# BurryChen/lv_slam

Hardware: AMD Instinct MI355X
Metric: NDT registrations/sec (64k-pt Velodyne pairs) (higher is better)
Workload: dtype f32 terms, f64 accumulation

## Files before the change

include/mi355_ndt.h:

```cpp
#ifndef MI355_NDT_H_
#define MI355_NDT_H_

#include <stddef.h>
#include <stdint.h>

#ifdef __cplusplus
extern "C" {
#endif

#define MI355NDT_OK               0
#define MI355NDT_ERR_BAD_HANDLE  (-1)
#define MI355NDT_ERR_BAD_ARG     (-2)
#define MI355NDT_ERR_HIP         (-3)
#define MI355NDT_ERR_GRID        (-4)
#define MI355NDT_ERR_NO_DEVICE   (-5)
#define MI355NDT_ERR_UNSUPPORTED (-6)
#define MI355NDT_WARN_TOLERANCE_ARITH 1
#define MI355NDT_TOLERANCE_MIN_HITS   4096
#define MI355NDT_ERR_STATE       (-7)

enum mi355ndt_neighbor { MI355NDT_KDTREE = 0, MI355NDT_DIRECT26 = 1, MI355NDT_DIRECT7 = 2, MI355NDT_DIRECT1 = 3 };
enum mi355ndt_variant { MI355NDT_VARIANT_OMP = 0 , MI355NDT_VARIANT_PCA = 1  };

typedef struct mi355ndt_params {
  float  resolution;
  double step_size;
  double outlier_ratio;
  double trans_epsilon;
  int    max_iterations;
  int    neighbor_mode;
  int    variant;
  int    min_points_per_voxel;
  double min_covar_eigvalue_mult;
} mi355ndt_params;

typedef struct mi355ndt_result {
  float     final_colmajor[16];
  double    trans_probability;
  double    score;
  int       iterations;
  int       converged;
  int       sweeps;
  int       status;
  long long hits_last;
} mi355ndt_result;

typedef struct mi355ndt_voxel {
  int32_t idx;
  int32_t n;
  double  mean[3];
  float   icov[9];
  int32_t weight;
} mi355ndt_voxel;

typedef struct mi355ndt_profile {
  double    sweep_ms;
  long long sweep_launches;
  double    sweep_alg_bytes;
  long long sweep_hits;
  long long sweep_points;
  double    build_ms;
  long long build_launches;
  double    build_alg_bytes;
  double    update_ms;
  long long update_launches;
  long long async_fallbacks;
  long long stream_launches;
  long long stream_carried;
  long long stream_redone;
  long long cloud_uploads;
  long long cloud_upload_bytes;
  long long cloud_transfers;
  long long cloud_promotions;
  long long stream_reserved_slots;
  long long stream_launch_slots;
  long long score_only_sweeps;
} mi355ndt_profile;

typedef struct mi355ndt_handle mi355ndt_handle;

const char* mi355ndt_version(void);
int mi355ndt_device_count(void);
int mi355ndt_host_numa_node(int device);

int mi355ndt_default_params(mi355ndt_params* p);

int mi355ndt_create(const mi355ndt_params* params, int device, mi355ndt_handle** out);
int mi355ndt_destroy(mi355ndt_handle* h);

int mi355ndt_set_params(mi355ndt_handle* h, const mi355ndt_params* params);
int mi355ndt_get_params(const mi355ndt_handle* h, mi355ndt_params* out);

int mi355ndt_set_stream(mi355ndt_handle* h, void* hip_stream);
const char* mi355ndt_last_error(const mi355ndt_handle* h);


int mi355ndt_set_target(mi355ndt_handle* h, const void* pts, size_t n, size_t stride_bytes);
int mi355ndt_set_source(mi355ndt_handle* h, const void* pts, size_t n, size_t stride_bytes);
int mi355ndt_promote_source_to_target(mi355ndt_handle* h);
int mi355ndt_align(mi355ndt_handle* h, const float guess_colmajor[16], mi355ndt_result* out);
int mi355ndt_get_aligned(mi355ndt_handle* h, void* out_pts, size_t stride_bytes);

int mi355ndt_get_incremental(mi355ndt_handle* h, int pair, float transformation_colmajor[16], float previous_colmajor[16]);

int mi355ndt_get_fitness_score(mi355ndt_handle* h, double max_range, double* score, long long* n_inliers);
int mi355ndt_fitness_score_T(mi355ndt_handle* h, const float T_colmajor[16], double max_range, double* score, long long* n_inliers);

int mi355ndt_calculate_score(mi355ndt_handle* h, const void* pts, size_t n, size_t stride_bytes, double* score);

int mi355ndt_convert_transform(const double x[6], float out_colmajor[16]);

enum mi355ndt_option {
  MI355NDT_OPT_F32_SUM_ORDER = 1,
  MI355NDT_OPT_ASYNC_ALIGN = 2,
  MI355NDT_OPT_DEBUG_ASYNC_ABORT = 3,
  MI355NDT_OPT_STREAM_THRESHOLD = 4,
  MI355NDT_OPT_STREAM_RESERVE = 5,
  MI355NDT_OPT_DEBUG_ASYNC_RINGS = 6,
  MI355NDT_OPT_ARITH = 7,
  MI355NDT_OPT_SCORE_ONLY_LAST_SWEEP = 8,
  MI355NDT_OPT_KF_FITNESS_CELL_MM = 9,
  MI355NDT_OPT_OUTLIER_CELL_MM = 10,
  MI355NDT_OPT_PREFILTER_GROUP = 11,
  MI355NDT_OPT_POSE_MODEL = 12,
  MI355NDT_OPT_NDT_CLASS = 13
};
int mi355ndt_set_option(mi355ndt_handle* h, int option, int value);
int mi355ndt_get_option(const mi355ndt_handle* h, int option, int* value);

int mi355ndt_derivatives(mi355ndt_handle* h, const double p[6], double* score, double g[6], double H[36], long long* hits);
int mi355ndt_compute_hessian(mi355ndt_handle* h, const double p[6], double H[36]);
int mi355ndt_derivatives_T(mi355ndt_handle* h, const float T_colmajor[16], const float Rj_rowmajor[9],
                           double* score, double g[6], double H[36], long long* hits);
int mi355ndt_get_grid(mi355ndt_handle* h, int pair, int min_b[3], int max_b[3], int div_b[3], int* n_voxels);
int mi355ndt_get_voxels(mi355ndt_handle* h, int pair, mi355ndt_voxel* out, size_t capacity);


int mi355ndt_batch_reserve(mi355ndt_handle* h, int n_pairs, size_t max_target_pts, size_t max_source_pts);
int mi355ndt_batch_set_target(mi355ndt_handle* h, int pair, const void* pts, size_t n, size_t stride_bytes);
int mi355ndt_batch_set_source(mi355ndt_handle* h, int pair, const void* pts, size_t n, size_t stride_bytes);
int mi355ndt_batch_set_clouds(mi355ndt_handle* h, int first_pair, int n, const void* const* targets, const size_t* target_counts,
                              const void* const* sources, const size_t* source_counts, size_t stride_bytes, int n_threads);
int mi355ndt_batch_bind_device(mi355ndt_handle* h, int n_pairs,
                               const float* d_targets, const int* target_counts, size_t target_pitch,
                               const float* d_sources, const int* source_counts, size_t source_pitch);
int mi355ndt_batch_build_targets(mi355ndt_handle* h);
int mi355ndt_batch_align(mi355ndt_handle* h, const float* guesses_colmajor, mi355ndt_result* out);
int mi355ndt_batch_size(const mi355ndt_handle* h);
int mi355ndt_batch_fitness_scores(mi355ndt_handle* h, const float* T_colmajor, double max_range, double* scores, long long* n_inliers);
int mi355ndt_batch_pose_records(mi355ndt_handle* h, int id_base, int id_stride, void* d_records, size_t capacity);

int mi355ndt_stream_begin(mi355ndt_handle* h, int n_contexts , int max_pairs, size_t max_target_pts, size_t max_source_pts);
int mi355ndt_stream_submit(mi355ndt_handle* h, int n_pairs, const float* d_targets, const int* target_counts, size_t target_pitch,
                           const float* d_sources, const int* source_counts, size_t source_pitch, const float* guesses_colmajor,
                           long long* batch_id);
int mi355ndt_stream_submit_host(mi355ndt_handle* h, int n_pairs, const void* const* targets, const size_t* target_counts, const void* const* sources,
                                const size_t* source_counts, size_t stride_bytes, const float* guesses_colmajor, int n_threads, long long* batch_id);
int mi355ndt_stream_collect(mi355ndt_handle* h, long long batch_id, mi355ndt_result* out);
int mi355ndt_stream_pose_records(mi355ndt_handle* h, void* d_records, size_t capacity, int id_base, int id_stride);
int mi355ndt_pack_pose_records(const mi355ndt_result* results, int n, int id_base, int id_stride, void* records, size_t capacity);
int mi355ndt_stream_end(mi355ndt_handle* h);

int mi355ndt_set_latency_mode(mi355ndt_handle* h, int on);

typedef struct mi355ndt_seq_params {
  double keyframe_delta_trans;
  double keyframe_delta_angle;
  double keyframe_delta_time;
} mi355ndt_seq_params;

typedef struct mi355ndt_seq_frame {
  double odom_colmajor[16];
  float  tf_s2k_colmajor[16];
  double trans_probability;
  double dx, da, dt;
  int    key_id;
  int    new_keyframe;
  int    iterations, converged;
  int    aligns;
  int    pad;
} mi355ndt_seq_frame;

typedef struct mi355ndt_seq_stats {
  double    upload_ms;
  double    build_ms;
  double    track_ms;
// ... 187 lines not shown
```

lv_slam_amd/csrc/mi355_ndt.hip:

```cpp
#include <hip/hip_runtime.h>

#include <cstdio>
#include <cstdlib>
#include <cstddef>
#include <cstring>
#include <string>
#include <vector>
#include <algorithm>
#include <cmath>
#include <mutex>
#include <atomic>
#include <thread>
#include <sched.h>
#include <fstream>
#include <chrono>
#include <memory>
#include <map>
#include <array>
#include <type_traits>

#include "mi355_ndt.h"
#include "ndt_math.hpp"
#include "ndt_types.hpp"
#include "ndt_build.hpp"
#include "ndt_segsort.hpp"
#include "ndt_sweep.hpp"
#include "ndt_newton.hpp"
#include "ndt_update.hpp"
#include "ndt_upload.hpp"
#include "ndt_pose_record.hpp"
#include "ndt_hessian.hpp"
#include "ndt_sweep_kd.hpp"
#include "ndt_fitness.hpp"
#include "ndt_prefilter.hpp"
#include "ndt_prefilter_batch.hpp"
#include "ndt_prefilter_approx.hpp"
#include "ndt_mapcloud.hpp"
#include "ndt_keyframe.hpp"
#include "ndt_kffitness.hpp"
#include "ndt_outlier.hpp"
#include "ndt_outlier_batch.hpp"
#include "ndt_gicp.hpp"
#include "gicp_bfgs.hpp"
#include "gicp_lockstep.hpp"
#include "ndt_icp.hpp"
#include "icp_outer.hpp"
#include "ndt_sequence.hpp"
#include "ndt_async.hpp"
#include "ndt_hostmem.hpp"
#include "ndt_grid_state.hpp"
#ifndef NDT_SINGLE_TU
#include "ndt_ord1_list.hpp"
#include "ndt_fast_list.hpp"
#define NDT_DECLARE extern template
NDT_ORD1_KERNELS(NDT_DECLARE)
NDT_FAST_KERNELS(NDT_DECLARE)
#endif

#include "ndt_engine.hpp"
#include "ndt_host_life.hpp"
#include "ndt_host_upload.hpp"
#include "ndt_host_profile.hpp"
#include "ndt_host_build.hpp"
#include "ndt_host_sweep.hpp"
#include "ndt_host_align.hpp"
#include "ndt_host_hooks.hpp"
#include "ndt_host_fitness.hpp"
#include "ndt_host_voxel.hpp"
#include "ndt_host_prefilter.hpp"
#include "ndt_host_mapcloud.hpp"
#include "ndt_host_keyframe.hpp"
#include "ndt_host_kffitness.hpp"
#include "ndt_host_outlier.hpp"
#include "ndt_host_gicp.hpp"
#include "ndt_host_gicp_batch.hpp"
#include "ndt_host_icp.hpp"
#include "ndt_host_icp_batch.hpp"
#include "ndt_host_sequence.hpp"
#include "ndt_host_stream.hpp"
```

lv_slam_amd/csrc/ndt_async.hpp:

```cpp
#pragma once
#include "ndt_types.hpp"
#include "ndt_math.hpp"
#include "ndt_sweep.hpp"
#include "ndt_update.hpp"
#include "ndt_pose_record.hpp"

#define ASYNC_POS_STRIDE 32
#define ASYNC_ARR_STRIDE 16
#define ASYNC_MAX_CTX    4
#define ASYNC_MAX_CARRY  128
#define ASYNC_CTX_SHIFT  24

struct AsyncCtx {
  const float* src; size_t pitch;
  PairState* st; const GridDesc* gd; const BitWord* words; const VoxelRec* recs; const float* cent;
  double* partials; const int* src_cnt; unsigned* arrived; mi355ndt_result* results;
  unsigned* n_done;
  int must_finish;
  int pose_base; PoseRecord* pose; int pose_stride;
  int score_only;
};
struct AsyncTab { AsyncCtx c[ASYNC_MAX_CTX]; };
#define NDT_GP(T) __attribute__((address_space(1))) T*
struct AsyncCtxG {
// ... 129 lines not shown
    if (rc == NEWTON_SWEEP && stop_thresh > 0 && !C.must_finish)
      suspend = n_live - __hip_atomic_load((const gu32*)&ctl->fin, RLX_AGENT) <= (unsigned)stop_thresh;
    if (rc == NEWTON_SWEEP && !suspend) {
      const unsigned g = __hip_atomic_fetch_add((gu32*)&ctl->pub, 1u, RLX_AGENT);
      __hip_atomic_store((gu32*)reinterpret_cast<unsigned*>(ring + (size_t)(g & 7u) * ring_cap + (g >> 3)), (unsigned)tw, RLX_AGENT);
    } else if (rc == NEWTON_SWEEP) {
      const unsigned k = __hip_atomic_fetch_add((gu32*)&ctl->susp, 1u, RLX_AGENT);
      if (k < (unsigned)ASYNC_MAX_CARRY) __hip_atomic_store((gu32*)&ctl->carry[k], (unsigned)tw, RLX_AGENT);
      asm volatile("s_waitcnt vmcnt(0)" ::: "memory");
      __hip_atomic_fetch_add((gu32*)&ctl->fin, 1u, RLX_AGENT);
    } else {
      if (C.pose) C.pose[b] = pose_record(Ssh.final_cm, Ssh.score, Ssh.it, Ssh.converged, C.pose_base + b * C.pose_stride);
      asm volatile("s_waitcnt vmcnt(0)" ::: "memory");
      if (C.n_done) __hip_atomic_fetch_add((gu32*)C.n_done, 1u, RLX_AGENT);
      __hip_atomic_fetch_add((gu32*)&ctl->fin, 1u, RLX_AGENT);
    }
  }
  TL_STAMP(9);
  if (rc == NEWTON_SWEEP) {
    constexpr int RBI = (int)(offsetof(PairState, reb_inc) / 8);
    double pn[6]; float inc[16];
    newton_rebase(Ssh.p, Ssh.dir, Ssh.a_t, pn, inc);
    if (lane == 0) {
      for (int a = 0; a < 6; a++) __hip_atomic_store(sg + RB0 + a, (unsigned long long)__double_as_longlong(pn[a]), RLX_AGENT);
      for (int a = 0; a < 8; a++)
        __hip_atomic_store(sg + RBI + a, (unsigned long long)__float_as_uint(inc[2 * a]) | ((unsigned long long)__float_as_uint(inc[2 * a + 1]) << 32), RLX_AGENT);
      asm volatile("s_waitcnt vmcnt(0)" ::: "memory");
      __hip_atomic_store(sg + RBT, (unsigned long long)(long long)Ssh.sweeps, RLX_AGENT);
    }
  }
  __builtin_amdgcn_s_setprio(0);
}

NDT_KERNEL void k_stream_inputs(const unsigned* __restrict__ host_in, unsigned* __restrict__ dev_in, const unsigned n_in, unsigned* __restrict__ clear, const unsigned n_clear,
                                unsigned long long* stamp) {
  if (threadIdx.x == 0 && stamp) *stamp = (unsigned long long)wall_clock64();
  for (unsigned i = threadIdx.x; i < n_in; i += blockDim.x) dev_in[i] = host_in[i];
  for (unsigned i = threadIdx.x; i < n_clear; i += blockDim.x) clear[i] = 0u;
}

NDT_KERNEL void k_stream_status(const AsyncCtl* __restrict__ ctl, const CtxStat* __restrict__ stat, volatile unsigned* host_slot, const unsigned seq) {
  const int i = threadIdx.x;
  static_assert(offsetof(AsyncCtl, fin) == 4 && offsetof(AsyncCtl, susp) == 16 && offsetof(StreamStatus, ctx) == 16 && offsetof(StreamStatus, seq) == 80 && offsetof(StreamStatus, build_t0) == 88, "status layout");
  if (i < 4) host_slot[i] = reinterpret_cast<const unsigned*>(ctl)[1 + i];
  else if (i < 4 + 4 * ASYNC_MAX_CTX) host_slot[i] = reinterpret_cast<const unsigned*>(stat)[i - 4];
  __threadfence_system();
  __syncthreads();
  if (i == 0) host_slot[20] = seq;
}

#define NDT_CTX_PARAMS(i) const float* __restrict__ src##i, size_t pitch##i, PairState* st##i, const GridDesc* __restrict__ gd##i, const BitWord* __restrict__ words##i, \
                          const VoxelRec* __restrict__ recs##i, double* partials##i, const int* __restrict__ src_cnt##i, unsigned* arrived##i, const float* __restrict__ cent##i
#define NDT_CTX_SEL(f, ci) ((ci) == 0 ? f##0 : (ci) == 1 ? f##1 : (ci) == 2 ? f##2 : f##3)
template <bool PCA, int K, int ORD>
__global__ void __launch_bounds__(SWEEP_THREADS, (SweepTune<PCA, K, ORD>::WPE))
k_align_async(const AsyncTab* __restrict__ tab, int items_per_pair, int* ring, int ring_cap, AsyncCtl* ctl, SweepConst sc, unsigned long long* hits_total,
              double step_max, double eps, int max_iterations, int stop_thresh, unsigned debug_abort_pos, unsigned debug_ring_mask, int claim_items,
              NDT_CTX_PARAMS(0), NDT_CTX_PARAMS(1), NDT_CTX_PARAMS(2), NDT_CTX_PARAMS(3)) {
  const int lane = threadIdx.x & 63, wv = threadIdx.x >> 6;
  __shared__ double exp_tab[64];
  __shared__ PairState Ssh[WAVES];
  __shared__ double sol[WAVES][SOL_WORDS];
  if (threadIdx.x < 64) exp_tab[threadIdx.x] = ndtm::c_exp2_64[threadIdx.x];
  __syncthreads();
  const int x = blockIdx.x & 7;
  if (!((debug_ring_mask >> x) & 1u)) return;
  const gu32* ringx = (const gu32*)reinterpret_cast<const unsigned*>(ring + (size_t)x * ring_cap);
  const gu32* fin_p = (const gu32*)&ctl->fin;
  gu32* pos_p = (gu32*)&ctl->pos[x * ASYNC_POS_STRIDE];
  const unsigned n_live = ctl->n_live;
  const int I = items_per_pair;
  const int CLAIM = K == 1 ? ASYNC_CLAIM(1) : (claim_items == 2 ? 2 : 1);
  const int Iu = I / CLAIM;
  Timeline tl;
  auto give_up = [&]() {
    __hip_atomic_store((gu32*)&ctl->abort_, 1u, RLX_AGENT);
    __hip_atomic_store((gu32*)&ctl->fin, n_live, RLX_AGENT);
  };
  bool held = false;
  bool helped = false;
  unsigned held_pos = 0;
  const gu64* pubfin_p = (const gu64*)reinterpret_cast<const unsigned long long*>(ctl);
  static_assert(offsetof(AsyncCtl, pub) == 0 && offsetof(AsyncCtl, fin) == 4, "pub and fin are polled as one 8-byte word");
  auto wait_ticket = [&](unsigned& p, int have) -> int {
    int w = have;
    unsigned sp = p;
    int st = 0;
    if (lane == 0) {
      unsigned spins = helped ? ASYNC_HELP_AFTER : 0u;
      const int t = (int)(p / (unsigned)Iu);
      while (w < 0) {
        const unsigned long long pf = __hip_atomic_load(pubfin_p, RLX_AGENT);
        if ((unsigned)(pf >> 32) >= n_live) { w = -2; break; }
        if (ASYNC_HELP_RINGS && spins >= ASYNC_HELP_AFTER && (spins & 3u) == 3u) {
          const unsigned y = ((unsigned)x + 1u + (spins >> 2) % 7u) & 7u;
          gu32* pos_y = (gu32*)&ctl->pos[y * ASYNC_POS_STRIDE];
          const unsigned q = __hip_atomic_load(pos_y, RLX_AGENT);
          const unsigned pubv = (unsigned)pf;
          const unsigned slots_y = pubv > y ? ((pubv - 1u - y) >> 3) + 1u : 0u;
          const unsigned tq = q / (unsigned)Iu;
          if (tq < slots_y && (int)tq < ring_cap) {
            unsigned expect = q;
            if (__hip_atomic_compare_exchange_strong(pos_y, &expect, q + 1u, __ATOMIC_RELAXED, __ATOMIC_RELAXED, __HIP_MEMORY_SCOPE_AGENT)) {
              const gu32* slot = (const gu32*)reinterpret_cast<const unsigned*>(ring + (size_t)y * ring_cap + tq);
              int ws = (int)__hip_atomic_load(slot, RLX_AGENT);
              unsigned lag = 0;
              while (ws < 0 && ++lag <= ASYNC_SPIN_LIMIT) { __builtin_amdgcn_s_sleep(2); ws = (int)__hip_atomic_load(slot, RLX_AGENT); }
              if (ws < 0) { give_up(); w = -2; break; }
              w = ws; sp = q; st = 1;
              break;
            }
          }
        }
        __builtin_amdgcn_s_sleep(32);
        if (t < ring_cap) w = (int)__hip_atomic_load(ringx + t, RLX_AGENT);
        if (++spins > ASYNC_SPIN_LIMIT) { give_up(); w = -2; break; }
      }
    }
    w = __builtin_amdgcn_readfirstlane(w);
    helped = __builtin_amdgcn_readfirstlane(st) != 0;
    if (helped) { held = true; held_pos = p; p = __builtin_amdgcn_readfirstlane(sp); }
    return w;
  };
  unsigned pos = 0;
  if (lane == 0) pos = __hip_atomic_fetch_add(pos_p, 1u, RLX_AGENT);
  pos = __builtin_amdgcn_readfirstlane(pos);
  int tw = -1;
  if (lane == 0 && (int)(pos / (unsigned)Iu) < ring_cap) tw = (int)__hip_atomic_load(ringx + pos / (unsigned)Iu, RLX_AGENT);
  tw = wait_ticket(pos, tw);
  if (tw < 0) return;
  unsigned pose_w = sweep_pose_words(NDT_CTX_SEL(st, tw >> ASYNC_CTX_SHIFT) + (tw & ((1 << ASYNC_CTX_SHIFT) - 1)));
#pragma unroll 1
  for (;;) {
    if (x == 0 && pos == debug_abort_pos) { if (lane == 0) give_up(); break; }
    const int rem = (int)(pos % (unsigned)Iu) * CLAIM;
    TL_STAMP(10);
    const int ci = tw >> ASYNC_CTX_SHIFT;
    AsyncCtx C = async_ctx_load(tab, ci);
    C.src = NDT_CTX_SEL(src, ci); C.pitch = NDT_CTX_SEL(pitch, ci); C.st = NDT_CTX_SEL(st, ci); C.gd = NDT_CTX_SEL(gd, ci); C.words = NDT_CTX_SEL(words, ci);
    C.recs = NDT_CTX_SEL(recs, ci); C.partials = NDT_CTX_SEL(partials, ci); C.src_cnt = NDT_CTX_SEL(src_cnt, ci); C.arrived = NDT_CTX_SEL(arrived, ci);
    C.cent = NDT_CTX_SEL(cent, ci);
    const int b = tw & ((1 << ASYNC_CTX_SHIFT) - 1);
    const int n_b = C.src_cnt[b];
#ifndef ASYNC_D1_PIPE
#define ASYNC_D1_PIPE 1
#endif
    const bool last = __builtin_amdgcn_readlane(pose_w, POSE_W_LAST) != 0;
    auto items = [&](auto so_c) {
      constexpr bool SO = decltype(so_c)::value;
      if constexpr (K == 1 && ASYNC_D1_PIPE && ORD != 2) {
        sweep_rows_d1<PCA, ORD, ASYNC_CLAIM(1), SO>(b, rem, C.src, C.pitch, C.gd, C.words, C.recs, C.partials, I, sc, exp_tab, pose_w, n_b, b, tl);
      } else {
#pragma unroll 1
        for (int k = 0; k < CLAIM; k++)
          sweep_item<PCA, K, 8, false, ORD, true, SO>(b, rem + k, C.src, C.pitch, C.st, C.gd, C.words, C.recs, C.partials, I, sc, C.cent, nullptr, exp_tab, pose_w, n_b, b, tl);
      }
    };
    if (last) items(std::true_type()); else items(std::false_type());
    unsigned npos = held_pos;
    if (lane == 0 && !held) npos = __hip_atomic_fetch_add(pos_p, 1u, RLX_AGENT);
    held = false;
    asm volatile("s_waitcnt vmcnt(0)" ::: "memory");
    npos = __builtin_amdgcn_readfirstlane(npos);
    const int tn = (int)(npos / (unsigned)Iu);
    unsigned old = 0;
    int ntw = -1;
    if (lane == 0) {
      old = __hip_atomic_fetch_add((gu32*)(C.arrived + (size_t)b * ASYNC_ARR_STRIDE), (unsigned)CLAIM, RLX_AGENT);
      if (tn < ring_cap) ntw = (int)__hip_atomic_load(ringx + tn, RLX_AGENT);
    }
    old = __builtin_amdgcn_readfirstlane(old);
    ntw = __builtin_amdgcn_readfirstlane(ntw);
    unsigned npose = 0;
    if (ntw >= 0) npose = sweep_pose_words(NDT_CTX_SEL(st, ntw >> ASYNC_CTX_SHIFT) + (ntw & ((1 << ASYNC_CTX_SHIFT) - 1)));
    TL_STAMP(8);
    if ((old + (unsigned)CLAIM) % (unsigned)I == 0u) {
      async_update(C, b, tw, n_b, I, Ssh[wv], sol[wv], ring, ring_cap, ctl, n_live, stop_thresh, hits_total, step_max, eps, max_iterations, tl);
      TL_STAMP(15);
    }
    if (ntw < 0) {
      ntw = wait_ticket(npos, ntw);
      if (ntw < 0) break;
      npose = sweep_pose_words(NDT_CTX_SEL(st, ntw >> ASYNC_CTX_SHIFT) + (ntw & ((1 << ASYNC_CTX_SHIFT) - 1)));
    }
    tw = ntw; pos = npos; pose_w = npose;
  }
  tl.flush(0, 16);
}
```

lv_slam_amd/csrc/ndt_build.hpp:

```cpp
#pragma once
#include "ndt_types.hpp"
#include "ndt_math.hpp"

__device__ __forceinline__ unsigned mm_enc_max(int ord) { return (unsigned)ord ^ 0x80000000u; }
__device__ __forceinline__ unsigned mm_enc_min(int ord) { return ~((unsigned)ord ^ 0x80000000u); }
__device__ __forceinline__ int mm_dec_max(unsigned e) { return (int)(e ^ 0x80000000u); }
__device__ __forceinline__ int mm_dec_min(unsigned e) { return (int)(~e ^ 0x80000000u); }

#define MM_ILP 4
struct __attribute__((packed, aligned(4))) MmQuad { float v[4]; };
__global__ void __launch_bounds__(256) k_minmax(const float* __restrict__ tgt, size_t pitch, const int* __restrict__ cnt, unsigned* mm) {
  const int b = blockIdx.y;
  const int n = cnt[b];
  const float* X = tgt + (size_t)b * 3 * pitch;
  int mn[3] = {INT_MAX, INT_MAX, INT_MAX}, mx[3] = {INT_MIN, INT_MIN, INT_MIN};
  auto take = [&](const float x, const float y, const float z) {
    if (!finite3(x, y, z)) return;
    const int ox = f2ord(x), oy = f2ord(y), oz = f2ord(z);
    mn[0] = min(mn[0], ox); mx[0] = max(mx[0], ox);
    mn[1] = min(mn[1], oy); mx[1] = max(mx[1], oy);
    mn[2] = min(mn[2], oz); mx[2] = max(mx[2], oz);
  };
  const int stride = (int)(gridDim.x * blockDim.x) * 4;
  for (int i0 = (int)(blockIdx.x * blockDim.x + threadIdx.x) * 4; i0 < n; i0 += stride * MM_ILP) {
// ... 97 lines not shown


#define RUN_ILP 4
template <typename KeyT>
__device__ __forceinline__ void run_heads(const KeyT* __restrict__ K, size_t pitch, size_t i0, size_t stride, int min_points, unsigned cmask,
                                          bool head[RUN_ILP], unsigned cell[RUN_ILP]) {
  KeyT k0[RUN_ILP], km[RUN_ILP], kl[RUN_ILP];
  const size_t span = (size_t)(min_points > 0 ? min_points - 1 : 0);
#pragma unroll
  for (int u = 0; u < RUN_ILP; u++) {
    const size_t i = i0 + (size_t)u * stride;
    const bool in = i < pitch;
    k0[u] = in ? K[i] : (KeyT)cmask;
    km[u] = (in && i != 0) ? K[i - 1] : ~(KeyT)0;
    kl[u] = (in && i + span < pitch) ? K[i + span] : ~(KeyT)0;
  }
#pragma unroll
  for (int u = 0; u < RUN_ILP; u++) {
    const size_t i = i0 + (size_t)u * stride;
    cell[u] = (unsigned)k0[u] & cmask;
    head[u] = i < pitch && cell[u] != cmask && (i == 0 || km[u] != k0[u]) && (i + span < pitch) && kl[u] == k0[u];
  }
}
#define LS_SLICE (64 * RUN_ILP)
static inline unsigned ls_slice_cap(int min_points) { return (unsigned)(LS_SLICE / (min_points > 0 ? min_points : 1) + 2); }
static inline unsigned ls_slices(size_t pitch) { return (unsigned)((pitch + LS_SLICE - 1) / LS_SLICE); }
template <typename KeyT>
__global__ void __launch_bounds__(256) k_mark(const KeyT* __restrict__ keys, size_t pitch, const GridDesc* __restrict__ gd,
                                               BitWord* words, unsigned* heads, unsigned* head_cnt, unsigned n_slices, unsigned slice_cap,
                                               int min_points, int cb) {
  const int b = blockIdx.y;
  const int lane = threadIdx.x & 63;
  const unsigned q = blockIdx.x * 4u + (threadIdx.x >> 6);
  if (q >= n_slices) return;
  const size_t i0 = (size_t)q * LS_SLICE + lane;
  bool head[RUN_ILP];
  unsigned cell[RUN_ILP];
  run_heads<KeyT>(keys + (size_t)b * pitch, pitch, i0, 64, min_points, (1u << cb) - 1u, head, cell);
  unsigned* H = heads + ((size_t)b * n_slices + q) * slice_cap;
  const unsigned long long below = (1ull << lane) - 1ull;
  unsigned n = 0;
#pragma unroll
  for (int u = 0; u < RUN_ILP; u++) {
    const unsigned long long hm = __ballot(head[u]);
    if (head[u]) {
      atomicOr(&words[gd[b].word_off + (cell[u] >> 6)].bits, 1ull << (cell[u] & 63));
      H[n + (unsigned)__popcll(hm & below)] = (unsigned)(i0 + (size_t)u * 64);
    }
    n += (unsigned)__popcll(hm);
  }
  if (lane == 0) head_cnt[(size_t)b * n_slices + q] = n;
}
#define RANK_ROWS 8
__global__ void __launch_bounds__(1024) k_rank(GridDesc* gd, BitWord* words, const unsigned* __restrict__ heads, const unsigned* __restrict__ head_cnt,
                                                 unsigned n_slices, unsigned slice_cap, unsigned* seg_start) {
  __shared__ unsigned wtot[17];
  const int b = blockIdx.x;
  BitWord* W = words + gd[b].word_off;
  const int nw = gd[b].nwords;
  const int lane = threadIdx.x & 63, wv = threadIdx.x >> 6;
  unsigned base = 0;
  for (int w0 = 0; w0 < nw; w0 += 1024 * RANK_ROWS) {
    const int wbase = w0 + wv * 64 * RANK_ROWS;
    unsigned c[RANK_ROWS], ex[RANK_ROWS], run = 0;
#pragma unroll
    for (int u = 0; u < RANK_ROWS; u++) { const int w = wbase + u * 64 + lane; c[u] = (w < nw) ? (unsigned)__popcll(W[w].bits) : 0u; }
#pragma unroll
    for (int u = 0; u < RANK_ROWS; u++) {
      unsigned inc = c[u];
#pragma unroll
      for (int o = 1; o < 64; o <<= 1) { const unsigned t = __shfl_up(inc, o); if (lane >= o) inc += t; }
      ex[u] = run + inc - c[u];
      run += __shfl(inc, 63);
    }
    if (lane == 0) wtot[wv] = run;
    __syncthreads();
    if (wv == 0) {
      const unsigned v = lane < 16 ? wtot[lane] : 0u;
      unsigned inc = v;
#pragma unroll
      for (int o = 1; o < 16; o <<= 1) { const unsigned t = __shfl_up(inc, o); if (lane >= o) inc += t; }
      if (lane < 16) wtot[lane] = inc - v;
      if (lane == 15) wtot[16] = inc;
    }
    __syncthreads();
    const unsigned off = base + wtot[wv];
#pragma unroll
    for (int u = 0; u < RANK_ROWS; u++) { const int w = wbase + u * 64 + lane; if (w < nw) W[w].prefix = off + ex[u]; }
    base += wtot[16];
    __syncthreads();
  }
  if (threadIdx.x == 0) gd[b].n_voxels = (int)base;
  unsigned hbase = 0;
  for (unsigned q0 = 0; q0 < n_slices; q0 += 1024) {
    const unsigned q = q0 + threadIdx.x;
    const unsigned c = q < n_slices ? head_cnt[(size_t)b * n_slices + q] : 0u;
    unsigned tot;
    const unsigned ex = block_exscan<1024>(c, &tot, wtot);
    const unsigned* H = heads + ((size_t)b * n_slices + q) * slice_cap;
    unsigned* S = seg_start + gd[b].rec_off + hbase + ex;
    for (unsigned k = 0; k < c; k++) S[k] = H[k];
    hbase += tot;
  }
}

__global__ void __launch_bounds__(256) k_sorted_points(const float* __restrict__ tgt, size_t pitch, const unsigned* __restrict__ vals, float4* __restrict__ sorted,
                                                        int nx, int n_targets) {
  int b, bx;
  if (!xcd_map(nx, n_targets, bx, b)) return;
  const float* X = tgt + (size_t)b * 3 * pitch;
  const unsigned* V = vals + (size_t)b * pitch;
  float4* P = sorted + (size_t)b * pitch;
  const size_t i0 = ((size_t)bx * 256 + threadIdx.x);
  const size_t stride = (size_t)nx * 256;
  for (size_t i = i0; i < pitch; i += stride * RUN_ILP) {
    unsigned v[RUN_ILP];
    float4 q[RUN_ILP];
#pragma unroll
    for (int u = 0; u < RUN_ILP; u++) { const size_t j = i + u * stride; v[u] = j < pitch ? V[j] : 0u; }
#pragma unroll
    for (int u = 0; u < RUN_ILP; u++) { const unsigned k = v[u] < pitch ? v[u] : 0u; q[u] = make_float4(X[k], X[pitch + k], X[2 * pitch + k], 0.f); }
#pragma unroll
    for (int u = 0; u < RUN_ILP; u++) { const size_t j = i + u * stride; if (j < pitch) P[j] = q[u]; }
  }
}

#ifdef NDT_TIMELINE
__device__ unsigned long long g_ltl[16];
#define LTL_DECL unsigned long long ltl[12] = {0, 0, 0, 0, 0, 0, 0, 0, 0, 0, 0, 0}; unsigned long long ltl_last = __builtin_readcyclecounter(); const unsigned long long ltl_t0 = ltl_last
#define LTL_STAMP(k) do { __builtin_amdgcn_sched_barrier(0); const unsigned long long t_ = __builtin_readcyclecounter(); ltl[k] += t_ - ltl_last; ltl_last = t_; __builtin_amdgcn_sched_barrier(0); } while (0)
#define LTL_COUNT(k, v) do { ltl[k] += (unsigned long long)(v); } while (0)
#define LTL_FLUSH() do { ltl[10] = 1; ltl[11] = __builtin_readcyclecounter() - ltl_t0; if ((threadIdx.x & 63) == 0 && (blockIdx.x % 24) == (threadIdx.x >> 6) * 5) for (int k_ = 0; k_ < 12; k_++) atomicAdd(&g_ltl[k_], ltl[k_]); } while (0)
#define LTL_ARRIVED1(a) asm volatile("" : "+v"(a))
#else
#define LTL_DECL do {} while (0)
#define LTL_STAMP(k) do {} while (0)
#define LTL_COUNT(k, v) do {} while (0)
#define LTL_FLUSH() do {} while (0)
#define LTL_ARRIVED1(a) do {} while (0)
#endif
#define LS_WAVES 4
template <typename KeyT, bool CENT, bool SORTED = false>
__global__ void __launch_bounds__(64 * LS_WAVES) k_leafsum(const float* __restrict__ tgt, size_t pitch,
                                                           const KeyT* __restrict__ keys, const unsigned* __restrict__ vals ,
                                                           const GridDesc* __restrict__ gd, const unsigned* __restrict__ seg_start,
                                                           double* sums, int* vox_idx, int* vox_n, int cb, float* cent,
                                                           int nx, int n_targets) {
  __shared__ double term[LS_WAVES][64][9];
  __shared__ float termf[CENT ? LS_WAVES : 1][64][3];
  int b, bx;
  if (!xcd_map(nx, n_targets, bx, b)) return;
// ... 249 lines not shown
```

lv_slam_amd/csrc/ndt_engine.hpp:

```cpp
#pragma once

struct mi355ndt_handle;
struct EngineDel { void operator()(mi355ndt_handle* e) const { (void)mi355ndt_destroy(e); } };

struct StreamCtx {
  long long batch_id = -1; int n_pairs = 0;
  bool busy = false;
  bool redo = false;
  bool done_sync = false;
  long long launch = -1;
  DevBuf<int> d_in; PinBuf<int> h_in; unsigned* h_in_dev = nullptr;
  PinBuf<mi355ndt_result> h_res; mi355ndt_result* d_res_map = nullptr;
  std::vector<float> guesses;
  PoseRecord* d_pose = nullptr; int pose_cap = 0, pose_base = 0, pose_stride = 1;
  std::unique_ptr<mi355ndt_handle, EngineDel> e;
};
struct StreamState {
  static constexpr int EV = 16;
  bool sync_only = false, drop_carry = true;
  int nctx = 0, max_pairs = 0, items = 0, ring_cap = 0, thresh = 0;
  bool thresh_given = false;
  size_t max_tgt = 0, max_src = 0;
  int plan_cb = 0; size_t plan_words = 0;
  void* pose_next = nullptr; size_t pose_cap_next = 0; int pose_base_next = 0, pose_stride_next = 1;
  long long next_id = 0, launches = 0, counted = 0;
  long long recovered_upto = -1;
  DevBuf<AsyncCtl> d_ctl;
  DevBuf<int> d_ring;
  DevBuf<CtxStat> d_stat;
  HipStream build_stream; int reserve_wg = 0, launch_slots = 0;
  HipEvent ev_built[ASYNC_MAX_CTX], ev_launched[EV], ev_prepared[EV]; bool prep_first = true;
  PinBuf<volatile StreamStatus> h_status; StreamStatus* d_status = nullptr;
  StreamCtx ctx[ASYNC_MAX_CTX];
};

struct VoxelScratch {
  DevBuf<float> in, x, out;
  DevBuf<unsigned char> keep;
  DevBuf<unsigned> keys, vals;
  DevBuf<unsigned> hist, offs, tmp;
  DevBuf<int> flag, pos;
  DevBuf<int> mm, cnt, aabb, stat;
  DevBuf<PfGrid> grid; DevBuf<McBox> box;
  DevBuf<unsigned char> tab; PinBuf<unsigned char> h_tab;
  DevBuf<double> part; PinBuf<double> h_part;
  PinBuf<int> h_ret;
  bool pending = false;
};

struct CloudIndex {
  static constexpr int NO_INDEX = -1;
  DevBuf<unsigned char> blob; int status = NO_INDEX; int n_fin = 0;
};

struct GicpCache {
  DevBuf<double> cov;
  int k = -1; double eps = 0.0;
};
struct GicpSide {
  DevBuf<float> rows_own; size_t n = 0, pitch = 0;
  int kf_id = -1; bool set = false;
  CloudIndex index; GicpCache cache;
};

struct mi355ndt_handle {
  int device = 0;
  HipStream own_stream;
  hipStream_t stream = nullptr;
  mi355ndt_params prm;
  std::string err;

  int n_pairs = 0, cap_pairs = 0;
  size_t tgt_pitch = 0, src_pitch = 0;
  size_t own_tgt_pitch = 0, own_src_pitch = 0;
  int own_tgt_pairs = 0, own_src_pairs = 0;
  DevBuf<float> d_tgt_own, d_src_own;
  const float *d_tgt = nullptr, *d_src = nullptr;
  DevBuf<int> d_tgt_cnt_own, d_src_cnt_own;
  int *d_tgt_cnt = nullptr, *d_src_cnt = nullptr;
  std::vector<int> h_tgt_cnt, h_src_cnt;
  std::vector<int> up_tgt_cnt, up_src_cnt;
  bool have_target = false, have_source = false;
  GridsBuilt built{};
// ... 35 lines not shown
    DevBuf<int> idx, m; DevBuf<double> maha, part; DevBuf<float> moved;
    PinBuf<double> h_rec; double* d_rec = nullptr;
    bool have_corr = false, have_final = false; int n_matched = 0;
    float final_cm[16] = {1,0,0,0, 0,1,0,0, 0,0,1,0, 0,0,0,1};
  } gicp;
  struct GicpBatch {
    struct Slot {
      GicpSide side;
      DevBuf<int> idx; DevBuf<double> maha, part;
      bool have_final = false; float final_cm[16];
    };
    std::vector<Slot> slot;
    DevBuf<int> m;
    PinBuf<double> h_rec; double* d_rec = nullptr;
    PinBuf<GcSlot> h_tab; DevBuf<GcSlot> d_tab;
    int rounds = 0; std::vector<int> requests;
  } gicp_batch;
  struct IcpWork {
    DevBuf<float> W, d2; DevBuf<int> idx; DevBuf<double> part;
    size_t n = 0, pitch = 0;
    bool have_final = false; IcpRun run;
  };
  struct Icp {
    mi355ndt_icp_params prm{0.0, 10, -DBL_MAX, 1.3407807929942596e154, 3, 0};
    GicpSide side[2];
    IcpWork work;
    DevBuf<int> m; DevBuf<float> moved;
    PinBuf<double> h_rec; double* d_rec = nullptr;
  } icp;
  struct IcpBatch {
    struct Slot { GicpSide side; IcpWork work; };
    std::vector<Slot> slot;
    DevBuf<int> m;
    PinBuf<double> h_rec; double* d_rec = nullptr;
    PinBuf<IcpSlot> h_tab; DevBuf<IcpSlot> d_tab;
    int rounds = 0; std::vector<int> requests;
  } icp_batch;
  float last_final[16] = {1,0,0,0, 0,1,0,0, 0,0,1,0, 0,0,0,1};
  PinBuf<unsigned> h_pin_u;

  DevBuf<PairState> d_state;
  DevBuf<double> d_partials;
  int chunks_per_pair = 0;
  int rows_per_pair = 0, pts_per_chunk = CHUNK_PTS;
  int items_per_pair = 0;
  bool async_force = false;
  bool async_align = true;
  int score_only_last = 1;
  DevBuf<int> d_ring; DevBuf<unsigned> d_arrived; DevBuf<AsyncCtl> d_actl;
  PinBuf<AsyncCtl> h_pin_actl;
  DevBuf<AsyncTab> d_atab;
  unsigned debug_abort_pos = 0xFFFFFFFFu;
  unsigned debug_ring_mask = 0xFFu;
  int arith = 0;
  DevBuf<VoxelRecF> d_recs_fast;
  int pose_model = 0;
  int ndt_class = 0;
  DevBuf<double> d_pcl_rows;
  DevBuf<float> d_euler_rows;
  int f32_sum_order = 0;
  double gauss_last[3] = {0, 0, 0};
  DevBuf<float> d_score_pts; DevBuf<double> d_score_part;
  bool latency_mode = false;
  bool seq_running = false;
  int fine_it = 0;
  int fine_tiles = 2;
  int dyn_shift = -1;
  DevBuf<int> d_grid_of;
  const int* d_grid_of_use = nullptr;
  DevBuf<SeqState> d_seq; DevBuf<mi355ndt_seq_frame> d_seq_out; DevBuf<double> d_stamps;
  PinBuf<volatile int> h_seq_flags; int* d_seq_flags = nullptr;
  DevBuf<float> d_guess_own;
  float* d_guess = nullptr;
  PinBuf<float> h_pin_guess;
  DevBuf<mi355ndt_result> d_results;
  DevBuf<int> d_active;
  DevBuf<int> d_active_list;
  DevBuf<SweepCtl> d_ctl;
  int ctl_idx = 0;
  int n_cu = 256;
  PinBuf<int> h_pin_active;
  HipEvent ev_burst[2];
  DevBuf<unsigned long long> d_hits;
  DevBuf<float> d_hook;
  DevBuf<float> d_aligned;
  PinBuf<float> h_pin_aligned;
  struct UpSlot { PinBuf<float> h; DevBuf<float> d; HipEvent ev; bool used = false, filling = false; };
  static constexpr int UP_SLOTS = 12;
  UpSlot up[UP_SLOTS];
  int up_next = 0;
  static constexpr int UP_STREAMS = 4;
  HipStream copy_stream[UP_STREAMS];
  HipEvent ev_uploads[UP_STREAMS], ev_compute;
  bool uploads_pending = false;
  std::mutex up_mtx;

  bool async_build = false;
  int plan_cb = 0; size_t plan_words = 0;
  unsigned* d_bstat = nullptr;
  bool counts_preloaded = false;
  bool build_stamped = false;
  bool word_off_cleared = false;

  std::unique_ptr<StreamState> ss;
  int s_thresh_opt = -1;
  int s_reserve_opt = -1;
// ... 44 lines not shown
  sc.K = neighbor_K(mode);
  sc.table = sc.K == 1 ? 0 : sc.K == 7 ? 1 : 2;
}

static void gauss_constants3(double outlier_ratio, float resolution, double d[3]) {
  double c1 = 10 * (1 - outlier_ratio);
  double c2 = outlier_ratio / pow((double)resolution, 3);
  d[2] = -log(c2);
  d[0] = -log(c1 + c2) - d[2];
  d[1] = -2 * log((-log(c1 * exp(-0.5) + c2) - d[2]) / d[0]);
}
static void gauss_constants(const mi355ndt_params& p, double& d1, double& d2) {
  double d[3];
  gauss_constants3(p.outlier_ratio, p.resolution, d);
  d1 = d[0]; d2 = d[1];
}

static int check_params(const mi355ndt_params& p) {
  if (!(p.resolution > 0) || !std::isfinite(p.resolution)) return MI355NDT_ERR_BAD_ARG;
  if (p.neighbor_mode < 0 || p.neighbor_mode > 3) return MI355NDT_ERR_BAD_ARG;
  if (p.variant < 0 || p.variant > 1) return MI355NDT_ERR_BAD_ARG;
  if (p.min_points_per_voxel < 1) return MI355NDT_ERR_BAD_ARG;
  if (p.max_iterations < 0) return MI355NDT_ERR_BAD_ARG;
  return MI355NDT_OK;
}

static int eff_model(const mi355ndt_handle* h) { return class_model(h->ndt_class, h->pose_model); }
static GridExtras eff_extras(const mi355ndt_handle* h, bool live = false) { return grid_extras(h->prm, model_arith(h->pose_model, h->arith, h->ndt_class), live, h->ndt_class); }
static bool fast_served(const mi355ndt_handle* h) { return eff_extras(h).recs_fast; }
static float* euler_rows_of(const mi355ndt_handle* h) { return eff_model(h) == POSE_MODEL_EULER ? h->d_euler_rows.p : nullptr; }
static double* pcl_rows_of(const mi355ndt_handle* h) { return h->ndt_class == NDT_CLASS_PCL ? h->d_pcl_rows.p : nullptr; }
#define NOT_EULER(h, what) do { \
    if ((h)->ndt_class == NDT_CLASS_PCL) { (h)->err = what ": not served under MI355NDT_OPT_NDT_CLASS = 1"; return MI355NDT_ERR_UNSUPPORTED; } \
    if ((h)->pose_model == POSE_MODEL_EULER) { (h)->err = what ": not served under MI355NDT_OPT_POSE_MODEL = 1"; return MI355NDT_ERR_UNSUPPORTED; } } while (0)

enum GridWant { GRIDS_ANY, GRIDS_CONFIG, GRIDS_LIVE };
static int ensure_grids(mi355ndt_handle* h, GridWant want);
template <typename N>
static void cloud_changed(mi355ndt_handle* h, bool tgt, int first_pair, int n, const N* counts) {
  std::lock_guard<std::mutex> lk(h->up_mtx);
  std::vector<int>& cnt = tgt ? h->h_tgt_cnt : h->h_src_cnt;
  for (int k = 0; k < n; k++) cnt[(size_t)(first_pair + k)] = (int)counts[k];
  (tgt ? h->have_target : h->have_source) = true;
  if (tgt) h->built.valid = false;
}
static void cloud_changed(mi355ndt_handle* h, bool tgt, int pair, size_t count) { cloud_changed(h, tgt, pair, 1, &count); }
static void clouds_reset(mi355ndt_handle* h, bool tgt, bool src) {
  std::lock_guard<std::mutex> lk(h->up_mtx);
  if (tgt) { std::fill(h->h_tgt_cnt.begin(), h->h_tgt_cnt.end(), 0); h->have_target = false; h->built.valid = false; }
  if (src) { std::fill(h->h_src_cnt.begin(), h->h_src_cnt.end(), 0); h->have_source = false; }
}
static bool async_served(const mi355ndt_handle* h) { return h->async_align && !mt_is_live(h->prm) && !is_pca_kd(h->prm) && model_leaves_rounds(h->pose_model, h->ndt_class); }
static double sweep_alg_bytes(double points, int K) { return points * (12.0 + 4.0 * K); }
static int launch_slots(const mi355ndt_handle* h, const SweepConst& sc, bool fast) { return h->n_cu * sweep_wpe(sc.K, fast); }
```

lv_slam_amd/csrc/ndt_host_align.hpp:

```cpp
#pragma once
static void tolerance_warnings(const mi355ndt_handle* h, mi355ndt_result* out, int n) {
  if (!fast_served(h)) return;
  for (int b = 0; b < n; b++)
    if (out[b].status == MI355NDT_OK && (out[b].hits_last < MI355NDT_TOLERANCE_MIN_HITS || out[b].iterations >= h->prm.max_iterations + 2))
      out[b].status = MI355NDT_WARN_TOLERANCE_ARITH;
}
static int ensure_seq_flags(mi355ndt_handle* h) {
  if (!h->d_seq_flags) {
    HIPCHK(h, h->h_seq_flags.reserve(16, hipHostMallocMapped | hipHostMallocCoherent));
    if (!(h->d_seq_flags = h->h_seq_flags.dev())) { h->err = "hipHostGetDevicePointer failed"; return MI355NDT_ERR_HIP; }
  }
  return MI355NDT_OK;
}

static int align_pump(mi355ndt_handle* h, SweepConst sc, int B) {
  int rc = ensure_seq_flags(h);
  if (rc) return rc;
  hipStream_t s = h->stream;
  h->h_seq_flags[0] = 0; h->h_seq_flags[1] = -1;
  sc.host_flags = h->d_seq_flags;
  sc.seq_no = 1;
  sc.rebase_block = 1;
  rc = launch_sweep(h, sc);
  if (rc) return rc;
  const int depth = 2;
  const long long max_rounds = h->prm.max_iterations + 4;
  long long enq = 0;
  auto t_progress = std::chrono::steady_clock::now();
  long long seen_last = -1;
  for (;;) {
    const long long seen = h->h_seq_flags[0];
    const int active = h->h_seq_flags[1];
    if (seen >= 1 && active == 0) break;
    if (seen != seen_last) { seen_last = seen; t_progress = std::chrono::steady_clock::now(); }
    if (enq >= max_rounds || enq + 1 - seen >= depth) {
      if (std::chrono::steady_clock::now() - t_progress > std::chrono::seconds(20)) { h->err = "align: the device stopped making progress"; return MI355NDT_ERR_STATE; }
      cpu_relax();
      continue;
    }
    k_update<<<B, UPD_THREADS, 0, s>>>(h->d_state, h->d_partials, h->rows_per_pair, h->pts_per_chunk, 1, h->d_results, h->d_active,
                                       h->d_active_list, h->d_ctl + h->ctl_idx, h->prof ? h->d_hits : nullptr, h->prm.step_size, h->prm.trans_epsilon,
                                       h->prm.max_iterations, 0, 0, nullptr, nullptr);
    sc.seq_no = (int)(enq + 2);
    rc = launch_sweep(h, sc);
    if (rc) return rc;
    enq++;
  }
  return MI355NDT_OK;
}

static void account_sweeps(mi355ndt_handle* h, const mi355ndt_result* out, const int* src_cnt, int n, int K) {
  if (!h->prof) return;
  for (int b = 0; b < n; b++) {
    h->P.sweep_alg_bytes += sweep_alg_bytes((double)out[b].sweeps * src_cnt[b], K);
    h->P.sweep_points += (long long)out[b].sweeps * src_cnt[b];
  }
}
static int finish_align(mi355ndt_handle* h, const SweepConst& sc, int B, mi355ndt_result* out, bool account, const AsyncCtl* launch = nullptr) {
  HIPCHK(h, hipMemcpyAsync(out, h->d_results, (size_t)B * sizeof(mi355ndt_result), hipMemcpyDeviceToHost, h->stream));
  HIPCHK(h, hipStreamSynchronize(h->stream));
  HIPCHK(h, hipGetLastError());
  if (launch && (launch->abort_ || launch->fin != (unsigned)B)) {
    h->P.async_fallbacks++;
    return MI355NDT_ERR_UNSUPPORTED;
  }
  if (account) account_sweeps(h, out, h->h_src_cnt.data(), B, sc.K);
  h->aligned_once = true;
  return MI355NDT_OK;
}

static int align_async(mi355ndt_handle* h, const SweepConst& sc, int B, mi355ndt_result* out) {
  const int ring_cap = async_ring_cap(h, B);
  if (ring_cap == 0) return MI355NDT_ERR_UNSUPPORTED;
  if (h->d_ring.reserve((size_t)8 * ring_cap) != hipSuccess) { (void)hipGetLastError(); return MI355NDT_ERR_UNSUPPORTED; }
  HIPCHK(h, h->d_arrived.reserve((size_t)B * ASYNC_ARR_STRIDE));
  HIPCHK(h, h->d_actl.reserve(1));
  HIPCHK(h, h->d_atab.reserve(1));
  HIPCHK(h, h->h_pin_actl.reserve(1));
  AsyncLaunch L;
  memset(&L.tab, 0, sizeof L.tab);
  fill_async_ctx(h, L.tab.c[0]);
  L.new_ci = 0; L.n_new = B;
  L.st_new = h->d_state; L.guess_new = h->d_guess; L.src_cnt_new = h->d_src_cnt; L.gd_new = h->d_grid; L.arrived_new = h->d_arrived;
  L.active_list = h->d_active_list; L.sweep_ctl = h->d_ctl;
  L.tab_dev = h->d_atab; L.ring = h->d_ring; L.ring_cap = ring_cap; L.ctl = h->d_actl; L.prev = nullptr;
  L.items_per_pair = h->items_per_pair; L.stop_thresh = 0; L.debug_abort_pos = h->debug_abort_pos; L.debug_ring_mask = h->debug_ring_mask;
  int rc = launch_async(h, sc, L);
  if (rc) return rc;
  HIPCHK(h, hipMemcpyAsync(h->h_pin_actl, h->d_actl, 8 * sizeof(unsigned), hipMemcpyDeviceToHost, h->stream));
  return finish_align(h, sc, B, out, true, h->h_pin_actl.p);
}

static int batch_align_impl(mi355ndt_handle* h, const float* guesses, mi355ndt_result* out) {
  if (!guesses || !out) return MI355NDT_ERR_BAD_ARG;
  if (h->n_pairs <= 0 || !h->d_tgt || !h->d_src) return MI355NDT_ERR_STATE;
  const bool mt_live = mt_is_live(h->prm);
  if (const char* why = model_refuses(h->prm, h->pose_model, h->ndt_class)) { h->err = why; return MI355NDT_ERR_UNSUPPORTED; }
  int rc = ensure_grids(h, GRIDS_CONFIG);
  if (rc) return rc;
  rc = prep_align_ws(h);
  if (rc) return rc;
  const int B = h->n_pairs;
  hipStream_t s = h->stream;
  SweepConst sc;
  make_sweep_const(h, sc);
  gauss_constants3(h->prm.outlier_ratio, h->prm.resolution, h->gauss_last);
  h->ev_last_fresh = false;
  memcpy(h->h_pin_guess, guesses, (size_t)B * 16 * sizeof(float));
  HIPCHK(h, hipMemcpyAsync(h->d_guess, h->h_pin_guess, (size_t)B * 16 * sizeof(float), hipMemcpyHostToDevice, s));
  h->ctl_idx = 0;
  const bool big_batch = (long long)B * h->items_per_pair > (long long)launch_slots(h, sc, sweep_ord(h, sc) == 2) * WAVES;
  if (async_served(h) && (big_batch || h->async_force) && !h->fine_it) {
    rc = align_async(h, sc, B, out);
    if (rc != MI355NDT_ERR_UNSUPPORTED) return rc;
  }
  HIPCHK(h, hipMemsetAsync(h->d_ctl, 0, 2 * sizeof(SweepCtl), s));
  k_init_state<<<(B + 63) / 64, 64, 0, s>>>(h->d_state, h->d_guess, h->d_src_cnt, h->d_grid, B, h->d_active_list, h->d_ctl, euler_rows_of(h), pcl_rows_of(h));
  if (h->fine_it) {
    rc = align_pump(h, sc, B);
    return rc ? rc : finish_align(h, sc, B, out, true);
  }
  rc = launch_sweep(h, sc);
  if (rc) return rc;
  const int max_rounds = h->prm.max_iterations + 4;
  double pts_total = 0;
  for (int b = 0; b < B; b++) pts_total += h->h_src_cnt[b];
  const double alg_static = sweep_alg_bytes(pts_total, sc.K);
  if (h->prof) {
    h->P.sweep_alg_bytes += alg_static;
    h->P.sweep_points += (long long)pts_total;
  }
  const int burst = 2;
  int round = 0, n_enq = 0;
  int cnt[2] = {0, 0};
  auto enqueue_burst = [&]() -> int {
    const int slot = n_enq & 1;
    h->ev_last_fresh = false;
    int* dact = h->d_active + slot * burst;
    hipError_t e = hipMemsetAsync(dact, 0, burst * sizeof(int), s);
    if (e != hipSuccess) return MI355NDT_ERR_HIP;
    int k = 0;
    for (; k < burst && round < max_rounds; k++, round++) {
      if (h->prof) HIPCHK(h, ev_begin(h, h->ev_update));
      k_update<<<B, UPD_THREADS, 0, s>>>(h->d_state, h->d_partials, h->rows_per_pair, h->pts_per_chunk, h->fine_it ? 1 : 0, h->d_results, dact + k,
                                h->d_active_list, h->d_ctl + h->ctl_idx, h->prof ? h->d_hits : nullptr,
                                h->prm.step_size, h->prm.trans_epsilon, h->prm.max_iterations, 0, mt_live ? 1 : 0, euler_rows_of(h), pcl_rows_of(h));
      if (mt_live) {
        launch_hessian(h, sc);
        k_update<<<B, UPD_THREADS, 0, s>>>(h->d_state, h->d_partials, h->rows_per_pair, h->pts_per_chunk, h->fine_it ? 1 : 0, h->d_results, dact + k,
                                  h->d_active_list, h->d_ctl + h->ctl_idx, nullptr,
                                  h->prm.step_size, h->prm.trans_epsilon, h->prm.max_iterations, 0, 2, nullptr, nullptr);
      }
      if (h->prof) HIPCHK(h, ev_end(h, h->ev_update));
      int r = launch_sweep(h, sc);
      if (r) return r;
    }
    cnt[slot] = k;
    HIPCHK(h, hipMemcpyAsync(h->h_pin_active + slot * burst, dact, burst * sizeof(int), hipMemcpyDeviceToHost, s));
    HIPCHK(h, hipEventRecord(h->ev_burst[slot], s));
    n_enq++;
    return MI355NDT_OK;
  };
  rc = enqueue_burst();
  if (rc) return rc;
  for (int done = 0; done < n_enq; done++) {
    if (round < max_rounds) { rc = enqueue_burst(); if (rc) return rc; }
// ... 92 lines not shown
```

lv_slam_amd/csrc/ndt_host_build.hpp:

```cpp
#pragma once

static int build_targets_impl(mi355ndt_handle* h, const GridExtras make) {
  if (h->n_pairs <= 0 || !h->d_tgt) return MI355NDT_ERR_STATE;
  HIPCHK(h, hipSetDevice(h->device));
  { int rcu = uploads_before_compute(h); if (rcu) return rcu; }
  const int B = h->n_pairs;
  const size_t pitch = h->tgt_pitch;
  const size_t total = (size_t)B * pitch;
  hipStream_t s = h->stream;
  if (h->async_build && h->counts_preloaded) {
    h->up_tgt_cnt.clear();
  } else if (h->up_tgt_cnt.size() != (size_t)B || !std::equal(h->up_tgt_cnt.begin(), h->up_tgt_cnt.end(), h->h_tgt_cnt.begin())) {
    HIPCHK(h, hipMemcpyAsync(h->d_tgt_cnt, h->h_tgt_cnt.data(), B * sizeof(int), hipMemcpyHostToDevice, s));
    HIPCHK(h, hipStreamSynchronize(s));
    h->up_tgt_cnt.assign(h->h_tgt_cnt.begin(), h->h_tgt_cnt.begin() + B);
  }

  HIPCHK(h, h->d_keys_a.reserve(total)); HIPCHK(h, h->d_keys_b.reserve(total));
  HIPCHK(h, h->d_vals_a.reserve(total)); HIPCHK(h, h->d_vals_b.reserve(total));
  const int minpts = h->prm.min_points_per_voxel;
  const size_t rpp = pitch / (size_t)minpts + 1;
  if (rpp > ((size_t)1 << ID_BITS)) { h->err = "target too large: voxel ids would not fit the sweep's queue entries"; return MI355NDT_ERR_BAD_ARG; }
  if ((size_t)B * rpp > h->d_recs.cap || rpp != h->recs_per_pair) {
    const size_t need = (size_t)B * rpp;
// ... 1 lines not shown
    HIPCHK(h, h->d_recs.realloc_exact(need)); HIPCHK(h, h->d_vox_idx.realloc_exact(need)); HIPCHK(h, h->d_vox_n.realloc_exact(need));
    HIPCHK(h, h->d_seg_start.realloc_exact(need)); HIPCHK(h, h->d_sums.realloc_exact(need * 9)); HIPCHK(h, h->d_cent.realloc_exact(need * 3));
    h->recs_per_pair = rpp;
  }
  h->ev_last_fresh = false;
  const bool build_events = h->prof && !(h->build_stamped && h->async_build);
  if (build_events) HIPCHK(h, ev_begin(h, h->ev_build));
  const int gx = (int)((pitch + 255) / 256);
  h->built.valid = false;
  if (!h->word_off_cleared) HIPCHK(h, hipMemsetAsync(h->d_word_off, 0, (2 + 6 * (size_t)h->cap_pairs) * sizeof(unsigned), s));
  h->word_off_cleared = false;
  k_minmax<<<dim3(std::max(1, std::min((gx + 3) / 4 / MM_ILP, 64)), B), 256, 0, s>>>(h->d_tgt, pitch, h->d_tgt_cnt, h->d_minmax);
  k_griddesc<<<(B + 63) / 64, 64, 0, s>>>(h->d_minmax, h->d_grid, h->d_nwords, h->prm.resolution, B, (unsigned)rpp);
  k_word_offsets<<<1, 1024, 0, s>>>(h->d_grid, h->d_nwords, B, h->d_word_off);
  size_t total_words;
  int cb;
  const bool planned = h->async_build && h->plan_cb > 0 && h->plan_words > 0 && h->plan_words <= h->d_words.cap && h->d_bstat;
  if (planned) {
    k_build_check<<<(B + 255) / 256, 256, 0, s>>>(h->d_word_off, h->d_grid, h->d_nwords, B, (unsigned)std::min(h->plan_words, (size_t)0xFFFFFFFFu), h->plan_cb, h->d_bstat + 1);
    total_words = h->plan_words;
    cb = h->plan_cb;
  } else {
    HIPCHK(h, hipMemcpyAsync(h->h_pin_u, h->d_word_off, 2 * sizeof(unsigned), hipMemcpyDeviceToHost, s));
    HIPCHK(h, hipStreamSynchronize(s));
    total_words = h->h_pin_u[0];
    cb = std::max(1, ceil_log2(h->h_pin_u[1] + 1u));
    if (h->async_build) cb = std::max(cb, h->plan_cb);
    if (h->d_bstat) HIPCHK(h, hipMemsetAsync(h->d_bstat + 3, 0, sizeof(unsigned), s));
  }
  if (total_words > h->d_words.cap) HIPCHK(h, h->d_words.reserve(std::max(total_words, (size_t)1024)));
  if (total_words) HIPCHK(h, hipMemsetAsync(h->d_words, 0, total_words * sizeof(BitWord), s));
  const bool want_cent = make.cent, fast_recs = make.recs_fast, want_kdw = make.kdw;
  if (make.icov64) HIPCHK(h, h->d_icov64.reserve(h->d_recs.cap * 9));
  if (fast_recs) HIPCHK(h, h->d_recs_fast.reserve(h->d_recs.cap));
  if (want_kdw) HIPCHK(h, h->d_kdw.reserve(h->d_recs.cap));
  {
    unsigned *ka = h->d_keys_a, *kb = h->d_keys_b;
    const RsPlan plan = rs_plan(cb);
    const int npass = plan.passes;
    const int tiles = (int)((pitch + RS_TILE - 1) / RS_TILE);
    const size_t rs_need = ((size_t)B * tiles) << RS_MAX_BITS;
    HIPCHK(h, h->d_rs_hist.reserve(rs_need)); HIPCHK(h, h->d_rs_offs.reserve(rs_need));
    unsigned *kin = (npass & 1) ? ka : kb, *kout = (npass & 1) ? kb : ka;
    unsigned *vin = (npass & 1) ? h->d_vals_a : h->d_vals_b, *vout = (npass & 1) ? h->d_vals_b : h->d_vals_a;
    const RsPoints points = {h->d_tgt, h->d_tgt_cnt, h->d_grid, cb, kin};
    for (int p = 0; p < npass; p++) {
      rs_pass(s, plan.bits, kin, vin, kout, vout, pitch, p * plan.bits, h->d_rs_hist, h->d_rs_offs, tiles, B, p == 0, p == 0 ? &points : nullptr);
      std::swap(kin, kout); std::swap(vin, vout);
    }
    const unsigned nsl = ls_slices(pitch), scap = ls_slice_cap(minpts);
    HIPCHK(h, h->d_heads.reserve((size_t)B * nsl * scap));
    HIPCHK(h, h->d_head_cnt.reserve((size_t)B * nsl));
    k_mark<unsigned><<<dim3((nsl + 3) / 4, B), 256, 0, s>>>(kb, pitch, h->d_grid, h->d_words, h->d_heads, h->d_head_cnt, nsl, scap, minpts, cb);
    k_rank<<<B, 1024, 0, s>>>(h->d_grid, h->d_words, h->d_heads, h->d_head_cnt, nsl, scap, h->d_seg_start);
    const int lb = std::max(1, std::min((int)((rpp + LS_WAVES - 1) / LS_WAVES), 64));
    auto leafsum = [&](auto kern, const unsigned* vals) {
      kern<<<xcd_grid(lb, B), 64 * LS_WAVES, 0, s>>>(h->d_tgt, pitch, kb, vals, h->d_grid, h->d_seg_start, h->d_sums, h->d_vox_idx, h->d_vox_n, cb, h->d_cent, lb, B);
    };
    if (fast_recs && !want_cent && !h->leaf_sorted) {
      k_leafsum_tree<<<xcd_grid(lb, B), 64 * LS_WAVES, 0, s>>>(h->d_tgt, pitch, kb, h->d_vals_b, h->d_grid, h->d_seg_start, h->d_sums, h->d_vox_idx, h->d_vox_n, cb, lb, B);
    } else if (h->leaf_sorted) {
      HIPCHK(h, h->d_sorted.reserve(total));
      const int gb = std::max(1, std::min((int)((pitch + 256 * RUN_ILP - 1) / (256 * RUN_ILP)), 64));
      k_sorted_points<<<xcd_grid(gb, B), 256, 0, s>>>(h->d_tgt, pitch, h->d_vals_b, h->d_sorted, gb, B);
      leafsum(want_cent ? k_leafsum<unsigned, true, true> : k_leafsum<unsigned, false, true>, reinterpret_cast<const unsigned*>(h->d_sorted.p));
    } else leafsum(want_cent ? k_leafsum<unsigned, true> : k_leafsum<unsigned, false>, h->d_vals_b);
  }
  k_voxels<<<dim3((unsigned)((rpp + 255) / 256), B), 256, 0, s>>>(h->d_grid, h->d_sums, h->d_recs, h->d_vox_n,
                                                                  h->prm.min_covar_eigvalue_mult, h->prm.variant == MI355NDT_VARIANT_PCA,
                                                                  make.icov64 ? h->d_icov64 : nullptr, want_kdw ? h->d_kdw : nullptr, fast_recs ? h->d_recs_fast : nullptr);
  HIPCHK(h, hipGetLastError());
  if (h->prof) {
    if (build_events) HIPCHK(h, ev_end(h, h->ev_build));
    double pts = 0;
    for (int b = 0; b < B; b++) pts += h->h_tgt_cnt[b];
    h->P.build_alg_bytes += pts * (12 + 12 + 4 + 16);
  }
  h->built = GridsBuilt{true, make, h->prm.resolution, cb, total_words, false};
  return compute_enqueued(h);
}

static int build_targets(mi355ndt_handle* h, const GridExtras make) {
  NOT_IN_STREAM(h);
  const int rc = build_targets_impl(h, make);
  if (rc != MI355NDT_OK && h->ev_compute) (void)compute_enqueued(h);
  return rc;
}
int mi355ndt_batch_build_targets(mi355ndt_handle* h) {
  if (!h) return MI355NDT_ERR_BAD_HANDLE;
  return build_targets(h, eff_extras(h));
}

static int ensure_grids(mi355ndt_handle* h, GridWant want) {
  HIPCHK(h, hipSetDevice(h->device));
  { int rcu = uploads_before_compute(h); if (rcu) return rcu; }
  const GridExtras make = eff_extras(h, want == GRIDS_LIVE);
  return grids_serve(h->built, want == GRIDS_ANY ? GridExtras{} : make) ? (int)MI355NDT_OK : build_targets(h, make);
}
```

lv_slam_amd/csrc/ndt_host_hooks.hpp:

```cpp
#pragma once

int mi355ndt_get_aligned(mi355ndt_handle* h, void* out_pts, size_t stride) {
  if (!h) return MI355NDT_ERR_BAD_HANDLE;
  if (!out_pts || stride < 12) return MI355NDT_ERR_BAD_ARG;
  if (h->n_pairs < 1 || !h->d_src) return MI355NDT_ERR_STATE;
  HIPCHK(h, hipSetDevice(h->device));
  { int rcu = uploads_before_compute(h); if (rcu) return rcu; }
  const int n = h->h_src_cnt[0];
  if (n == 0) return MI355NDT_OK;
  HIPCHK(h, h->d_aligned.reserve((size_t)3 * n));
  HIPCHK(h, h->h_pin_aligned.reserve((size_t)3 * n));
  k_transform<<<(n + 255) / 256, 256, 0, h->stream>>>(h->d_src, h->src_pitch, h->d_state, 0, h->d_aligned, n);
  HIPCHK(h, hipMemcpyAsync(h->h_pin_aligned, h->d_aligned, (size_t)3 * n * sizeof(float), hipMemcpyDeviceToHost, h->stream));
  HIPCHK(h, hipStreamSynchronize(h->stream));
  unsigned char* o = (unsigned char*)out_pts;
  if (stride == 12) memcpy(o, h->h_pin_aligned, (size_t)n * 12);
  else for (int i = 0; i < n; i++) memcpy(o + (size_t)i * stride, h->h_pin_aligned + (size_t)3 * i, 12);
  return MI355NDT_OK;
}

int mi355ndt_get_incremental(mi355ndt_handle* h, int pair, float last[16], float prev[16]) {
  if (!h) return MI355NDT_ERR_BAD_HANDLE;
  if (pair < 0 || pair >= h->n_pairs) return MI355NDT_ERR_BAD_ARG;
  if (!h->d_state) return MI355NDT_ERR_STATE;
  if (!h->aligned_once) {
    for (int a = 0; a < 16; a++) { const float v = (a % 5 == 0) ? 1.f : 0.f; if (last) last[a] = v; if (prev) prev[a] = v; }
    return MI355NDT_OK;
  }
  HIPCHK(h, hipSetDevice(h->device));
  float buf[32];
  HIPCHK(h, hipMemcpyAsync(buf, (const char*)(h->d_state + pair) + offsetof(PairState, inc_cm), sizeof buf, hipMemcpyDeviceToHost, h->stream));
  HIPCHK(h, hipStreamSynchronize(h->stream));
  if (last) memcpy(last, buf, 16 * sizeof(float));
  if (prev) memcpy(prev, buf + 16, 16 * sizeof(float));
  return MI355NDT_OK;
}

static int run_hook_sweep(mi355ndt_handle* h, double* score, double g[6], double H[36], long long* hits) {
  SweepConst sc;
  make_sweep_const(h, sc);
  int rc = launch_sweep(h, sc);
  if (rc) return rc;
  k_update<<<1, UPD_THREADS, 0, h->stream>>>(h->d_state, h->d_partials, h->rows_per_pair, h->pts_per_chunk, h->fine_it ? 1 : 0, h->d_results, h->d_active, h->d_active_list, h->d_ctl,
                                    nullptr, 0, 0, 0, 1, 0, nullptr, nullptr);
  PairState S;
  HIPCHK(h, hipMemcpyAsync(&S, h->d_state, sizeof(PairState), hipMemcpyDeviceToHost, h->stream));
  HIPCHK(h, hipStreamSynchronize(h->stream));
  HIPCHK(h, hipGetLastError());
  if (score) *score = S.score;
  if (g) memcpy(g, S.g, sizeof S.g);
  if (H) memcpy(H, S.H, sizeof S.H);
  if (hits) *hits = S.hits;
  return MI355NDT_OK;
}

static int hook_ready(mi355ndt_handle* h) {
  h->ev_last_fresh = false;
  if (h->n_pairs < 1 || !h->have_target || !h->have_source) return MI355NDT_ERR_STATE;
  const int rc = ensure_grids(h, GRIDS_CONFIG);
  return rc ? rc : prep_align_ws(h);
}

int mi355ndt_derivatives(mi355ndt_handle* h, const double p[6], double* score, double g[6], double H[36], long long* hits) {
  if (!h) return MI355NDT_ERR_BAD_HANDLE;
  if (!p) return MI355NDT_ERR_BAD_ARG;
  if (const char* why = model_refuses(h->prm, h->pose_model, h->ndt_class)) { h->err = why; return MI355NDT_ERR_UNSUPPORTED; }
  int rc = hook_ready(h);
  if (rc) return rc;
  double* dp = (double*)h->d_hook.p;
  HIPCHK(h, hipMemcpyAsync(dp, p, 6 * sizeof(double), hipMemcpyHostToDevice, h->stream));
  HIPCHK(h, hipStreamSynchronize(h->stream));
  HIPCHK(h, hipMemsetAsync(h->d_ctl, 0, 2 * sizeof(SweepCtl), h->stream));
  h->ctl_idx = 0;
  k_set_pose_p<<<1, 1, 0, h->stream>>>(h->d_state, 0, dp, h->d_src_cnt, h->d_grid, h->d_active_list, h->d_ctl, 0, euler_rows_of(h), pcl_rows_of(h));
  return run_hook_sweep(h, score, g, H, hits);
}

int mi355ndt_compute_hessian(mi355ndt_handle* h, const double p[6], double H[36]) {
  if (!h) return MI355NDT_ERR_BAD_HANDLE;
  if (!p || !H) return MI355NDT_ERR_BAD_ARG;
  NOT_EULER(h, "mi355ndt_compute_hessian");
  int rc = hook_ready(h);
  if (rc == MI355NDT_OK) rc = ensure_grids(h, GRIDS_LIVE);
  if (rc) return rc;
  h->fine_it = 0; h->rows_per_pair = h->items_per_pair = h->chunks_per_pair * QUARTERS; h->pts_per_chunk = CHUNK_PTS;
  double* dp = (double*)h->d_hook.p;
  HIPCHK(h, hipMemcpyAsync(dp, p, 6 * sizeof(double), hipMemcpyHostToDevice, h->stream));
// ... 126 lines not shown
```

lv_slam_amd/csrc/ndt_host_life.hpp:

```cpp
#pragma once

const char* mi355ndt_version(void) { return "mi355ndt 0.1 (gfx950)"; }

int mi355ndt_device_count(void) {
  int n = 0;
  if (hipGetDeviceCount(&n) != hipSuccess) return 0;
  return n;
}

int mi355ndt_host_numa_node(int device) {
  int node = -1;
  if (hipDeviceGetAttribute(&node, hipDeviceAttributeHostNumaId, device) != hipSuccess) {
    (void)hipGetLastError();
    char bdf[64];
    if (hipDeviceGetPCIBusId(bdf, (int)sizeof bdf, device) != hipSuccess) { (void)hipGetLastError(); return -1; }
    for (char* c = bdf; *c; c++) if (*c >= 'A' && *c <= 'F') *c = (char)(*c - 'A' + 'a');
    std::ifstream f(std::string("/sys/bus/pci/devices/") + bdf + "/numa_node");
    if (f && (f >> node)) return node;
    unsigned dom = 0, bus = 0, dv = 0, fn = 0;
    if (sscanf(bdf, "%x:%x:%x.%x", &dom, &bus, &dv, &fn) != 4) return -1;
    const long want = (long)((bus << 8) | (dv << 3) | fn);
    auto prop = [](const std::string& path, const char* key, long& out) {
      std::ifstream pf(path);
      std::string k; long v;
// ... 25 lines not shown
static bool numa_cpus(int node, cpu_set_t* set) {
  CPU_ZERO(set);
  if (node < 0) return false;
  std::ifstream f("/sys/devices/system/node/node" + std::to_string(node) + "/cpulist");
  std::string txt;
  if (!f || !std::getline(f, txt)) return false;
  bool any = false;
  size_t pos = 0;
  while (pos < txt.size()) {
    size_t comma = txt.find(',', pos);
    std::string part = txt.substr(pos, comma == std::string::npos ? std::string::npos : comma - pos);
    size_t dash = part.find('-');
    int lo = atoi(part.c_str()), hi = dash == std::string::npos ? lo : atoi(part.c_str() + dash + 1);
    for (int c = lo; c <= hi && c < CPU_SETSIZE; c++) { CPU_SET(c, set); any = true; }
    if (comma == std::string::npos) break;
    pos = comma + 1;
  }
  return any;
}

int mi355ndt_default_params(mi355ndt_params* p) {
  if (!p) return MI355NDT_ERR_BAD_ARG;
  p->resolution = 1.0f;
  p->step_size = 0.1;
  p->outlier_ratio = 0.55;
  p->trans_epsilon = 0.1;
  p->max_iterations = 35;
  p->neighbor_mode = MI355NDT_DIRECT7;
  p->variant = MI355NDT_VARIANT_OMP;
  p->min_points_per_voxel = 6;
  p->min_covar_eigvalue_mult = 0.01;
  return MI355NDT_OK;
}

int mi355ndt_create(const mi355ndt_params* params, int device, mi355ndt_handle** out) {
  if (!out) return MI355NDT_ERR_BAD_ARG;
  *out = nullptr;
  int n = 0;
  if (hipGetDeviceCount(&n) != hipSuccess || n <= 0) return MI355NDT_ERR_NO_DEVICE;
  if (device < 0 || device >= n) return MI355NDT_ERR_BAD_ARG;
  mi355ndt_params p;
  mi355ndt_default_params(&p);
  if (params) p = *params;
  int rc = check_params(p);
  if (rc) return rc;
  std::unique_ptr<mi355ndt_handle> h(new mi355ndt_handle());
  h->device = device;
  h->prm = p;
  gauss_constants3(0.55, 1.0f, h->gauss_last);
  { hipDeviceProp_t pr; if (hipGetDeviceProperties(&pr, device) == hipSuccess && pr.multiProcessorCount > 0) h->n_cu = pr.multiProcessorCount; }
  if (const char* e = std::getenv("MI355NDT_LEAF_SORTED")) h->leaf_sorted = std::atoi(e) != 0;
  if (const char* e = std::getenv("MI355NDT_FINE_TILES")) { const int v = std::atoi(e); if (v == 1 || v == 2) h->fine_tiles = v; }
  if (const char* e = std::getenv("MI355NDT_ARITH")) h->arith = std::atoi(e) == 1 ? 1 : 0;
  if (const char* e = std::getenv("MI355NDT_ASYNC")) { h->async_align = std::atoi(e) != 0; h->async_force = std::atoi(e) == 2; }
  if (const char* e = std::getenv("MI355NDT_SCORE_ONLY_LAST_SWEEP")) h->score_only_last = std::atoi(e) != 0;
  if (const char* e = std::getenv("MI355NDT_SWEEP_DYN_SHIFT")) { const int v = std::atoi(e); if (v >= 0 && v <= 30) h->dyn_shift = v; }
  if (hipSetDevice(device) != hipSuccess || h->own_stream.create() != hipSuccess) return MI355NDT_ERR_HIP;
  h->stream = h->own_stream;
  if (h->h_pin_u.realloc_exact(4) != hipSuccess ||
      h->h_pin_active.realloc_exact(128) != hipSuccess ||
      h->d_active.realloc_exact(128) != hipSuccess ||
      h->d_ctl.realloc_exact(2) != hipSuccess ||
      h->d_hits.realloc_exact(2) != hipSuccess ||
      hipMemsetAsync(h->d_hits, 0, 2 * sizeof(unsigned long long), h->stream) != hipSuccess ||
      h->d_hook.realloc_exact(64 * sizeof(double) / sizeof(float)) != hipSuccess ||
      h->ev_compute.create() != hipSuccess || h->ev_burst[0].create() != hipSuccess || h->ev_burst[1].create() != hipSuccess) return MI355NDT_ERR_HIP;
  for (int i = 0; i < mi355ndt_handle::UP_STREAMS; i++)
    if (h->copy_stream[i].create() != hipSuccess || h->ev_uploads[i].create() != hipSuccess) return MI355NDT_ERR_HIP;
  *out = h.release();
  return MI355NDT_OK;
}

int mi355ndt_destroy(mi355ndt_handle* h) {
  if (!h) return MI355NDT_ERR_BAD_HANDLE;
  (void)hipSetDevice(h->device);
  (void)hipStreamSynchronize(h->stream);
  if (h->ss) (void)mi355ndt_stream_end(h);
  for (hipStream_t cs : h->copy_stream) if (cs) (void)hipStreamSynchronize(cs);
  delete h;
  return MI355NDT_OK;
}

int mi355ndt_get_params(const mi355ndt_handle* h, mi355ndt_params* out) {
  if (!h) return MI355NDT_ERR_BAD_HANDLE;
  if (!out) return MI355NDT_ERR_BAD_ARG;
  *out = h->prm;
  return MI355NDT_OK;
}

int mi355ndt_set_stream(mi355ndt_handle* h, void* s) {
  if (!h) return MI355NDT_ERR_BAD_HANDLE;
  NOT_IN_STREAM(h);
  (void)hipSetDevice(h->device);
  (void)hipStreamSynchronize(h->stream);
  if (s) {
    h->own_stream.reset();
    h->stream = (hipStream_t)s;
  } else if (!h->own_stream) {
    HIPCHK(h, h->own_stream.create());
    h->stream = h->own_stream;
  }
  return MI355NDT_OK;
}

const char* mi355ndt_last_error(const mi355ndt_handle* h) { return h ? h->err.c_str() : "bad handle"; }

int mi355ndt_synchronize(mi355ndt_handle* h) {
  if (!h) return MI355NDT_ERR_BAD_HANDLE;
  HIPCHK(h, hipSetDevice(h->device));
  for (hipStream_t cs : h->copy_stream) if (cs) HIPCHK(h, hipStreamSynchronize(cs));
  HIPCHK(h, hipStreamSynchronize(h->stream));
  return MI355NDT_OK;
}

int mi355ndt_batch_size(const mi355ndt_handle* h) { return h ? h->n_pairs : MI355NDT_ERR_BAD_HANDLE; }

int mi355ndt_set_params(mi355ndt_handle* h, const mi355ndt_params* p) {
  if (!h) return MI355NDT_ERR_BAD_HANDLE;
  NOT_IN_STREAM(h);
  if (!p) return MI355NDT_ERR_BAD_ARG;
  int rc = check_params(*p);
  if (rc) return rc;
  const mi355ndt_params old = h->prm;
  h->prm = *p;
  const bool radius_search = class_neighbor_mode(h->ndt_class, p->neighbor_mode) == MI355NDT_KDTREE || mt_is_live(*p);
  const bool keep_grid = old.resolution != p->resolution && h->n_pairs == 1 && !h->have_source && !radius_search && h->d_tgt == h->d_tgt_own;
  const bool regrid = (old.resolution != p->resolution && !keep_grid) || old.variant != p->variant ||
                      old.min_points_per_voxel != p->min_points_per_voxel ||
                      old.min_covar_eigvalue_mult != p->min_covar_eigvalue_mult ||
                      !grids_serve(h->built, grid_extras(*p, 0, false, h->ndt_class));
  if (regrid && h->built.valid) {
    h->built.valid = false;
    rc = ensure_grids(h, GRIDS_CONFIG);
    if (rc) h->prm = old;
    return rc;
  }
  return MI355NDT_OK;
}

int mi355ndt_set_option(mi355ndt_handle* h, int option, int value) {
  if (!h) return MI355NDT_ERR_BAD_HANDLE;
  if (h->ss && (option == MI355NDT_OPT_F32_SUM_ORDER || option == MI355NDT_OPT_ARITH || option == MI355NDT_OPT_ASYNC_ALIGN ||
                       option == MI355NDT_OPT_SCORE_ONLY_LAST_SWEEP || option == MI355NDT_OPT_POSE_MODEL || option == MI355NDT_OPT_NDT_CLASS)) NOT_IN_STREAM(h);
  if (option == MI355NDT_OPT_NDT_CLASS) {
    if (value != NDT_CLASS_OMP && value != NDT_CLASS_PCL) return MI355NDT_ERR_BAD_ARG;
    h->ndt_class = value;
    return MI355NDT_OK;
  }
  if (option == MI355NDT_OPT_POSE_MODEL) {
    if (value != POSE_MODEL_SE3 && value != POSE_MODEL_EULER) return MI355NDT_ERR_BAD_ARG;
    h->pose_model = value;
    return MI355NDT_OK;
  }
  if (option == MI355NDT_OPT_F32_SUM_ORDER) {
    if (value != 0 && value != 1) return MI355NDT_ERR_BAD_ARG;
    h->f32_sum_order = value;
    return MI355NDT_OK;
  }
  if (option == MI355NDT_OPT_ARITH) {
    if (value != 0 && value != 1) return MI355NDT_ERR_BAD_ARG;
    h->arith = value;
    return MI355NDT_OK;
  }
  if (option == MI355NDT_OPT_ASYNC_ALIGN) {
    if (value < 0 || value > 2) return MI355NDT_ERR_BAD_ARG;
    h->async_align = value != 0;
    h->async_force = value == 2;
    return MI355NDT_OK;
  }
  if (option == MI355NDT_OPT_SCORE_ONLY_LAST_SWEEP) {
    if (value != 0 && value != 1) return MI355NDT_ERR_BAD_ARG;
    h->score_only_last = value;
    return MI355NDT_OK;
  }
  if (option == MI355NDT_OPT_DEBUG_ASYNC_ABORT) {
    h->debug_abort_pos = value < 0 ? 0xFFFFFFFFu : (unsigned)value;
    return MI355NDT_OK;
  }
  if (option == MI355NDT_OPT_DEBUG_ASYNC_RINGS) {
    if ((value & 0xFF) == 0) return MI355NDT_ERR_BAD_ARG;
    h->debug_ring_mask = (unsigned)value & 0xFFu;
    return MI355NDT_OK;
  }
  if (option == MI355NDT_OPT_STREAM_THRESHOLD) {
    if (value < -1 || value > ASYNC_MAX_CARRY) return MI355NDT_ERR_BAD_ARG;
    h->s_thresh_opt = value;
    return MI355NDT_OK;
  }
  if (option == MI355NDT_OPT_STREAM_RESERVE) {
    if (value < -1 || value > 4096) return MI355NDT_ERR_BAD_ARG;
    h->s_reserve_opt = value;
    return MI355NDT_OK;
  }
  if (option == MI355NDT_OPT_KF_FITNESS_CELL_MM) {
    if (value < 1 || value > 1000000) return MI355NDT_ERR_BAD_ARG;
    h->kff_cell_mm = value;
    return MI355NDT_OK;
  }
  if (option == MI355NDT_OPT_OUTLIER_CELL_MM) {
    if (value < 1 || value > 1000000) return MI355NDT_ERR_BAD_ARG;
    h->ol_cell_mm = value;
    return MI355NDT_OK;
  }
  if (option == MI355NDT_OPT_PREFILTER_GROUP) {
    if (value < 0 || value > 4096) return MI355NDT_ERR_BAD_ARG;
    h->pf_group = value;
    return MI355NDT_OK;
  }
  return MI355NDT_ERR_BAD_ARG;
}
int mi355ndt_get_option(const mi355ndt_handle* h, int option, int* value) {
  if (!h) return MI355NDT_ERR_BAD_HANDLE;
  if (!value) return MI355NDT_ERR_BAD_ARG;
  if (option == MI355NDT_OPT_F32_SUM_ORDER) { *value = h->f32_sum_order; return MI355NDT_OK; }
  if (option == MI355NDT_OPT_ARITH) { *value = h->arith; return MI355NDT_OK; }
  if (option == MI355NDT_OPT_POSE_MODEL) { *value = h->pose_model; return MI355NDT_OK; }
  if (option == MI355NDT_OPT_NDT_CLASS) { *value = h->ndt_class; return MI355NDT_OK; }
  if (option == MI355NDT_OPT_ASYNC_ALIGN) { *value = h->async_force ? 2 : (h->async_align ? 1 : 0); return MI355NDT_OK; }
  if (option == MI355NDT_OPT_SCORE_ONLY_LAST_SWEEP) { *value = h->score_only_last; return MI355NDT_OK; }
  if (option == MI355NDT_OPT_DEBUG_ASYNC_ABORT) { *value = h->debug_abort_pos == 0xFFFFFFFFu ? -1 : (int)h->debug_abort_pos; return MI355NDT_OK; }
  if (option == MI355NDT_OPT_DEBUG_ASYNC_RINGS) { *value = (int)h->debug_ring_mask; return MI355NDT_OK; }
  if (option == MI355NDT_OPT_STREAM_THRESHOLD) { *value = h->s_thresh_opt; return MI355NDT_OK; }
  if (option == MI355NDT_OPT_STREAM_RESERVE) { *value = h->s_reserve_opt; return MI355NDT_OK; }
  if (option == MI355NDT_OPT_KF_FITNESS_CELL_MM) { *value = h->kff_cell_mm; return MI355NDT_OK; }
  if (option == MI355NDT_OPT_OUTLIER_CELL_MM) { *value = h->ol_cell_mm; return MI355NDT_OK; }
  if (option == MI355NDT_OPT_PREFILTER_GROUP) { *value = h->pf_group; return MI355NDT_OK; }
  return MI355NDT_ERR_BAD_ARG;
}
```

lv_slam_amd/csrc/ndt_host_profile.hpp:

```cpp
#pragma once

static hipError_t ev_take(mi355ndt_handle* h, hipEvent_t* e) {
  if (!h->ev_pool.empty()) { *e = h->ev_pool.back(); h->ev_pool.pop_back(); return hipSuccess; }
  return hipEventCreate(e);
}
static hipError_t ev_begin(mi355ndt_handle* h, std::vector<mi355ndt_handle::EvSpan>& v) {
  if (h->ev_last_fresh && h->ev_last) {
    v.push_back({h->ev_last, nullptr, true});
    h->ev_last_fresh = false;
    return hipSuccess;
  }
  hipEvent_t a;
  hipError_t e = ev_take(h, &a); if (e != hipSuccess) return e;
  v.push_back({a, nullptr, false});
  return hipEventRecord(a, h->stream);
}
static hipError_t ev_end(mi355ndt_handle* h, std::vector<mi355ndt_handle::EvSpan>& v) {
  hipEvent_t b;
  hipError_t e = ev_take(h, &b); if (e != hipSuccess) return e;
  v.back().second = b;
  h->ev_last = b;
  h->ev_last_fresh = true;
  return hipEventRecord(b, h->stream);
}
// ... 6 lines not shown
  }
  v.clear();
  h->ev_last_fresh = false;
}
int mi355ndt_profile_enable(mi355ndt_handle* h, int on) {
  if (!h) return MI355NDT_ERR_BAD_HANDLE;
  h->prof = on != 0;
  if (h->ss) for (int c = 0; c < h->ss->nctx; c++) if (h->ss->ctx[c].e) { h->ss->ctx[c].e->ev_pool_target = 128; (void)mi355ndt_profile_enable(h->ss->ctx[c].e.get(), on); }
  if (h->prof) {
    HIPCHK(h, hipSetDevice(h->device));
    while (h->ev_pool.size() < h->ev_pool_target) {
      hipEvent_t e;
      HIPCHK(h, hipEventCreate(&e));
      h->ev_pool.push_back(e);
    }
  }
  return MI355NDT_OK;
}
int mi355ndt_profile_reset(mi355ndt_handle* h) {
  if (!h) return MI355NDT_ERR_BAD_HANDLE;
  (void)hipSetDevice(h->device);
  (void)hipStreamSynchronize(h->stream);
  double d; long long n;
  ev_collect(h, h->ev_sweep, d, n); ev_collect(h, h->ev_update, d, n); ev_collect(h, h->ev_build, d, n);
  if (h->ss) for (int c = 0; c < h->ss->nctx; c++) if (mi355ndt_handle* e = h->ss->ctx[c].e.get()) {
    ev_collect(e, e->ev_sweep, d, n); ev_collect(e, e->ev_update, d, n); ev_collect(e, e->ev_build, d, n);
    e->P = mi355ndt_profile{};
  }
  h->P = mi355ndt_profile{};
  (void)hipMemsetAsync(h->d_hits, 0, 2 * sizeof(unsigned long long), h->stream);
  (void)hipStreamSynchronize(h->stream);
  return MI355NDT_OK;
}
int mi355ndt_profile_get(mi355ndt_handle* h, mi355ndt_profile* out) {
  if (!h) return MI355NDT_ERR_BAD_HANDLE;
  if (!out) return MI355NDT_ERR_BAD_ARG;
  HIPCHK(h, hipSetDevice(h->device));
  HIPCHK(h, hipStreamSynchronize(h->stream));
  ev_collect(h, h->ev_sweep, h->P.sweep_ms, h->P.sweep_launches);
  ev_collect(h, h->ev_update, h->P.update_ms, h->P.update_launches);
  ev_collect(h, h->ev_build, h->P.build_ms, h->P.build_launches);
  if (h->ss) for (int c = 0; c < h->ss->nctx; c++) if (mi355ndt_handle* e = h->ss->ctx[c].e.get()) {
    ev_collect(e, e->ev_sweep, h->P.sweep_ms, h->P.sweep_launches);
    ev_collect(e, e->ev_update, h->P.update_ms, h->P.update_launches);
    ev_collect(e, e->ev_build, h->P.build_ms, h->P.build_launches);
    h->P.build_alg_bytes += e->P.build_alg_bytes; e->P.build_alg_bytes = 0;
    { std::lock_guard<std::mutex> lk(e->up_mtx);
      h->P.cloud_uploads += e->P.cloud_uploads; e->P.cloud_uploads = 0; h->P.cloud_upload_bytes += e->P.cloud_upload_bytes; e->P.cloud_upload_bytes = 0;
      h->P.cloud_transfers += e->P.cloud_transfers; e->P.cloud_transfers = 0; }
  }
  unsigned long long hh[2] = {0, 0};
  HIPCHK(h, hipMemcpy(hh, h->d_hits, sizeof hh, hipMemcpyDeviceToHost));
  *out = h->P;
  if (h->ss) { out->stream_reserved_slots = h->ss->reserve_wg; out->stream_launch_slots = h->ss->launch_slots; }
  out->sweep_hits += (long long)hh[0];
  out->sweep_alg_bytes += 64.0 * (double)hh[0];
  out->score_only_sweeps = (long long)hh[1];
  return MI355NDT_OK;
}
```

lv_slam_amd/csrc/ndt_host_stream.hpp:

```cpp
#pragma once

static void stream_geometry(const StreamState& ss, mi355ndt_handle* e) {
  e->chunks_per_pair = ss.items / QUARTERS; e->rows_per_pair = e->items_per_pair = ss.items; e->pts_per_chunk = CHUNK_PTS; e->fine_it = 0;
}
static size_t stream_partials(const StreamState& ss) { return (size_t)ss.max_pairs * ss.items * NACC; }
static void stream_learn_plan(StreamState& ss, const mi355ndt_handle* e) {
  ss.plan_cb = std::max(ss.plan_cb, e->built.cb);
  ss.plan_words = std::max(ss.plan_words, e->built.total_words + e->built.total_words / 4 + 1024);
}
int mi355ndt_stream_end(mi355ndt_handle* h) {
  if (!h) return MI355NDT_ERR_BAD_HANDLE;
  if (!h->ss) return MI355NDT_OK;
  (void)hipSetDevice(h->device);
  StreamState& ss = *h->ss;
  if (ss.build_stream) (void)hipStreamSynchronize(ss.build_stream);
  (void)hipStreamSynchronize(h->stream);
  for (int c = 0; c < ss.nctx; c++) {
    mi355ndt_handle* e = ss.ctx[c].e.get();
    if (!e) continue;
    ev_collect(e, e->ev_sweep, h->P.sweep_ms, h->P.sweep_launches);
    ev_collect(e, e->ev_update, h->P.update_ms, h->P.update_launches);
    ev_collect(e, e->ev_build, h->P.build_ms, h->P.build_launches);
    h->P.build_alg_bytes += e->P.build_alg_bytes; e->P.build_alg_bytes = 0;
  }
  h->ss.reset();
  return MI355NDT_OK;
}

int mi355ndt_stream_begin(mi355ndt_handle* h, int n_contexts, int max_pairs, size_t max_tgt, size_t max_src) {
  if (!h) return MI355NDT_ERR_BAD_HANDLE;
  if (n_contexts < 2 || n_contexts > ASYNC_MAX_CTX || max_pairs < 1 || max_pairs > MAX_PAIRS || max_pairs >= (1 << ASYNC_CTX_SHIFT) ||
      max_tgt == 0 || max_src == 0 || max_tgt >= (1u << 31) || max_src >= (1u << 31)) return MI355NDT_ERR_BAD_ARG;
  if (h->ss) return MI355NDT_ERR_STATE;
  NOT_EULER(h, "mi355ndt_stream_begin");
  HIPCHK(h, hipSetDevice(h->device));
  HIPCHK(h, hipStreamSynchronize(h->stream));
  std::unique_ptr<StreamState> session(new StreamState());
  StreamState& ss = *session;
  ss.nctx = n_contexts; ss.max_pairs = max_pairs; ss.max_tgt = max_tgt; ss.max_src = max_src;
  ss.items = std::max(1, (int)((max_src + CHUNK_PTS - 1) / CHUNK_PTS)) * QUARTERS;
  ss.sync_only = !async_served(h);
  h->built = GridsBuilt{};
  SweepConst sc;
  make_sweep_const(h, sc);
  const int slots = launch_slots(h, sc, fast_served(h));
  {
    const int iu = ss.items / (sc.K == 1 ? ASYNC_CLAIM(1) : sc.K == 7 ? 2 : 1);
    const int waves = slots * WAVES;
    int t = h->s_thresh_opt >= 0 ? h->s_thresh_opt : 4 * ((waves + iu - 1) / std::max(1, iu));
    const char* env = std::getenv("MI355NDT_STREAM_THRESH");
    if (env) t = std::atoi(env);
    ss.thresh = std::max(0, std::min(t, ASYNC_MAX_CARRY));
    ss.thresh_given = h->s_thresh_opt >= 0 || env;
  }
  {
    const bool small_batch = (unsigned long long)max_pairs * (unsigned long long)max_tgt <= 768ull * 65536ull;
    int r = sc.K == 1 ? (max_tgt <= 98304 ? 128 : 96) : ((sc.K == 7 && small_batch) ? (sc.pca ? 32 : 64) : 0);
    if (const char* e = std::getenv("MI355NDT_STREAM_RESERVE")) r = std::atoi(e);
    if (h->s_reserve_opt >= 0) r = h->s_reserve_opt;
    r = std::max(0, std::min(r, slots / 2)) & ~7;
    if (n_contexts < 3) r = 0;
    ss.reserve_wg = r;
    ss.launch_slots = std::max(8, slots - r);
  }
  ss.ring_cap = async_ring_cap(h, (long long)max_pairs + ASYNC_MAX_CARRY);
  if (ss.ring_cap == 0) ss.sync_only = true;
  if (ss.d_stat.realloc_exact(ASYNC_MAX_CTX) != hipSuccess ||
      hipMemsetAsync(ss.d_stat, 0, ASYNC_MAX_CTX * sizeof(CtxStat), h->stream) != hipSuccess) return MI355NDT_ERR_HIP;
  for (int c = 0; c < n_contexts; c++) {
    StreamCtx& S = ss.ctx[c];
    mi355ndt_handle* e = nullptr;
    int rc = mi355ndt_create(&h->prm, h->device, &e);
    S.e.reset(e);
    if (rc) return rc;
    if (ss.reserve_wg > 0 && !ss.build_stream) {
      if (ss.build_stream.create() != hipSuccess) return MI355NDT_ERR_HIP;
      for (auto& ev : ss.ev_built) if (ev.create() != hipSuccess) return MI355NDT_ERR_HIP;
      for (auto& ev : ss.ev_launched) if (ev.create() != hipSuccess) return MI355NDT_ERR_HIP;
      for (auto& ev : ss.ev_prepared) if (ev.create() != hipSuccess) return MI355NDT_ERR_HIP;
      if (const char* pf = std::getenv("MI355NDT_STREAM_PREP_FIRST")) ss.prep_first = std::atoi(pf) != 0;
    }
    rc = mi355ndt_set_stream(e, ss.reserve_wg > 0 ? ss.build_stream : h->stream);
    if (rc) return rc;
    e->f32_sum_order = h->f32_sum_order; e->arith = h->arith; e->async_align = h->async_align; e->dyn_shift = h->dyn_shift; e->score_only_last = h->score_only_last;
    e->async_build = true;
    e->ev_pool_target = 128;
    rc = ensure_pair_arrays(e, max_pairs);
    if (rc) { h->err = e->err; return rc; }
    static_assert(sizeof(float) == sizeof(int), "the input block holds ints and floats");
    const size_t in_words = (size_t)max_pairs * (2 + 16);
    if (S.d_in.realloc_exact(in_words) != hipSuccess || S.h_in.realloc_exact(in_words, hipHostMallocMapped) != hipSuccess ||
        !(S.h_in_dev = (unsigned*)S.h_in.dev()) ||
        S.h_res.realloc_exact(max_pairs, hipHostMallocMapped | hipHostMallocCoherent) != hipSuccess ||
        !(S.d_res_map = S.h_res.dev())) { h->err = "stream_begin: allocation failed"; return MI355NDT_ERR_HIP; }
    e->d_tgt_cnt = S.d_in; e->d_src_cnt = S.d_in + max_pairs; e->d_guess = (float*)(S.d_in + 2 * (size_t)max_pairs);
    e->d_bstat = reinterpret_cast<unsigned*>(ss.d_stat + c);
    if (e->d_partials.reserve(stream_partials(ss)) != hipSuccess || e->d_arrived.reserve((size_t)max_pairs * ASYNC_ARR_STRIDE) != hipSuccess)
      { h->err = "stream_begin: allocation failed"; return MI355NDT_ERR_HIP; }
    if (h->prof) (void)mi355ndt_profile_enable(e, 1);
  }
  if (ss.d_ctl.realloc_exact(2) != hipSuccess || hipMemsetAsync(ss.d_ctl, 0, 2 * sizeof(AsyncCtl), h->stream) != hipSuccess ||
      ss.h_status.realloc_exact(StreamState::EV, hipHostMallocMapped | hipHostMallocCoherent) != hipSuccess ||
      !(ss.d_status = ss.h_status.dev())) return MI355NDT_ERR_HIP;
  memset((void*)ss.h_status.p, 0, StreamState::EV * sizeof(StreamStatus));
  if (h->d_atab.reserve(1) != hipSuccess) return MI355NDT_ERR_HIP;
  if (!ss.sync_only && ss.d_ring.realloc_exact((size_t)8 * ss.ring_cap) != hipSuccess) { (void)hipGetLastError(); ss.sync_only = true; }
  if (ss.build_stream) HIPCHK(h, hipStreamSynchronize(ss.build_stream));
  HIPCHK(h, hipStreamSynchronize(h->stream));
  h->ss = std::move(session);
  return MI355NDT_OK;
}

static int stream_launch(mi355ndt_handle* h, int new_ci, int n_new) {
  StreamState& ss = *h->ss;
  hipStream_t s = h->stream;
  SweepConst sc;
  make_sweep_const(h, sc);
  AsyncLaunch L;
  memset(&L.tab, 0, sizeof L.tab);
  const bool flush = new_ci < 0;
  for (int c = 0; c < ss.nctx; c++) {
    mi355ndt_handle* e = ss.ctx[c].e.get();
    if (!e->d_src) continue;
    fill_async_ctx(e, L.tab.c[c]);
    L.tab.c[c].results = ss.ctx[c].d_res_map;
    L.tab.c[c].n_done = &ss.d_stat[c].done;
    L.tab.c[c].pose = ss.ctx[c].busy ? ss.ctx[c].d_pose : nullptr; L.tab.c[c].pose_base = ss.ctx[c].pose_base; L.tab.c[c].pose_stride = ss.ctx[c].pose_stride;
    const int ahead = (ss.reserve_wg > 0 || ss.nctx >= 3) ? 2 : 1;
    bool mf = flush;
    for (int a = 1; a <= ahead; a++) mf = mf || c == (new_ci + a) % ss.nctx;
    L.tab.c[c].must_finish = mf ? 1 : 0;
  }
  const long long j = ss.launches;
  L.new_ci = flush ? 0 : new_ci; L.n_new = flush ? 0 : n_new;
  if (!flush) {
    mi355ndt_handle* e = ss.ctx[new_ci].e.get();
    L.st_new = e->d_state; L.guess_new = e->d_guess; L.src_cnt_new = e->d_src_cnt; L.gd_new = e->d_grid; L.arrived_new = e->d_arrived;
    L.active_list = e->d_active_list; L.sweep_ctl = nullptr; L.done_new = &ss.d_stat[new_ci].done;
    L.pose_new = ss.ctx[new_ci].d_pose; L.pose_cap = ss.ctx[new_ci].pose_cap;
  }
  L.tab_dev = h->d_atab; L.ring = ss.d_ring; L.ring_cap = ss.ring_cap;
  L.ctl = ss.d_ctl + (j & 1); L.prev = ss.drop_carry ? nullptr : ss.d_ctl + ((j + 1) & 1);
  L.items_per_pair = ss.items; L.stop_thresh = flush ? 0 : (ss.thresh_given ? ss.thresh : std::min(ss.thresh, n_new / 4)); L.debug_abort_pos = h->debug_abort_pos; L.debug_ring_mask = h->debug_ring_mask;
  L.reserve_wg = flush ? 0 : ss.reserve_wg;
  L.ev_prepared = (ss.reserve_wg > 0 && ss.prep_first) ? ss.ev_prepared[j % StreamState::EV] : nullptr;
  L.claim_items = (sc.K == 7 && L.stop_thresh > 0) ? 2 : 1;
  h->ev_last_fresh = false;
  if (!flush && ss.reserve_wg > 0) HIPCHK(h, hipStreamWaitEvent(s, ss.ev_built[new_ci], 0));
  L.stamp_end = (!flush && h->prof) ? &ss.d_status[j % StreamState::EV].build_t1 : nullptr;
  int rc = launch_async(h, sc, L);
  if (rc) return rc;
  ss.drop_carry = false;
  const int slot = (int)(j % StreamState::EV);
  k_stream_status<<<1, 64, 0, s>>>(L.ctl, ss.d_stat, reinterpret_cast<volatile unsigned*>(ss.d_status + slot), (unsigned)(j + 1));
  HIPCHK(h, hipGetLastError());
  if (ss.reserve_wg > 0) HIPCHK(h, hipEventRecord(ss.ev_launched[slot], s));
  ss.launches++;
  h->P.stream_launches++;
  return MI355NDT_OK;
}

static int stream_wait_launch(mi355ndt_handle* h, long long j) {
  StreamState& ss = *h->ss;
  volatile StreamStatus* st = ss.h_status + (j % StreamState::EV);
  const auto t0 = std::chrono::steady_clock::now();
  for (unsigned spins = 0; st->seq != (unsigned)(j + 1); spins++) {
    if ((spins & 1023) == 1023) {
      if (std::chrono::steady_clock::now() - t0 > std::chrono::seconds(60)) { h->err = "stream: the device stopped reporting"; return MI355NDT_ERR_STATE; }
      std::this_thread::yield();
    } else cpu_relax();
  }
  std::atomic_thread_fence(std::memory_order_acquire);
  for (; ss.counted <= j; ss.counted++) {
    volatile StreamStatus* c = ss.h_status + (ss.counted % StreamState::EV);
    h->P.stream_carried += c->susp;
    const unsigned long long b0 = c->build_t0, b1 = c->build_t1;
    if (b0 && b1 > b0) { h->P.build_ms += (double)(b1 - b0) * 1e-5; h->P.build_launches++; }
    c->build_t0 = 0; c->build_t1 = 0;
  }
  return MI355NDT_OK;
}

static int stream_run_sync(mi355ndt_handle* h, StreamCtx& S) {
  StreamState& ss = *h->ss;
  mi355ndt_handle* e = S.e.get();
  if (ss.build_stream) HIPCHK(h, hipStreamSynchronize(ss.build_stream));
  HIPCHK(h, hipStreamSynchronize(h->stream));
  e->async_build = false; e->counts_preloaded = false;
  e->up_tgt_cnt.clear(); e->up_src_cnt.clear();
  int rc = mi355ndt_batch_build_targets(e);
  if (rc == MI355NDT_OK) rc = mi355ndt_batch_align(e, S.guesses.data(), S.h_res);
  e->async_build = true;
  if (rc) { h->err = e->err; return rc; }
  stream_learn_plan(ss, e);
  stream_geometry(ss, e);
  if (e->d_partials.reserve(stream_partials(ss)) != hipSuccess) return MI355NDT_ERR_HIP;
  return MI355NDT_OK;
}

int mi355ndt_stream_submit(mi355ndt_handle* h, int n_pairs, const float* d_t, const int* tc, size_t tp, const float* d_s, const int* scnt, size_t sp,
                           const float* guesses, long long* batch_id) {
  if (!h) return MI355NDT_ERR_BAD_HANDLE;
  if (!h->ss) return MI355NDT_ERR_STATE;
  StreamState& ss = *h->ss;
  if (n_pairs < 1 || n_pairs > ss.max_pairs || !guesses || !batch_id || !tc || !scnt) return MI355NDT_ERR_BAD_ARG;
// ... 172 lines not shown
```

lv_slam_amd/csrc/ndt_host_sweep.hpp:

```cpp
#pragma once

constexpr int SWEEP_IT_BATCH = 8;
constexpr bool euler_sweep_exists(int K, int ord) { return (K == 1 || K == 7 || K == 26 || K == 27) && (ord == 0 || ord == 1); }
constexpr bool sweep_exists(bool pca, int K, int ord, int it) {
  if ((K != 1 && K != 7 && K != 26 && K != 27) || (pca && K == 27)) return false;
  if (ord < 0 || ord > 2 || (it != SWEEP_IT_BATCH && it != 1 && it != 2)) return false;
  return (K == 1 || K == 7) || (ord != 2 && it == SWEEP_IT_BATCH);
}
template <int N> using IC = std::integral_constant<int, N>;
template <class F>
static int dispatch_sweep(bool pca, int K, int ord, int it, F&& f) {
  int rc = MI355NDT_ERR_UNSUPPORTED;
  auto one = [&](auto P, auto KK, auto O, auto IT) {
    if constexpr (sweep_exists(decltype(P)::value, decltype(KK)::value, decltype(O)::value, decltype(IT)::value))
      if (pca == decltype(P)::value && K == decltype(KK)::value && ord == decltype(O)::value && it == decltype(IT)::value) rc = f(P, KK, O, IT);
  };
  auto by_it = [&](auto P, auto KK, auto O) { one(P, KK, O, IC<SWEEP_IT_BATCH>{}); one(P, KK, O, IC<1>{}); one(P, KK, O, IC<2>{}); };
  auto by_ord = [&](auto P, auto KK) { by_it(P, KK, IC<0>{}); by_it(P, KK, IC<1>{}); by_it(P, KK, IC<2>{}); };
  auto by_K = [&](auto P) { by_ord(P, IC<1>{}); by_ord(P, IC<7>{}); by_ord(P, IC<26>{}); by_ord(P, IC<27>{}); };
  by_K(std::false_type{}); by_K(std::true_type{});
  return rc;
}

static int prep_align_ws(mi355ndt_handle* h) {
  const int B = h->n_pairs;
  int maxn = 0;
  for (int b = 0; b < B; b++) maxn = std::max(maxn, h->h_src_cnt[b]);
  h->chunks_per_pair = std::max(1, (maxn + CHUNK_PTS - 1) / CHUNK_PTS);
  {
    const bool fine_served = sweep_exists(false, neighbor_K(h->prm.neighbor_mode), 0, h->fine_tiles);
    const bool small = h->seq_running || (long long)B * h->chunks_per_pair * QUARTERS < 4LL * h->n_cu * WAVES;
    h->fine_it = (h->latency_mode && fine_served && !mt_is_live(h->prm) && small && model_leaves_rounds(h->pose_model, h->ndt_class)) ? h->fine_tiles : 0;
  }
  if (eff_model(h) == POSE_MODEL_EULER) HIPCHK(h, h->d_euler_rows.reserve((size_t)B * EULER_ROW_WORDS));
  if (h->ndt_class == NDT_CLASS_PCL) HIPCHK(h, h->d_pcl_rows.reserve((size_t)B * EULER_ROW_WORDS));
  if (h->fine_it) {
    const int item_pts = h->fine_it * 64;
    h->pts_per_chunk = 4 * item_pts;
    h->rows_per_pair = std::max(1, (maxn + h->pts_per_chunk - 1) / h->pts_per_chunk);
    h->items_per_pair = 4 * h->rows_per_pair;
  } else {
    h->rows_per_pair = h->chunks_per_pair * QUARTERS;
    h->items_per_pair = h->rows_per_pair;
    h->pts_per_chunk = CHUNK_PTS;
  }
  size_t need = (size_t)B * std::max(h->rows_per_pair, h->chunks_per_pair * QUARTERS) * NACC;
  HIPCHK(h, h->d_partials.reserve(need));
  if (h->up_src_cnt.size() != (size_t)B || !std::equal(h->up_src_cnt.begin(), h->up_src_cnt.end(), h->h_src_cnt.begin())) {
    HIPCHK(h, hipMemcpyAsync(h->d_src_cnt, h->h_src_cnt.data(), B * sizeof(int), hipMemcpyHostToDevice, h->stream));
    HIPCHK(h, hipStreamSynchronize(h->stream));
    h->up_src_cnt.assign(h->h_src_cnt.begin(), h->h_src_cnt.begin() + B);
  }
  return MI355NDT_OK;
}

static void make_sweep_const(const mi355ndt_handle* h, SweepConst& sc) {
  double d1, d2;
  gauss_constants(h->prm, d1, d2);
  sc.d1 = d1;
  sc.d2f = (float)d2;
  sc.pca = h->prm.variant == MI355NDT_VARIANT_PCA;
  const float leaf = (h->built.valid && h->built.leaf > 0.f) ? h->built.leaf : h->prm.resolution;
  { int ex; float mant = std::frexp(leaf, &ex); sc.leaf_pow2 = (mant == 0.5f) && ex > -100 && ex < 100; sc.inv_leaf = 1.0f / leaf; }
  sc.kd_r2 = (float)((double)h->prm.resolution * (double)h->prm.resolution);
  build_offsets(class_neighbor_mode(h->ndt_class, h->prm.neighbor_mode), sc);
  sc.dyn_shift = h->dyn_shift >= 0 ? h->dyn_shift : (sc.K == 1 ? 3 : 2);
  sc.host_flags = nullptr;
  sc.seq_no = 0;
  sc.rebase_block = 0;
  sc.d1f = (float)d1;
  sc.kq = (float)(-0.5 * (double)sc.d2f * 1.4426950408889634);
  sc.euler_rows = euler_rows_of(h);
  sc.pcl_rows = pcl_rows_of(h);
  sc.icov64 = h->d_icov64.p;
  sc.d2 = d2;
// ... 32 lines not shown
    const long long items = (long long)(max_pairs > 0 ? max_pairs : h->n_pairs) * h->items_per_pair;
    grid.x = (unsigned)std::max(1LL, std::min((long long)grid.x, (items + WAVES - 1) / WAVES));
    if (sc.rebase_block) grid.x += 1;
  }
  if (h->ndt_class == NDT_CLASS_PCL) {
    if (sc.pca || h->fine_it || sc.K != 27 || !sc.pcl_rows || !sc.icov64 || !h->built.made.icov64 || !h->built.made.cent) {
      h->err = "no sweep kernel serves this configuration under MI355NDT_OPT_NDT_CLASS = 1";
      return MI355NDT_ERR_UNSUPPORTED;
    }
    k_sweep<false, 27, SWEEP_IT_BATCH, false, 0, 2><<<grid, SWEEP_THREADS, 0, h->stream>>>(h->d_src, h->src_pitch, h->d_state, h->d_grid, h->d_words, h->d_recs, h->d_partials,
                                                                                           h->items_per_pair, h->d_active_list, ctl, ctl_next, sc, h->d_cent, h->d_grid_of_use);
  } else if (h->pose_model == POSE_MODEL_EULER) {
    const int rc = launch_sweep_euler(h, sc, ord, grid, ctl, ctl_next);
    if (rc) { h->err = "no sweep kernel serves this configuration under MI355NDT_OPT_POSE_MODEL = 1"; return rc; }
  } else if (!h->fine_it && sc.pca && sc.K == 27) {
    const dim3 kdgrid((unsigned)h->chunks_per_pair, (unsigned)h->n_pairs);
    auto kd = ord == 1 ? k_sweep_pca_kd<1> : k_sweep_pca_kd<0>;
    kd<<<kdgrid, SWEEP_THREADS, 0, h->stream>>>(h->d_src, h->src_pitch, h->d_state, h->d_grid, h->d_words, h->d_recs, h->d_cent, h->d_kdw, h->d_partials,
                                                h->chunks_per_pair, h->d_active_list, ctl, ctl_next, sc);
  } else {
    const int rc = dispatch_sweep(sc.pca != 0, sc.K, ord, h->fine_it ? h->fine_it : SWEEP_IT_BATCH, [&](auto P, auto KK, auto O, auto IT) {
      constexpr int it = decltype(IT)::value;
      k_sweep<decltype(P)::value, decltype(KK)::value, it, it != SWEEP_IT_BATCH, decltype(O)::value><<<grid, SWEEP_THREADS, 0, h->stream>>>(
          h->d_src, h->src_pitch, h->d_state, h->d_grid, h->d_words, sweep_recs(h, sc), h->d_partials, h->items_per_pair, h->d_active_list, ctl, ctl_next, sc,
          h->d_cent, h->d_grid_of_use);
      return MI355NDT_OK;
    });
    if (rc) { h->err = "no sweep kernel serves this configuration"; return rc; }
  }
  h->ctl_idx ^= 1;
  if (h->prof) HIPCHK(h, ev_end(h, h->ev_sweep));
  return MI355NDT_OK;
}

static void launch_hessian(mi355ndt_handle* h, const SweepConst& sc) {
  double gc[3] = {0, 0, 0};
  gauss_constants(h->prm, gc[0], gc[1]);
  k_hessian<<<dim3((unsigned)h->chunks_per_pair, (unsigned)h->n_pairs), HESS_THREADS, 0, h->stream>>>(
      h->d_src, h->src_pitch, h->d_state, h->d_grid, h->d_words, h->d_recs, h->d_icov64, h->d_cent, h->d_partials, h->chunks_per_pair,
      gc[0], gc[1], sc.kd_r2, sc.leaf_pow2, sc.inv_leaf);
}


struct AsyncLaunch {
  AsyncTab tab;
  int new_ci = 0, n_new = 0;
  PairState* st_new = nullptr; const float* guess_new = nullptr; const int* src_cnt_new = nullptr; const GridDesc* gd_new = nullptr; unsigned* arrived_new = nullptr;
  int* active_list = nullptr; SweepCtl* sweep_ctl = nullptr; unsigned* done_new = nullptr; PoseRecord* pose_new = nullptr; int pose_cap = 0;
  AsyncTab* tab_dev = nullptr; int* ring = nullptr; int ring_cap = 0; AsyncCtl* ctl = nullptr; const AsyncCtl* prev = nullptr;
  int items_per_pair = 0, stop_thresh = 0; unsigned debug_abort_pos = 0xFFFFFFFFu, debug_ring_mask = 0xFFu;
  unsigned long long* stamp_end = nullptr;
  int claim_items = 1;
  int reserve_wg = 0;
  hipEvent_t ev_prepared = nullptr;
};
#define NDT_CTX_ARGS(i) L.tab.c[i].src, L.tab.c[i].pitch, L.tab.c[i].st, L.tab.c[i].gd, L.tab.c[i].words, L.tab.c[i].recs, L.tab.c[i].partials, L.tab.c[i].src_cnt, \
                        L.tab.c[i].arrived, L.tab.c[i].cent
template <bool PCA, int K, int ORD>
static int launch_async_t(mi355ndt_handle* h, const SweepConst& sc, const AsyncLaunch& L) {
  auto kern = k_align_async<PCA, K, ORD>;
  static std::atomic<int> per_cu_of_device[64];
  int per_cu = per_cu_of_device[h->device & 63].load(std::memory_order_relaxed);
  if (per_cu == 0) {
    if (hipOccupancyMaxActiveBlocksPerMultiprocessor(&per_cu, kern, SWEEP_THREADS, 0) != hipSuccess) { (void)hipGetLastError(); return MI355NDT_ERR_UNSUPPORTED; }
    per_cu_of_device[h->device & 63].store(per_cu, std::memory_order_relaxed);
  }
  const int slots = launch_slots(h, sc, ORD == 2);
  if (per_cu * h->n_cu < slots || slots < 8) return MI355NDT_ERR_UNSUPPORTED;
  dim3 grid((unsigned)std::max(8, slots - L.reserve_wg));
  kern<<<grid, SWEEP_THREADS, 0, h->stream>>>(L.tab_dev, L.items_per_pair, L.ring, L.ring_cap, L.ctl, sc, h->prof ? h->d_hits : nullptr,
                                             h->prm.step_size, h->prm.trans_epsilon, h->prm.max_iterations, L.stop_thresh, L.debug_abort_pos, L.debug_ring_mask, L.claim_items,
                                             NDT_CTX_ARGS(0), NDT_CTX_ARGS(1), NDT_CTX_ARGS(2), NDT_CTX_ARGS(3));
  return MI355NDT_OK;
}
static int launch_async(mi355ndt_handle* h, const SweepConst& sc, const AsyncLaunch& L) {
  hipStream_t s = h->stream;
  {
    const size_t n = std::max(std::max(std::max((size_t)8 * L.ring_cap, (size_t)L.n_new * ASYNC_ARR_STRIDE), sizeof(AsyncCtl) / sizeof(unsigned)), (size_t)L.pose_cap);
    k_async_prepare<<<(unsigned)((n + 255) / 256), 256, 0, s>>>(L.tab, L.tab_dev, L.new_ci, L.n_new, L.st_new, L.guess_new, L.src_cnt_new, L.gd_new, L.arrived_new,
                                                               L.active_list, L.sweep_ctl, L.ring, L.ring_cap, L.ctl, L.prev, L.done_new, L.pose_new, L.pose_cap, L.stamp_end);
    if (L.ev_prepared) HIPCHK(h, hipEventRecord(L.ev_prepared, s));
  }
  if (h->prof) HIPCHK(h, ev_begin(h, h->ev_sweep));
  const int rc = dispatch_sweep(sc.pca != 0, sc.K, sweep_ord(h, sc), SWEEP_IT_BATCH, [&](auto P, auto KK, auto O, auto) {
    return launch_async_t<decltype(P)::value, decltype(KK)::value, decltype(O)::value>(h, sc, L);
  });
  if (h->prof) HIPCHK(h, ev_end(h, h->ev_sweep));
  return rc;
}
static int async_ring_cap(const mi355ndt_handle* h, long long pairs) {
  const long long cap = (pairs * ((long long)h->prm.max_iterations + 4) + 7) / 8 + 1;
  return cap > (1LL << 26) ? 0 : (int)cap;
}
static void fill_async_ctx(const mi355ndt_handle* e, AsyncCtx& c) {
  SweepConst sc;
  make_sweep_const(e, sc);
  c.src = e->d_src; c.pitch = e->src_pitch; c.st = e->d_state; c.gd = e->d_grid; c.words = e->d_words; c.recs = sweep_recs(e, sc); c.cent = e->d_cent;
  c.partials = e->d_partials; c.src_cnt = e->d_src_cnt; c.arrived = e->d_arrived; c.results = e->d_results; c.n_done = nullptr; c.must_finish = 1; c.pose = nullptr; c.pose_base = 0; c.pose_stride = 0; c.score_only = e->score_only_last;
}
```

lv_slam_amd/csrc/ndt_ord1_list.hpp:

```cpp
#pragma once
#define NDT_SWEEP_ARGS_T (const float*, size_t, const PairState*, const GridDesc*, const BitWord*, const VoxelRec*, double*, int, const int*, SweepCtl*, SweepCtl*, \
                          SweepConst, const float*, const int*)
#define NDT_KD_ARGS_T (const float*, size_t, const PairState*, const GridDesc*, const BitWord*, const VoxelRec*, const float*, const int*, double*, int, const int*, \
                       SweepCtl*, SweepCtl*, SweepConst)
#define NDT_CTX_T const float*, size_t, PairState*, const GridDesc*, const BitWord*, const VoxelRec*, double*, const int*, unsigned*, const float*
#define NDT_ASYNC_ARGS_T (const AsyncTab*, int, int*, int, AsyncCtl*, SweepConst, unsigned long long*, double, double, int, int, unsigned, unsigned, int, NDT_CTX_T, NDT_CTX_T, NDT_CTX_T, NDT_CTX_T)
#define NDT_ORD1_KERNELS(X)                                                                                   \
  X __global__ void k_sweep<false, 1, 8, false, 1> NDT_SWEEP_ARGS_T;  X __global__ void k_sweep<true, 1, 8, false, 1> NDT_SWEEP_ARGS_T;   \
  X __global__ void k_sweep<false, 7, 8, false, 1> NDT_SWEEP_ARGS_T;  X __global__ void k_sweep<true, 7, 8, false, 1> NDT_SWEEP_ARGS_T;   \
  X __global__ void k_sweep<false, 26, 8, false, 1> NDT_SWEEP_ARGS_T; X __global__ void k_sweep<true, 26, 8, false, 1> NDT_SWEEP_ARGS_T;  \
  X __global__ void k_sweep<false, 27, 8, false, 1> NDT_SWEEP_ARGS_T;                                                                      \
  X __global__ void k_sweep<false, 1, 8, false, 1, 1> NDT_SWEEP_ARGS_T;  X __global__ void k_sweep<false, 7, 8, false, 1, 1> NDT_SWEEP_ARGS_T;   \
  X __global__ void k_sweep<false, 26, 8, false, 1, 1> NDT_SWEEP_ARGS_T; X __global__ void k_sweep<false, 27, 8, false, 1, 1> NDT_SWEEP_ARGS_T; \
  X __global__ void k_sweep<false, 1, 1, true, 1> NDT_SWEEP_ARGS_T;   X __global__ void k_sweep<true, 1, 1, true, 1> NDT_SWEEP_ARGS_T;    \
  X __global__ void k_sweep<false, 1, 2, true, 1> NDT_SWEEP_ARGS_T;   X __global__ void k_sweep<true, 1, 2, true, 1> NDT_SWEEP_ARGS_T;    \
  X __global__ void k_sweep<false, 7, 1, true, 1> NDT_SWEEP_ARGS_T;   X __global__ void k_sweep<true, 7, 1, true, 1> NDT_SWEEP_ARGS_T;    \
  X __global__ void k_sweep<false, 7, 2, true, 1> NDT_SWEEP_ARGS_T;   X __global__ void k_sweep<true, 7, 2, true, 1> NDT_SWEEP_ARGS_T;    \
  X __global__ void k_sweep_pca_kd<1> NDT_KD_ARGS_T;                                                                                       \
  X __global__ void k_align_async<false, 1, 1> NDT_ASYNC_ARGS_T;  X __global__ void k_align_async<true, 1, 1> NDT_ASYNC_ARGS_T;           \
  X __global__ void k_align_async<false, 7, 1> NDT_ASYNC_ARGS_T;  X __global__ void k_align_async<true, 7, 1> NDT_ASYNC_ARGS_T;           \
  X __global__ void k_align_async<false, 26, 1> NDT_ASYNC_ARGS_T; X __global__ void k_align_async<true, 26, 1> NDT_ASYNC_ARGS_T;          \
  X __global__ void k_align_async<false, 27, 1> NDT_ASYNC_ARGS_T;
```

lv_slam_amd/csrc/ndt_sweep.hpp:

```cpp
#pragma once
#include "ndt_types.hpp"
#include "ndt_math.hpp"
#include "ndt_newton.hpp"
#include <type_traits>

struct NoHook { __device__ __forceinline__ void operator()() const {} };

template <int ORD>
__device__ __forceinline__ float sum3(float t0, float t1, float t2) { return ORD == 1 ? (t0 + t2) + t1 : (t0 + t1) + t2; }

template <int ORD>
__device__ __forceinline__ bool eval_prefix(const float u[3], const float C[9], const double d1, const float d2f, const bool ok_in,
                                            const double* __restrict__ exp_tab, float y[3], float& e1, float& s_inc) {
#pragma unroll
  for (int j = 0; j < 3; j++) y[j] = sum3<ORD>(u[0] * C[j], u[1] * C[3 + j], u[2] * C[6 + j]);
  const float qf = sum3<ORD>(u[0] * y[0], u[1] * y[1], u[2] * y[2]);
  const float e0 = ndtm::exp_f32arg((-d2f * qf) * 0.5f, exp_tab);
  s_inc = (float)(-d1 * (double)e0);
  e1 = d2f * e0;
  const bool ok = ok_in && !(e1 > 1.f || e1 < 0.f || e1 != e1);
  s_inc = ok ? s_inc : 0.f;
  return ok;
}

// ... 305 lines not shown
  const int o26[26][3] = {{-1,-1,-1}, {-1,0,-1}, {-1,1,-1}, {0,-1,-1}, {0,0,-1}, {0,1,-1}, {1,-1,-1}, {1,0,-1}, {1,1,-1}, {-1,-1,0}, {0,-1,0}, {1,-1,0}, {-1,0,0}, {1,1,1}, {1,0,1}, {1,-1,1}, {0,1,1}, {0,0,1}, {0,-1,1}, {-1,1,1}, {-1,0,1}, {-1,-1,1}, {1,1,0}, {0,1,0}, {-1,1,0}, {1,0,0}};
  return K == 1 ? 0 : (K == 7 ? o7[q][a] : (K == 26 ? o26[q][a] : (a == 0 ? q % 3 - 1 : (a == 1 ? (q / 3) % 3 - 1 : q / 9 - 1))));
}

#define Q_GROUP 7
#define ID_BITS 23
#define WAVES   (SWEEP_THREADS / 64)

#ifdef NDT_TIMELINE
__device__ unsigned long long g_tl[16];
struct Timeline {
  unsigned long long t[16], last;
  __device__ __forceinline__ Timeline() { for (int k = 0; k < 16; k++) t[k] = 0; last = __builtin_readcyclecounter(); }
  __device__ __forceinline__ void stamp(const int k) {
    __builtin_amdgcn_sched_barrier(0);
    const unsigned long long t_ = __builtin_readcyclecounter();
    t[k] += t_ - last; last = t_;
    __builtin_amdgcn_sched_barrier(0);
  }
  __device__ __forceinline__ void count(const int k = 7) { t[k] += 1; }
  __device__ __forceinline__ void restart() { last = __builtin_readcyclecounter(); }
  __device__ __forceinline__ void flush(const int k0, const int k1) const { if ((threadIdx.x & 63) == 0) for (int k = k0; k < k1; k++) atomicAdd(&g_tl[k], t[k]); }
};
#else
struct Timeline {
  __device__ __forceinline__ void stamp(int) {}
  __device__ __forceinline__ void count(int = 7) {}
  __device__ __forceinline__ void restart() {}
  __device__ __forceinline__ void flush(int, int) const {}
};
#endif
#define TL_STAMP(k) tl.stamp(k)
struct SweepCtl {
  int n_active;
  int next_item[8];
};
#define QUARTERS WAVES

#ifndef FAST_WPE7
#define FAST_WPE7 4
#endif
#ifndef FAST_WPE1
#define FAST_WPE1 3
#endif
#ifndef FAST_TP7
#define FAST_TP7 1
#endif
#ifndef FAST_TP1
#define FAST_TP1 2
#endif
#ifndef FAST_PIPE
#define FAST_PIPE 1
#endif
template <bool PCA, int K, int ORD = 0>
struct SweepTune {
  static constexpr bool FAST = (ORD == 2);
  static constexpr int  WPE  = FAST ? (K == 1 ? FAST_WPE1 : FAST_WPE7) : SWEEP_WPE;
  static constexpr bool PIPE = FAST ? (FAST_PIPE != 0) : true;
  static constexpr int  TP   = FAST ? (K == 1 ? FAST_TP1 : FAST_TP7) : (K == 1 ? 8 : (K <= 7 ? 2 : 1));
};
static inline int sweep_wpe(int K, bool fast = false) { return fast ? (K == 1 ? FAST_WPE1 : FAST_WPE7) : SWEEP_WPE; }

#define POSE_W_LAST 21
__device__ __forceinline__ unsigned sweep_pose_words(const PairState* S) {
  static_assert(offsetof(PairState, T) == 0 && offsetof(PairState, Rj) == 48 && offsetof(PairState, last_sweep) == 4 * POSE_W_LAST, "pose words");
  const int lane = threadIdx.x & 63;
  unsigned w = 0;
  if (lane <= POSE_W_LAST) w = __hip_atomic_load((const gu32*)reinterpret_cast<const unsigned*>(S) + lane, RLX_AGENT);
  return w;
}

__device__ __forceinline__ void pose_from_words(const unsigned pose_w, float T[12], float Rj[9]) {
#pragma unroll
  for (int a = 0; a < 12; a++) T[a] = __uint_as_float(__builtin_amdgcn_readlane(pose_w, a));
#pragma unroll
  for (int a = 0; a < 9; a++) Rj[a] = __uint_as_float(__builtin_amdgcn_readlane(pose_w, 12 + a));
}

__device__ __forceinline__ void score_row_store(const double lane_score, double* P, const unsigned nhits, const int lane) {
  const double v = score_tree(lane_score);
  if (lane == 0) {
    gu64* PG = (gu64*)reinterpret_cast<unsigned long long*>(P);
    __hip_atomic_store(PG, (unsigned long long)__double_as_longlong(v), RLX_AGENT);
    __hip_atomic_store(PG + 43, (unsigned long long)__double_as_longlong((double)nhits), RLX_AGENT);
  }
}

template <bool AGENT>
__device__ __forceinline__ void wave_row_store(const double row[43], double* P, const unsigned nhits, const int lane) {
  typedef unsigned int u2v __attribute__((ext_vector_type(2)));
  double P1[22], P2[11];
#pragma unroll
  for (int i = 0; i < 22; i++) {
    const double a = row[i], b2 = (i + 22 < 43) ? row[i + 22] : 0.0;
    const u2v lo = __builtin_amdgcn_permlane32_swap((unsigned)__double2loint(a), (unsigned)__double2loint(b2), false, false);
    const u2v hi = __builtin_amdgcn_permlane32_swap((unsigned)__double2hiint(a), (unsigned)__double2hiint(b2), false, false);
    P1[i] = __hiloint2double((int)hi.x, (int)lo.x) + __hiloint2double((int)hi.y, (int)lo.y);
  }
#pragma unroll
  for (int i = 0; i < 11; i++) {
    const double a = P1[i], b2 = P1[i + 11];
    const u2v lo = __builtin_amdgcn_permlane16_swap((unsigned)__double2loint(a), (unsigned)__double2loint(b2), false, false);
    const u2v hi = __builtin_amdgcn_permlane16_swap((unsigned)__double2hiint(a), (unsigned)__double2hiint(b2), false, false);
    double v = __hiloint2double((int)hi.x, (int)lo.x) + __hiloint2double((int)hi.y, (int)lo.y);
#pragma unroll
    for (int o = 8; o > 0; o >>= 1) v += __shfl_xor(v, o);
    P2[i] = v;
  }
  if ((lane & 15) == 0) {
    const int row4 = lane >> 4, base = 11 * (row4 & 1) + 22 * (row4 >> 1);
    if (AGENT) {
      gu64* PG = (gu64*)reinterpret_cast<unsigned long long*>(P);
#pragma unroll
      for (int i = 0; i < 11; i++) if (base + i < 43) __hip_atomic_store(PG + base + i, (unsigned long long)__double_as_longlong(P2[i]), RLX_AGENT);
      if (lane == 0) __hip_atomic_store(PG + 43, (unsigned long long)__double_as_longlong((double)nhits), RLX_AGENT);
    } else {
#pragma unroll
      for (int i = 0; i < 11; i++) if (base + i < 43) P[base + i] = P2[i];
      if (lane == 0) P[43] = (double)nhits;
    }
  }
}

__device__ __forceinline__ void move_axis(const float* Ta, const float* Ra, const float px, const float py, const float pz, float& xt, float& r) {
  xt = ((Ta[0] * px + Ta[1] * py) + Ta[2] * pz) + Ta[3];
  r = (Ra[0] * px + Ra[1] * py) + Ra[2] * pz;
}
__device__ __forceinline__ void stage_point(float* sp, const float xt[3], const float r[3]) {
  sp[0] = xt[0]; sp[1] = xt[1]; sp[2] = xt[2]; sp[3] = r[0]; sp[4] = r[1]; sp[5] = r[2];
}
__device__ __forceinline__ void rel_cell(const float xt[3], const SweepConst& sc, const float leaf, const int mb0, const int mb1, const int mb2,
                                         int& r0, int& r1, int& r2) {
  const int c0 = (int)floorf(sc.leaf_pow2 ? xt[0] * sc.inv_leaf : xt[0] / leaf);
  const int c1 = (int)floorf(sc.leaf_pow2 ? xt[1] * sc.inv_leaf : xt[1] / leaf);
  const int c2 = (int)floorf(sc.leaf_pow2 ? xt[2] * sc.inv_leaf : xt[2] / leaf);
  r0 = c0 - mb0; r1 = c1 - mb1; r2 = c2 - mb2;
}
__device__ __forceinline__ bool bitmap_rank(const uint4 bw, const unsigned cell, unsigned& id) {
  const unsigned long long bits = ((unsigned long long)bw.y << 32) | bw.x;
  const unsigned long long tb = bits << (63u - (cell & 63u));
  id = bw.z + (unsigned)__popcll(tb) - 1u;
  return (long long)tb < 0;
}

template <typename T, int SLOT>
__device__ __forceinline__ T& item_lds() { __shared__ T v; return v; }

struct BatchX { unsigned slot; double m0, m1, m2; float C[9]; int weight; double w; };
struct BatchF { unsigned slot; float mh[3], ml[3], c[6]; int weight; float w; };
struct BatchD { unsigned slot; double m0, m1, m2; double C[9]; };
struct NoRows {};
template <bool PCA, int K, int ORD, bool SO, int Q_CAP, bool W_LATE = false, int PM = 0>
struct HitQueue {
  static_assert(PM == 0 || ((PM == 1 || PM == 2) && !PCA && ORD != 2 && !SO), "the Euler model: ndt_omp, exact arithmetic, full rows");
  static_assert(PM != 2 || (K == 27 && ORD == 0), "PCL's class: the radius search, one instantiation");
  typename std::conditional<PM == 1, EulerRows, typename std::conditional<PM == 2, PclCtx, NoRows>::type>::type rw;
  static constexpr bool KD = (K == 27), FAST = (ORD == 2), PCAQ = PCA && K > 1;
  static constexpr int NA = FAST ? NACC_F : 43;
  typedef typename std::conditional<FAST, float, double>::type AccT;
  typedef typename std::conditional<K == 1, int, AccT>::type QW;
  typedef typename std::conditional<FAST, BatchF, typename std::conditional<PM == 2, BatchD, BatchX>::type>::type Batch;
  unsigned* const ent; QW* const qw; const float (*const stage)[6];
  const VoxelRec* const R; const SweepConst& sc; const double* const exp_tab;
  const int lane; const unsigned long long lt_mask;
  AccT (&acc)[NA];
  unsigned nhits;
  int head, count;
  int old;
  __device__ __forceinline__ HitQueue(AccT (&acc_)[NA], unsigned* ent_, QW* qw_, const float (*stage_)[6], const VoxelRec* R_, const SweepConst& sc_, const double* exp_tab_, const int lane_)
      : ent(ent_), qw(qw_), stage(stage_), R(R_), sc(sc_), exp_tab(exp_tab_), lane(lane_), lt_mask((1ull << lane_) - 1ull), acc(acc_), head(0), count(0), old(0) { new_row(); }
  __device__ __forceinline__ void new_row() {
#pragma unroll
    for (int a = 0; a < NA; a++) acc[a] = (AccT)0;
    nhits = 0;
  }
  __device__ __forceinline__ void push(const bool hit, const unsigned slot, const unsigned id, const double w) {
    const unsigned long long mask = __ballot(hit);
    if (hit) {
      const int pos = (head + count + (int)__popcll(mask & lt_mask)) & (Q_CAP - 1);
      ent[pos] = (slot << ID_BITS) | id;
      if (PCAQ) qw[pos] = (QW)w;
    }
    count += (int)__popcll(mask);
  }
  __device__ __forceinline__ void fetch(const int off, const int m, Batch& B) const {
    const int k = lane < m ? lane : m - 1;
    const unsigned e = ent[(head + off + k) & (Q_CAP - 1)];
    B.slot = e >> ID_BITS;
    if constexpr (FAST) {
      const VoxelRecF& vr = reinterpret_cast<const VoxelRecF*>(R)[e & ((1u << ID_BITS) - 1)];
#pragma unroll
      for (int a = 0; a < 3; a++) { B.mh[a] = vr.mh[a]; B.ml[a] = vr.ml[a]; }
#pragma unroll
      for (int a = 0; a < 6; a++) B.c[a] = vr.c[a];
      B.weight = vr.weight;
      if (!W_LATE) B.w = 1.f;
      if (PCAQ) B.w = (float)qw[(head + off + k) & (Q_CAP - 1)];
      else if (PCA && !W_LATE) B.w = (float)vr.weight;
    } else if constexpr (PM == 2) {
      const unsigned id = e & ((1u << ID_BITS) - 1);
      const VoxelRec& vr = R[id];
      B.m0 = vr.mean[0]; B.m1 = vr.mean[1]; B.m2 = vr.mean[2];
#pragma unroll
      for (int a = 0; a < 9; a++) B.C[a] = rw.icov64[(size_t)id * 9 + a];
    } else {
      const VoxelRec& vr = R[e & ((1u << ID_BITS) - 1)];
      B.m0 = vr.mean[0]; B.m1 = vr.mean[1]; B.m2 = vr.mean[2];
#pragma unroll
      for (int a = 0; a < 9; a++) B.C[a] = vr.icov[a];
      B.weight = vr.weight;
      if (!W_LATE) B.w = 1.0;
      if (PCAQ) B.w = (double)qw[(head + off + k) & (Q_CAP - 1)];
      else if (PCA && !W_LATE) B.w = (double)vr.weight;
    }
  }
  template <typename Mid>
  __device__ __forceinline__ void eval_batch(const Batch& B, const int m, Mid mid) {
    const float* sp = stage[B.slot];
    const float xt0 = sp[0], xt1 = sp[1], xt2 = sp[2];
    float r[3] = {sp[3], sp[4], sp[5]};
    bool live = lane < m;
    if constexpr (PM != 2) live = live && (PCAQ || KD || B.weight != VOX_DEAD);
    if constexpr (PM == 2) {
      const double u[3] = {(double)xt0 - B.m0, (double)xt1 - B.m1, (double)xt2 - B.m2};
      eval_hit_pcl<Mid>(u, r, B.C, rw.rows, sc.d1, sc.d2, live, acc, mid);
    } else if constexpr (FAST) {
      float u[3] = {(xt0 - B.mh[0]) - B.ml[0], (xt1 - B.mh[1]) - B.ml[1], (xt2 - B.mh[2]) - B.ml[2]};
      const float w = (W_LATE && !PCAQ) ? (PCA ? (float)B.weight : 1.f) : B.w;
      if constexpr (SO) { mid(); eval_score_fast<PCA>(u, B.c, sc.d1f, sc.d2f, sc.kq, w, live, acc[0]); }
      else eval_hit_fast<PCA, Mid>(u, r, B.c, sc.d1f, sc.d2f, sc.kq, w, live, acc, mid);
    } else {
      float u[3] = {(float)((double)xt0 - B.m0), (float)((double)xt1 - B.m1), (float)((double)xt2 - B.m2)};
      const double w = (W_LATE && !PCAQ) ? (PCA ? (double)B.weight : 1.0) : B.w;
      if constexpr (SO) { mid(); eval_score<PCA, ORD>(u, B.C, sc.d1, sc.d2f, w, live, acc[0], exp_tab); }
      else if constexpr (PM == 1) eval_hit_euler<Mid, KD, ORD>(u, r, B.C, rw, sc.d1, sc.d2f, live, acc, exp_tab, mid);
      else eval_hit<PCA, Mid, KD, ORD>(u, r, B.C, sc.d1, sc.d2f, w, live, acc, exp_tab, mid);
    }
    nhits += PCAQ ? (unsigned)m : (unsigned)__popcll(__ballot(live));
    head = (head + m) & (Q_CAP - 1);
    count -= m;
    old = old > m ? old - m : 0;
  }
  __device__ __forceinline__ void drain(const int m) {
    Batch B;
    fetch(0, m, B);
    eval_batch(B, m, NoHook());
  }
  __device__ __forceinline__ void drain_full() {
    if (PM == 2 || !SweepTune<PCA, K, ORD>::PIPE) {
      while (count >= 64) drain(64);
      return;
    }
    if (count < 64) return;
    Batch A;
    fetch(0, 64, A);
#pragma unroll 1
    for (;;) {
      const bool more = count >= 128;
      Batch N;
      eval_batch(A, 64, [&]() { if (more) fetch(64, 64, N); });
      if (!more) break;
      A = N;
    }
  }
};

template <bool PCA, int K, int IT, bool FINE, int ORD, bool ASYNC, bool SO = false, int PM = 0>
__device__ __forceinline__ void sweep_item(const int b, const int rem, const float* __restrict__ src, const size_t pitch, const PairState* st,
                                           const GridDesc* __restrict__ gd, const BitWord* __restrict__ words, const VoxelRec* __restrict__ recs,
                                           double* partials, const int rows_per_pair, const SweepConst& sc, const float* __restrict__ cent,
                                           const int* __restrict__ grid_of, const double* exp_tab,
                                           const unsigned pose_w, const int n_async, const int g_async,
                                           Timeline& tl) {
  constexpr bool KD = (K == 27);
  constexpr bool FAST = (ORD == 2);
  static_assert(!SO || (ASYNC && !FINE), "score-only items belong to the one-launch align");
  static_assert(!FAST || K == 1 || K == 7, "tolerance arithmetic is instantiated for DIRECT1 / DIRECT7");
  static_assert(PM == 0 || (!PCA && !FAST && !ASYNC && !FINE && !SO), "the Euler model takes the lockstep rounds: ndt_omp, exact arithmetic, batch items");
  static_assert(PM != 2 || (K == 27 && ORD == 0 && IT == 8), "PCL's class: the radius search, batch items");
  typedef SweepTune<PCA, K, ORD> Tune;
  const int lane = threadIdx.x & 63, wv = threadIdx.x >> 6;
  constexpr bool PCAQ = PCA && K > 1;
  constexpr int TP = Tune::TP < IT ? Tune::TP : IT;
  constexpr int Q_NEED = (IT / TP > 1 ? 64 : 0) + TP * (K < Q_GROUP ? K : Q_GROUP) * 64;
  constexpr int Q_CAP = FAST ? (Q_NEED <= 128 ? 128 : Q_NEED <= 256 ? 256 : Q_NEED <= 512 ? 512 : 1024) : ((K > 1 && K <= Q_GROUP) ? 1024 : 512);
  static_assert(Q_NEED <= Q_CAP, "hit queue");
  typedef HitQueue<PCA, K, ORD, SO, Q_CAP, false, PM> Queue;
  auto& q_ent = item_lds<unsigned[WAVES][Q_CAP], 0>();
  auto& q_w = item_lds<typename Queue::QW[PCAQ ? WAVES : 1][PCAQ ? Q_CAP : 1], 1>();
  constexpr int NBUF = (IT / TP > 1) ? 2 : 1;
  auto& stage = item_lds<float[WAVES][NBUF * 64 * TP][6], 2>();

  auto& red = item_lds<double[FINE ? WAVES : 1][FINE ? NACC : 1], 3>();
  const PairState& S = st[b];
  const int n = ASYNC ? n_async : S.n_src;
  const GridDesc& g = gd[ASYNC ? g_async : (grid_of ? grid_of[b] : b)];
  const float* X = src + (size_t)b * 3 * pitch;
  const BitWord* W = words + g.word_off;
  const VoxelRec* R = recs + g.rec_off;
  const bool grid_ok = (g.status == GRID_OK);
  float T[12], Rj[9];
  if constexpr (ASYNC) pose_from_words(pose_w, T, Rj);
  else {
#pragma unroll
    for (int a = 0; a < 12; a++) T[a] = S.T[a];
#pragma unroll
    for (int a = 0; a < 9; a++) Rj[a] = PM != 0 ? 0.f : S.Rj[a];
  }
  const float leaf = g.leaf;
  const int mb0 = g.min_b[0], mb1 = g.min_b[1], mb2 = g.min_b[2];
  const int xb0 = g.max_b[0], xb1 = g.max_b[1], xb2 = g.max_b[2];
  const int mul1 = g.mul1, mul2 = g.mul2, nwords = g.nwords;
  {
    typename Queue::AccT acc[Queue::NA];
    Queue Q(acc, q_ent[wv], q_w[PCAQ ? wv : 0], stage[wv], R, sc, exp_tab, lane);
    if constexpr (PM == 1) Q.rw = euler_rows_of_pair(sc.euler_rows, b);
    if constexpr (PM == 2) { Q.rw.rows = pcl_rows_of_pair(sc.pcl_rows, b); Q.rw.icov64 = sc.icov64 + (size_t)g.rec_off * 9; }
    const int wbase = rem * (IT * 64);
    if (wbase < n && grid_ok) {
      constexpr int NST = IT / TP;
      const unsigned e0 = (unsigned)(xb0 - mb0), e1 = (unsigned)(xb1 - mb1), e2 = (unsigned)(xb2 - mb2);
      const unsigned empty_cell = (unsigned)(nwords - 1) << 6;
      float nx[TP], ny[TP], nz[TP];
#pragma unroll
      for (int p = 0; p < TP; p++) {
        const int i = wbase + p * 64 + lane;
        nx[p] = ny[p] = nz[p] = 0.f;
        if (i < n) { nx[p] = X[i]; ny[p] = X[pitch + i]; nz[p] = X[2 * pitch + i]; }
      }
      TL_STAMP(1);
#pragma unroll 1
      for (int st = 0; st < NST; st++) {
        if (wbase + st * TP * 64 >= n) break;
        if (Q.old > 0) { __builtin_amdgcn_wave_barrier(); Q.drain(Q.old); }
        Q.old = Q.count;
        int r0[TP], r1[TP], r2[TP], cc[TP];
        bool valid[TP];
        float kx[TP], ky[TP], kz[TP];
#pragma unroll
        for (int p = 0; p < TP; p++) {
          const int i = wbase + (st * TP + p) * 64 + lane;
          const float px = nx[p], py = ny[p], pz = nz[p];
          const int inext = i + TP * 64;
          if (st + 1 < NST && inext < n) { nx[p] = X[inext]; ny[p] = X[pitch + inext]; nz[p] = X[2 * pitch + inext]; }
          bool ok = i < n && finite3(px, py, pz);
          float xt[3], r[3];
#pragma unroll
          for (int a = 0; a < 3; a++) move_axis(T + 4 * a, Rj + 3 * a, px, py, pz, xt[a], r[a]);
          ok = ok && finite3(xt[0], xt[1], xt[2]);
          if constexpr (PM != 0) { const float xo[3] = {px, py, pz}; stage_point(stage[wv][((st & 1) * TP + p) * 64 + lane], xt, xo); }
          else stage_point(stage[wv][((st & 1) * TP + p) * 64 + lane], xt, r);
          kx[p] = xt[0]; ky[p] = xt[1]; kz[p] = xt[2];
          rel_cell(xt, sc, leaf, mb0, mb1, mb2, r0[p], r1[p], r2[p]);
          cc[p] = r0[p] + r1[p] * mul1 + r2[p] * mul2;
          valid[p] = ok;
        }
        TL_STAMP(2);
        double suf[TP];
#pragma unroll
        for (int p = 0; p < TP; p++) suf[p] = 1.0;
#pragma unroll
        for (int q1 = K; q1 > 0; q1 -= Q_GROUP) {
          unsigned cellv[TP][Q_GROUP];
          uint4 bwv[TP][Q_GROUP];
#pragma unroll
          for (int p = 0; p < TP; p++) {
#pragma unroll
            for (int j = 0; j < Q_GROUP; j++) {
              const int q = q1 - 1 - j;
              if (q < 0) continue;
              const int o0 = probe_off(K, q, 0), o1 = probe_off(K, q, 1), o2 = probe_off(K, q, 2);
              const bool inside = valid[p] && (unsigned)(r0[p] + o0) <= e0 && (unsigned)(r1[p] + o1) <= e1 && (unsigned)(r2[p] + o2) <= e2;
              cellv[p][j] = inside ? (unsigned)(cc[p] + o0 + o1 * mul1 + o2 * mul2) : empty_cell;
              bwv[p][j] = *reinterpret_cast<const uint4*>(W + (cellv[p][j] >> 6));
            }
          }
          TL_STAMP(3);
          unsigned idv[TP][Q_GROUP];
          int wiv[TP][Q_GROUP];
#pragma unroll
          for (int p = 0; p < TP; p++) {
#pragma unroll
            for (int j = 0; j < Q_GROUP; j++) {
              if (q1 - 1 - j < 0) continue;
              const bool occ = bitmap_rank(bwv[p][j], cellv[p][j], idv[p][j]);
              wiv[p][j] = occ ? 1 : VOX_DEAD;
              if (PCAQ) { if (occ) wiv[p][j] = R[idv[p][j]].weight; }
              if (KD && occ) {
                const float* cp = cent + 3 * (size_t)(g.rec_off + idv[p][j]);
                const float dx = kx[p] - cp[0], dy = ky[p] - cp[1], dz = kz[p] - cp[2];
                if (!(((dx * dx + dy * dy) + dz * dz) < sc.kd_r2)) wiv[p][j] = VOX_DEAD;
              }
            }
          }
#pragma unroll
          for (int p = 0; p < TP; p++) {
            const int slot = ((st & 1) * TP + p) * 64 + lane;
#pragma unroll
            for (int j = 0; j < Q_GROUP; j++) {
              if (q1 - 1 - j < 0) continue;
              const bool hit = wiv[p][j] != VOX_DEAD;
              if (PCAQ && hit) suf[p] *= (double)wiv[p][j];
              Q.push(hit, (unsigned)slot, idv[p][j], suf[p]);
            }
          }
          __builtin_amdgcn_wave_barrier();
          TL_STAMP(4);
          Q.drain_full();
          TL_STAMP(5);
        }
      }
      __builtin_amdgcn_wave_barrier();
      if (Q.count > 0) Q.drain(Q.count);
      TL_STAMP(5);
    }
    double* P = FINE ? &red[FINE ? wv : 0][0] : partials + ((size_t)b * rows_per_pair + rem) * NACC;
    if constexpr (SO) score_row_store((double)Q.acc[0], P, Q.nhits, lane);
    else if constexpr (FAST) {
      double accd[43];
      fast_acc_to_row(Q.acc, accd);
      wave_row_store<ASYNC && !FINE>(accd, P, Q.nhits, lane);
    } else wave_row_store<ASYNC && !FINE>(Q.acc, P, Q.nhits, lane);
    if (FINE) {
      __syncthreads();
      if (wv == 0 && lane < NACC)
        partials[((size_t)b * (rows_per_pair >> 2) + (rem >> 2)) * NACC + lane] = ((red[0][lane] + red[FINE ? 1 : 0][lane]) + red[FINE ? 2 : 0][lane]) + red[FINE ? 3 : 0][lane];
      __syncthreads();
    }
    TL_STAMP(6);
    tl.count();
  }
}

template <bool PCA, int ORD, int NROWS, bool SO = false>
__device__ __forceinline__ void sweep_rows_d1(const int b, const int rem0, const float* __restrict__ src, const size_t pitch,
                                              const GridDesc* __restrict__ gd, const BitWord* __restrict__ words, const VoxelRec* __restrict__ recs,
                                              double* partials, const int rows_per_pair, const SweepConst& sc, const double* exp_tab,
                                              const unsigned pose_w, const int n, const int g_idx, Timeline& tl) {
  constexpr int TP = 2, IT = 8, NST = IT / TP, Q_CAP = 512;
  const int lane = threadIdx.x & 63, wv = threadIdx.x >> 6;
  auto& q_ent = item_lds<unsigned[WAVES][Q_CAP], 4>();
  auto& stage = item_lds<float[WAVES][64 * IT][6], 5>();
  const GridDesc& g = gd[g_idx];
  const float* X = src + (size_t)b * 3 * pitch;
  const BitWord* W = words + g.word_off;
  const VoxelRec* R = recs + g.rec_off;
  const bool grid_ok = (g.status == GRID_OK);
  float T[12], Rj[9];
  pose_from_words(pose_w, T, Rj);
  const float leaf = g.leaf;
  const int mb0 = g.min_b[0], mb1 = g.min_b[1], mb2 = g.min_b[2];
  const unsigned e0 = (unsigned)(g.max_b[0] - mb0), e1 = (unsigned)(g.max_b[1] - mb1), e2 = (unsigned)(g.max_b[2] - mb2);
  const int mul1 = g.mul1, mul2 = g.mul2;
  const int base = rem0 * (IT * 64);
  constexpr int S_TOTAL = NROWS * NST;

  double acc[43];
  HitQueue<PCA, 1, ORD, SO, Q_CAP, true> Q(acc, q_ent[wv], nullptr, stage[wv], R, sc, exp_tab, lane);

  float nx[TP], ny[TP], nz[TP];
  uint4 bw[TP];
  unsigned cellv[TP];
  auto load_points = [&](const int s) {
#pragma unroll
// ... 138 lines not shown
```

lv_slam_amd/ndt.py:

```python
from __future__ import annotations

import ctypes as C
import math
import os
import numpy as np

_HERE = os.path.dirname(os.path.abspath(__file__))
LIB_PATH = os.environ.get("MI355NDT_LIB") or os.path.join(_HERE, "libmi355ndt.so")

KDTREE, DIRECT26, DIRECT7, DIRECT1 = 0, 1, 2, 3
VARIANT_OMP, VARIANT_PCA = 0, 1

OK = 0
ERR = {-1: "bad handle", -2: "bad argument", -3: "HIP error", -4: "target grid unusable", -5: "no HIP device",
       -6: "unsupported configuration", -7: "target/source not set"}


class NDTError(RuntimeError):
    def __init__(self, code, where, detail=""):
        self.code = code
        super().__init__(f"{where}: {ERR.get(code, code)}" + (f" ({detail})" if detail else ""))


class Params(C.Structure):
    _fields_ = [("resolution", C.c_float), ("step_size", C.c_double), ("outlier_ratio", C.c_double),
                ("trans_epsilon", C.c_double), ("max_iterations", C.c_int), ("neighbor_mode", C.c_int),
                ("variant", C.c_int), ("min_points_per_voxel", C.c_int), ("min_covar_eigvalue_mult", C.c_double)]


class Result(C.Structure):
    _fields_ = [("final_colmajor", C.c_float * 16), ("trans_probability", C.c_double), ("score", C.c_double),
                ("iterations", C.c_int), ("converged", C.c_int), ("sweeps", C.c_int), ("status", C.c_int),
                ("hits_last", C.c_longlong)]


class Voxel(C.Structure):
    _fields_ = [("idx", C.c_int32), ("n", C.c_int32), ("mean", C.c_double * 3), ("icov", C.c_float * 9),
                ("weight", C.c_int32)]


class Profile(C.Structure):
    _fields_ = [("sweep_ms", C.c_double), ("sweep_launches", C.c_longlong), ("sweep_alg_bytes", C.c_double),
                ("sweep_hits", C.c_longlong), ("sweep_points", C.c_longlong), ("build_ms", C.c_double),
                ("build_launches", C.c_longlong), ("build_alg_bytes", C.c_double), ("update_ms", C.c_double),
                ("update_launches", C.c_longlong), ("async_fallbacks", C.c_longlong), ("stream_launches", C.c_longlong),
                ("stream_carried", C.c_longlong), ("stream_redone", C.c_longlong), ("cloud_uploads", C.c_longlong), ("cloud_upload_bytes", C.c_longlong),
                ("cloud_transfers", C.c_longlong), ("cloud_promotions", C.c_longlong),
                ("stream_reserved_slots", C.c_longlong), ("stream_launch_slots", C.c_longlong), ("score_only_sweeps", C.c_longlong)]


class InfParams(C.Structure):
    _fields_ = [("use_const_inf_matrix", C.c_int), ("const_stddev_x", C.c_double), ("const_stddev_q", C.c_double), ("var_gain_a", C.c_double),
                ("min_stddev_x", C.c_double), ("max_stddev_x", C.c_double), ("min_stddev_q", C.c_double), ("max_stddev_q", C.c_double),
                ("fitness_score_thresh", C.c_double)]


class OutlierParams(C.Structure):
    _fields_ = [("method", C.c_int), ("mean_k", C.c_int), ("stddev_mul", C.c_double), ("radius", C.c_double), ("min_neighbors", C.c_int)]


class OutlierStats(C.Structure):
    _fields_ = [("n_in", C.c_longlong), ("n_valid", C.c_longlong), ("mean", C.c_double), ("stddev", C.c_double), ("threshold", C.c_double)]


class GicpParams(C.Structure):
    _fields_ = [("k_correspondences", C.c_int), ("gicp_epsilon", C.c_double), ("rotation_epsilon", C.c_double), ("transformation_epsilon", C.c_double),
                ("max_iterations", C.c_int), ("max_inner_iterations", C.c_int), ("corr_dist_threshold", C.c_double)]


class GicpResult(C.Structure):
    _fields_ = [("final_colmajor", C.c_float * 16), ("converged", C.c_int), ("iterations", C.c_int), ("inner_status", C.c_int), ("n_matched", C.c_int),
                ("delta", C.c_double)]


class IcpParams(C.Structure):
    _fields_ = [("transformation_epsilon", C.c_double), ("max_iterations", C.c_int), ("euclidean_fitness_epsilon", C.c_double),
                ("corr_dist_threshold", C.c_double), ("min_number_correspondences", C.c_int), ("use_reciprocal_correspondences", C.c_int)]


class IcpResult(C.Structure):
    _fields_ = [("final_colmajor", C.c_float * 16), ("converged", C.c_int), ("iterations", C.c_int), ("state", C.c_int), ("matches", C.c_int),
                ("mse", C.c_double)]


class PrefilterParams(C.Structure):
    _fields_ = [("use_distance_filter", C.c_int), ("extended", C.c_int), ("distance_near", C.c_double), ("distance_far", C.c_double),
                ("downsample_resolution", C.c_float), ("use_transform", C.c_int), ("transform_colmajor", C.c_float * 16)]


class PrefilterParamsEx(C.Structure):
    _fields_ = [("base", PrefilterParams), ("downsample_method", C.c_int), ("use_angle_calibration", C.c_int), ("angle_calibration_rad", C.c_double)]


class SeqParams(C.Structure):
    _fields_ = [("keyframe_delta_trans", C.c_double), ("keyframe_delta_angle", C.c_double), ("keyframe_delta_time", C.c_double)]


class SeqFrame(C.Structure):
    _fields_ = [("odom_colmajor", C.c_double * 16), ("tf_s2k_colmajor", C.c_float * 16), ("trans_probability", C.c_double),
                ("dx", C.c_double), ("da", C.c_double), ("dt", C.c_double), ("key_id", C.c_int), ("new_keyframe", C.c_int),
                ("iterations", C.c_int), ("converged", C.c_int), ("aligns", C.c_int), ("pad", C.c_int)]


class SeqStats(C.Structure):
    _fields_ = [("upload_ms", C.c_double), ("build_ms", C.c_double), ("track_ms", C.c_double), ("aligns", C.c_longlong),
                ("update_launches", C.c_longlong)]


SYMBOLS = [
    "mi355ndt_version", "mi355ndt_device_count", "mi355ndt_host_numa_node", "mi355ndt_default_params", "mi355ndt_create", "mi355ndt_destroy",
    "mi355ndt_set_params", "mi355ndt_get_params", "mi355ndt_set_stream", "mi355ndt_last_error",
    "mi355ndt_set_target", "mi355ndt_set_source", "mi355ndt_promote_source_to_target", "mi355ndt_align", "mi355ndt_get_aligned", "mi355ndt_get_incremental",
    "mi355ndt_get_fitness_score", "mi355ndt_fitness_score_T", "mi355ndt_prefilter", "mi355ndt_use_prefiltered", "mi355ndt_derivatives", "mi355ndt_compute_hessian", "mi355ndt_derivatives_T", "mi355ndt_get_grid", "mi355ndt_get_voxels",
    "mi355ndt_batch_reserve", "mi355ndt_batch_set_target", "mi355ndt_batch_set_source", "mi355ndt_batch_set_clouds", "mi355ndt_batch_bind_device",
    "mi355ndt_batch_build_targets", "mi355ndt_batch_align", "mi355ndt_batch_size", "mi355ndt_batch_pose_records", "mi355ndt_batch_fitness_scores",
    "mi355ndt_profile_enable", "mi355ndt_profile_reset", "mi355ndt_profile_get", "mi355ndt_synchronize",
    "mi355ndt_set_latency_mode", "mi355ndt_sequence_run",
    "mi355ndt_calculate_score", "mi355ndt_convert_transform", "mi355ndt_set_option", "mi355ndt_get_option",
    "mi355ndt_stream_begin", "mi355ndt_stream_submit", "mi355ndt_stream_submit_host", "mi355ndt_stream_collect", "mi355ndt_stream_end", "mi355ndt_stream_pose_records", "mi355ndt_pack_pose_records",
    "mi355ndt_map_cloud",
    "mi355ndt_window_keyframe", "mi355ndt_keyframe_add", "mi355ndt_keyframe_get", "mi355ndt_keyframe_release", "mi355ndt_keyframe_count",
    "mi355ndt_map_cloud_keyframes", "mi355ndt_batch_set_target_keyframe", "mi355ndt_batch_set_source_keyframe",
    "mi355ndt_keyframe_fitness_scores", "mi355ndt_inf_params_default", "mi355ndt_information_matrix",
    "mi355ndt_outlier_params_default", "mi355ndt_prefilter_outliers", "mi355ndt_batch_remove_outliers", "mi355ndt_sequence_run_raw_outliers",
    "mi355ndt_prefilter_params_default", "mi355ndt_batch_prefilter", "mi355ndt_batch_get_cloud", "mi355ndt_sequence_run_raw",
    "mi355ndt_prefilter_p", "mi355ndt_prefilter_params_ex_default",
    "mi355ndt_gicp_params_default", "mi355ndt_gicp_set_params", "mi355ndt_gicp_set_target", "mi355ndt_gicp_set_source", "mi355ndt_gicp_set_target_keyframe",
    "mi355ndt_gicp_set_source_keyframe", "mi355ndt_gicp_covariances", "mi355ndt_gicp_correspondences", "mi355ndt_gicp_cost", "mi355ndt_gicp_align",
    "mi355ndt_gicp_get_aligned",
    "mi355ndt_gicp_batch_reserve", "mi355ndt_gicp_batch_set_source", "mi355ndt_gicp_batch_set_source_keyframe", "mi355ndt_gicp_batch_align",
    "mi355ndt_gicp_batch_get_aligned", "mi355ndt_gicp_batch_stats",
    "mi355ndt_icp_params_default", "mi355ndt_icp_set_params", "mi355ndt_icp_set_target", "mi355ndt_icp_set_source", "mi355ndt_icp_set_target_keyframe",
    "mi355ndt_icp_set_source_keyframe", "mi355ndt_icp_correspondences", "mi355ndt_icp_align", "mi355ndt_icp_get_aligned",
    "mi355ndt_icp_batch_reserve", "mi355ndt_icp_batch_set_source", "mi355ndt_icp_batch_set_source_keyframe", "mi355ndt_icp_batch_align",
    "mi355ndt_icp_batch_get_aligned", "mi355ndt_icp_batch_stats",
]
ICP_BATCH_MAX = 64
ICP_STATES = ["NOT_CONVERGED", "ITERATIONS", "TRANSFORM", "ABS_MSE", "REL_MSE", "NO_CORRESPONDENCES"]
GICP_BATCH_MAX = 64
GICP_TARGET, GICP_SOURCE = 0, 1
OPT_ASYNC_ALIGN = 2
OPT_DEBUG_ASYNC_ABORT = 3
OPT_DEBUG_ASYNC_RINGS = 6
OPT_STREAM_RESERVE = 5
OPT_STREAM_THRESHOLD = 4
WARN_TOLERANCE_ARITH = 1
OPT_ARITH = 7
OPT_F32_SUM_ORDER = 1
OPT_SCORE_ONLY_LAST_SWEEP = 8
OPT_KF_FITNESS_CELL_MM = 9
OPT_OUTLIER_CELL_MM = 10
OPT_PREFILTER_GROUP = 11
OPT_POSE_MODEL = 12
POSE_MODELS = {"se3": 0, "euler": 1}
OPT_NDT_CLASS = 13
NDT_CLASSES = {"omp": 0, "pcl": 1}
PREFILTER_EXTENDED = 0x50467832
DOWNSAMPLE_VOXELGRID = 0
DOWNSAMPLE_APPROX_VOXELGRID = 1
ANGLE_CALIBRATION_RAD = 0.11 * math.pi / 180
OUTLIER_STATISTICAL = 1
OUTLIER_RADIUS = 2

_LIB = None


def load_library(path: str = LIB_PATH):
    global _LIB
    if _LIB is not None:
        return _LIB
    if not os.path.exists(path):
        raise ImportError(f"{path} not found: build it with `python -c 'import __graft_entry__ as g; g.build()'` "
                          "(hipcc --offload-arch=gfx950).  There is no CPU fallback.")
    L = C.CDLL(path)
    vp, i, sz = C.c_void_p, C.c_int, C.c_size_t
    L.mi355ndt_version.restype = C.c_char_p
    L.mi355ndt_last_error.restype = C.c_char_p
    L.mi355ndt_last_error.argtypes = [vp]
    L.mi355ndt_default_params.argtypes = [C.POINTER(Params)]
    L.mi355ndt_host_numa_node.argtypes = [i]
    L.mi355ndt_create.argtypes = [C.POINTER(Params), i, C.POINTER(vp)]
    L.mi355ndt_destroy.argtypes = [vp]
    L.mi355ndt_set_params.argtypes = [vp, C.POINTER(Params)]
    L.mi355ndt_get_params.argtypes = [vp, C.POINTER(Params)]
    L.mi355ndt_set_stream.argtypes = [vp, vp]
    L.mi355ndt_set_target.argtypes = [vp, vp, sz, sz]
    L.mi355ndt_set_source.argtypes = [vp, vp, sz, sz]
    L.mi355ndt_promote_source_to_target.argtypes = [vp]
    L.mi355ndt_align.argtypes = [vp, vp, C.POINTER(Result)]
    L.mi355ndt_get_aligned.argtypes = [vp, vp, sz]
    L.mi355ndt_get_incremental.argtypes = [vp, i, vp, vp]
    L.mi355ndt_get_fitness_score.argtypes = [vp, C.c_double, vp, vp]
    L.mi355ndt_fitness_score_T.argtypes = [vp, vp, C.c_double, vp, vp]
    L.mi355ndt_prefilter.argtypes = [vp, vp, sz, sz, i, C.c_double, C.c_double, C.c_float, vp, sz, sz, C.POINTER(sz)]
    L.mi355ndt_use_prefiltered.argtypes = [vp, i]
    L.mi355ndt_outlier_params_default.argtypes = [C.POINTER(OutlierParams)]
    L.mi355ndt_prefilter_outliers.argtypes = [vp, C.POINTER(OutlierParams), vp, vp, sz, sz, C.POINTER(sz), C.POINTER(OutlierStats)]
    L.mi355ndt_batch_remove_outliers.argtypes = [vp, i, i, i, C.POINTER(OutlierParams), vp, vp, vp, vp]
    L.mi355ndt_sequence_run_raw_outliers.argtypes = [vp, i, vp, vp, sz, vp, C.POINTER(PrefilterParams), C.POINTER(OutlierParams), C.POINTER(SeqParams), vp, vp,
                                                     C.POINTER(SeqStats), vp, vp]
    L.mi355ndt_prefilter_params_default.argtypes = [C.POINTER(PrefilterParams)]
    L.mi355ndt_prefilter_params_ex_default.argtypes = [C.POINTER(PrefilterParamsEx)]
    L.mi355ndt_prefilter_p.argtypes = [vp, vp, sz, sz, C.POINTER(PrefilterParams), vp, sz, sz, C.POINTER(sz)]
    L.mi355ndt_batch_prefilter.argtypes = [vp, i, i, vp, vp, vp, vp, sz, C.POINTER(PrefilterParams), vp, vp]
    L.mi355ndt_batch_get_cloud.argtypes = [vp, i, i, vp, sz, sz, C.POINTER(sz)]
    L.mi355ndt_sequence_run_raw.argtypes = [vp, i, vp, vp, sz, vp, C.POINTER(PrefilterParams), C.POINTER(SeqParams), vp, vp, C.POINTER(SeqStats), vp, vp]
    L.mi355ndt_gicp_params_default.argtypes = [C.POINTER(GicpParams)]
    L.mi355ndt_gicp_set_params.argtypes = [vp, C.POINTER(GicpParams)]
    L.mi355ndt_gicp_set_target.argtypes = [vp, vp, sz, sz]
    L.mi355ndt_gicp_set_source.argtypes = [vp, vp, sz, sz]
    L.mi355ndt_gicp_set_target_keyframe.argtypes = [vp, i]
    L.mi355ndt_gicp_set_source_keyframe.argtypes = [vp, i]
    L.mi355ndt_gicp_covariances.argtypes = [vp, i, vp, sz]
    L.mi355ndt_gicp_correspondences.argtypes = [vp, vp, vp, vp, vp, C.POINTER(i)]
    L.mi355ndt_gicp_cost.argtypes = [vp, vp, vp, C.POINTER(C.c_double), vp]
    L.mi355ndt_gicp_align.argtypes = [vp, vp, C.POINTER(GicpResult)]
    L.mi355ndt_gicp_get_aligned.argtypes = [vp, vp, sz]
    L.mi355ndt_gicp_batch_reserve.argtypes = [vp, i]
    L.mi355ndt_gicp_batch_set_source.argtypes = [vp, i, vp, sz, sz]
    L.mi355ndt_gicp_batch_set_source_keyframe.argtypes = [vp, i, i]
    L.mi355ndt_gicp_batch_align.argtypes = [vp, vp, vp]
    L.mi355ndt_gicp_batch_get_aligned.argtypes = [vp, i, vp, sz]
    L.mi355ndt_gicp_batch_stats.argtypes = [vp, C.POINTER(i), vp]
    L.mi355ndt_icp_params_default.argtypes = [C.POINTER(IcpParams)]
    L.mi355ndt_icp_set_params.argtypes = [vp, C.POINTER(IcpParams)]
    L.mi355ndt_icp_set_target.argtypes = [vp, vp, sz, sz]
    L.mi355ndt_icp_set_source.argtypes = [vp, vp, sz, sz]
    L.mi355ndt_icp_set_target_keyframe.argtypes = [vp, i]
    L.mi355ndt_icp_set_source_keyframe.argtypes = [vp, i]
    L.mi355ndt_icp_correspondences.argtypes = [vp, vp, vp, vp, vp, vp, C.POINTER(i)]
    L.mi355ndt_icp_align.argtypes = [vp, vp, C.POINTER(IcpResult)]
    L.mi355ndt_icp_get_aligned.argtypes = [vp, vp, sz]
    L.mi355ndt_icp_batch_reserve.argtypes = [vp, i]
    L.mi355ndt_icp_batch_set_source.argtypes = [vp, i, vp, sz, sz]
    L.mi355ndt_icp_batch_set_source_keyframe.argtypes = [vp, i, i]
    L.mi355ndt_icp_batch_align.argtypes = [vp, vp, vp]
    L.mi355ndt_icp_batch_get_aligned.argtypes = [vp, i, vp, sz]
    L.mi355ndt_icp_batch_stats.argtypes = [vp, C.POINTER(i), vp]
    L.mi355ndt_map_cloud.argtypes = [vp, i, vp, vp, sz, vp, C.c_double, vp, sz, sz, C.POINTER(sz)]
    L.mi355ndt_window_keyframe.argtypes = [vp, i, vp, vp, sz, i, vp, C.c_float, C.POINTER(i), C.POINTER(sz)]
    L.mi355ndt_keyframe_add.argtypes = [vp, vp, sz, sz, i, C.POINTER(i)]
    L.mi355ndt_keyframe_get.argtypes = [vp, i, vp, sz, sz, i, C.POINTER(sz)]
    L.mi355ndt_keyframe_release.argtypes = [vp, i]
    L.mi355ndt_keyframe_count.argtypes = [vp]
# ... 189 lines not shown
        self._icp_n = [0, 0]
        self._icp_batch_n = []

    def close(self):
        if getattr(self, "h", None):
            self.lib.mi355ndt_destroy(self.h)
            self.h = None

    __del__ = close

    def _chk(self, rc, where):
        if rc != OK:
            raise NDTError(rc, where, (self.lib.mi355ndt_last_error(self.h) or b"").decode())

    def get_params(self) -> Params:
        p = Params()
        self._chk(self.lib.mi355ndt_get_params(self.h, C.byref(p)), "get_params")
        return p

    def set_params(self, p: Params):
        self._chk(self.lib.mi355ndt_set_params(self.h, C.byref(p)), "set_params")

    def set_stream(self, stream_ptr: int | None):
        self._chk(self.lib.mi355ndt_set_stream(self.h, C.c_void_p(stream_ptr or 0)), "set_stream")

    def set_target(self, cloud):
        a = _as_points(cloud)
        self._chk(self.lib.mi355ndt_set_target(self.h, a.ctypes.data_as(C.c_void_p), a.shape[0], a.strides[0]), "set_target")

    def promote_source_to_target(self):
        self._chk(self.lib.mi355ndt_promote_source_to_target(self.h), "promote_source_to_target")

    def set_source(self, cloud):
        a = _as_points(cloud)
        self._n_src = a.shape[0]
        self._chk(self.lib.mi355ndt_set_source(self.h, a.ctypes.data_as(C.c_void_p), a.shape[0], a.strides[0]), "set_source")

    def align(self, guess) -> dict:
        g = _colmajor(guess)
        r = Result()
        self._chk(self.lib.mi355ndt_align(self.h, g.ctypes.data_as(C.c_void_p), C.byref(r)), "align")
        return _result_dict(r)

    def get_aligned(self) -> np.ndarray:
        out = np.zeros((self._n_src, 3), np.float32)
        self._chk(self.lib.mi355ndt_get_aligned(self.h, out.ctypes.data_as(C.c_void_p), 12), "get_aligned")
        return out

    def get_incremental(self, pair: int = 0):
        a, b = np.zeros(16, np.float32), np.zeros(16, np.float32)
        self._chk(self.lib.mi355ndt_get_incremental(self.h, pair, a.ctypes.data_as(C.c_void_p), b.ctypes.data_as(C.c_void_p)), "get_incremental")
        return a.reshape(4, 4).T.copy(), b.reshape(4, 4).T.copy()

    def fitness_score(self, max_range: float = float("inf"), T=None):
        s, n = C.c_double(), C.c_longlong()
        mr = 1.7976931348623157e308 if max_range == float("inf") else float(max_range)
        if T is None:
            self._chk(self.lib.mi355ndt_get_fitness_score(self.h, mr, C.byref(s), C.byref(n)), "get_fitness_score")
        else:
            t = _colmajor(T)
            self._chk(self.lib.mi355ndt_fitness_score_T(self.h, t.ctypes.data_as(C.c_void_p), mr, C.byref(s), C.byref(n)), "fitness_score_T")
        return s.value, n.value

    def calculate_score(self, cloud) -> float:
        a = _as_points(cloud)
        s = C.c_double()
        self._chk(self.lib.mi355ndt_calculate_score(self.h, a.ctypes.data_as(C.c_void_p), a.shape[0], a.strides[0] if a.shape[0] else 12, C.byref(s)), "calculate_score")
        return s.value

    def set_option(self, option: int, value: int):
        self._chk(self.lib.mi355ndt_set_option(self.h, option, value), "set_option")

    def get_option(self, option: int) -> int:
        v = C.c_int()
        self._chk(self.lib.mi355ndt_get_option(self.h, option, C.byref(v)), "get_option")
        return v.value

    def prefilter(self, cloud, distance_near=0.5, distance_far=100.0, downsample_resolution=0.1, use_distance_filter=True,
                  fetch=True, outlier=None):
        a = _as_points(cloud)
        n_out = C.c_size_t()
        if outlier is not None:
            self.prefilter(a, distance_near, distance_far, downsample_resolution, use_distance_filter, fetch=False)
            return self.prefilter_outliers(**{"fetch": fetch, **outlier})
        out = np.zeros((a.shape[0], 3), np.float32) if fetch else None
        self._chk(self.lib.mi355ndt_prefilter(self.h, a.ctypes.data_as(C.c_void_p), a.shape[0], a.strides[0] if a.shape[0] else 12,
                                              int(use_distance_filter), float(distance_near), float(distance_far),
                                              float(downsample_resolution), out.ctypes.data_as(C.c_void_p) if fetch else None,
                                              a.shape[0], 12, C.byref(n_out)), "prefilter")
        self._pf_count = n_out.value
        return out[: n_out.value].copy() if fetch else n_out.value

    def prefilter_p(self, cloud, distance_near=0.5, distance_far=100.0, downsample_resolution=0.1, use_distance_filter=True, transform=None,
                    downsample_method="VOXELGRID", angle_calibration=False, fetch=True):
        prm = _prefilter_params(distance_near, distance_far, downsample_resolution, use_distance_filter, transform, downsample_method, angle_calibration)
        a = _as_points(cloud)
        n_out = C.c_size_t()
        out = np.zeros((a.shape[0], 3), np.float32) if fetch else None
        self._chk(self.lib.mi355ndt_prefilter_p(self.h, a.ctypes.data_as(C.c_void_p), a.shape[0], a.strides[0] if a.shape[0] else 12, C.byref(prm.base),
                                                out.ctypes.data_as(C.c_void_p) if fetch else None, a.shape[0], 12, C.byref(n_out)), "prefilter_p")
        self._pf_count = n_out.value
        return out[: n_out.value].copy() if fetch else n_out.value

    def prefilter_outliers(self, method="STATISTICAL", mean_k=20, stddev_mul=1.0, radius=0.8, min_neighbors=2, fetch=True, return_stats=False):
        if isinstance(method, str):
            method = {"STATISTICAL": OUTLIER_STATISTICAL, "RADIUS": OUTLIER_RADIUS}.get(method.upper(), 0)
# ... 719 lines not shown
```

Measured before the change: 65270.

## Add lean sweep variant with higher waves-per-SIMD and split probe tiles for async align

Introduces a LEAN template path for the one-launch async align sweep. It uses a different SweepTune (more waves per SIMD, smaller probe groups within a staged super-tile), and is chosen automatically when the estimated voxel-record footprint fits a share of L2. It also shrinks k_rank from 1024 to 512 threads, and adds an option, profile fields and a partial-rows debug getter. The aim is more latency hiding through occupancy on DIRECT7 workloads, at the cost of register and LDS pressure and possible L2 thrash when the estimate is wrong.

```diff
diff --git a/include/mi355_ndt.h b/include/mi355_ndt.h
--- a/include/mi355_ndt.h
+++ b/include/mi355_ndt.h
@@ -75,6 +75,8 @@
   long long stream_reserved_slots;
   long long stream_launch_slots;
   long long score_only_sweeps;
+  long long async_waves_per_simd;
+  long long async_launch_slots;
 } mi355ndt_profile;
 
 typedef struct mi355ndt_handle mi355ndt_handle;
@@ -123,7 +125,8 @@
   MI355NDT_OPT_OUTLIER_CELL_MM = 10,
   MI355NDT_OPT_PREFILTER_GROUP = 11,
   MI355NDT_OPT_POSE_MODEL = 12,
-  MI355NDT_OPT_NDT_CLASS = 13
+  MI355NDT_OPT_NDT_CLASS = 13,
+  MI355NDT_OPT_SWEEP_WAVES = 14
 };
 int mi355ndt_set_option(mi355ndt_handle* h, int option, int value);
 int mi355ndt_get_option(const mi355ndt_handle* h, int option, int* value);
@@ -132,6 +135,7 @@
 int mi355ndt_compute_hessian(mi355ndt_handle* h, const double p[6], double H[36]);
 int mi355ndt_derivatives_T(mi355ndt_handle* h, const float T_colmajor[16], const float Rj_rowmajor[9],
                            double* score, double g[6], double H[36], long long* hits);
+int mi355ndt_get_partial_rows(mi355ndt_handle* h, double* out, size_t capacity, int* rows_per_pair);
 int mi355ndt_get_grid(mi355ndt_handle* h, int pair, int min_b[3], int max_b[3], int div_b[3], int* n_voxels);
 int mi355ndt_get_voxels(mi355ndt_handle* h, int pair, mi355ndt_voxel* out, size_t capacity);
 
diff --git a/lv_slam_amd/csrc/mi355_ndt.hip b/lv_slam_amd/csrc/mi355_ndt.hip
--- a/lv_slam_amd/csrc/mi355_ndt.hip
+++ b/lv_slam_amd/csrc/mi355_ndt.hip
@@ -49,6 +49,7 @@
 #include "ndt_async.hpp"
 #include "ndt_hostmem.hpp"
 #include "ndt_grid_state.hpp"
+#include "ndt_sweep_waves.hpp"
 #ifndef NDT_SINGLE_TU
 #include "ndt_ord1_list.hpp"
 #include "ndt_fast_list.hpp"
diff --git a/lv_slam_amd/csrc/ndt_async.hpp b/lv_slam_amd/csrc/ndt_async.hpp
--- a/lv_slam_amd/csrc/ndt_async.hpp
+++ b/lv_slam_amd/csrc/ndt_async.hpp
@@ -205,8 +205,8 @@
 #define NDT_CTX_PARAMS(i) const float* __restrict__ src##i, size_t pitch##i, PairState* st##i, const GridDesc* __restrict__ gd##i, const BitWord* __restrict__ words##i, \
                           const VoxelRec* __restrict__ recs##i, double* partials##i, const int* __restrict__ src_cnt##i, unsigned* arrived##i, const float* __restrict__ cent##i
 #define NDT_CTX_SEL(f, ci) ((ci) == 0 ? f##0 : (ci) == 1 ? f##1 : (ci) == 2 ? f##2 : f##3)
-template <bool PCA, int K, int ORD>
-__global__ void __launch_bounds__(SWEEP_THREADS, (SweepTune<PCA, K, ORD>::WPE))
+template <bool PCA, int K, int ORD, bool LEAN = false>
+__global__ void __launch_bounds__(SWEEP_THREADS, (SweepTune<PCA, K, ORD, LEAN>::WPE))
 k_align_async(const AsyncTab* __restrict__ tab, int items_per_pair, int* ring, int ring_cap, AsyncCtl* ctl, SweepConst sc, unsigned long long* hits_total,
               double step_max, double eps, int max_iterations, int stop_thresh, unsigned debug_abort_pos, unsigned debug_ring_mask, int claim_items,
               NDT_CTX_PARAMS(0), NDT_CTX_PARAMS(1), NDT_CTX_PARAMS(2), NDT_CTX_PARAMS(3)) {
@@ -306,7 +306,7 @@
       } else {
 #pragma unroll 1
         for (int k = 0; k < CLAIM; k++)
-          sweep_item<PCA, K, 8, false, ORD, true, SO>(b, rem + k, C.src, C.pitch, C.st, C.gd, C.words, C.recs, C.partials, I, sc, C.cent, nullptr, exp_tab, pose_w, n_b, b, tl);
+          sweep_item<PCA, K, 8, false, ORD, true, SO, 0, LEAN>(b, rem + k, C.src, C.pitch, C.st, C.gd, C.words, C.recs, C.partials, I, sc, C.cent, nullptr, exp_tab, pose_w, n_b, b, tl);
       }
     };
     if (last) items(std::true_type()); else items(std::false_type());
diff --git a/lv_slam_amd/csrc/ndt_build.hpp b/lv_slam_amd/csrc/ndt_build.hpp
--- a/lv_slam_amd/csrc/ndt_build.hpp
+++ b/lv_slam_amd/csrc/ndt_build.hpp
@@ -173,15 +173,18 @@
   if (lane == 0) head_cnt[(size_t)b * n_slices + q] = n;
 }
 #define RANK_ROWS 8
-__global__ void __launch_bounds__(1024) k_rank(GridDesc* gd, BitWord* words, const unsigned* __restrict__ heads, const unsigned* __restrict__ head_cnt,
-                                                 unsigned n_slices, unsigned slice_cap, unsigned* seg_start) {
+#define RANK_WAVES 8
+#define RANK_THREADS (64 * RANK_WAVES)
+__global__ void __launch_bounds__(RANK_THREADS) k_rank(GridDesc* gd, BitWord* words, const unsigned* __restrict__ heads, const unsigned* __restrict__ head_cnt,
+                                                         unsigned n_slices, unsigned slice_cap, unsigned* seg_start) {
   __shared__ unsigned wtot[17];
+  static_assert(RANK_WAVES <= 16, "wtot");
   const int b = blockIdx.x;
   BitWord* W = words + gd[b].word_off;
   const int nw = gd[b].nwords;
   const int lane = threadIdx.x & 63, wv = threadIdx.x >> 6;
   unsigned base = 0;
-  for (int w0 = 0; w0 < nw; w0 += 1024 * RANK_ROWS) {
+  for (int w0 = 0; w0 < nw; w0 += RANK_THREADS * RANK_ROWS) {
     const int wbase = w0 + wv * 64 * RANK_ROWS;
     unsigned c[RANK_ROWS], ex[RANK_ROWS], run = 0;
 #pragma unroll
@@ -197,12 +200,12 @@
     if (lane == 0) wtot[wv] = run;
     __syncthreads();
     if (wv == 0) {
-      const unsigned v = lane < 16 ? wtot[lane] : 0u;
+      const unsigned v = lane < RANK_WAVES ? wtot[lane] : 0u;
       unsigned inc = v;
 #pragma unroll
-      for (int o = 1; o < 16; o <<= 1) { const unsigned t = __shfl_up(inc, o); if (lane >= o) inc += t; }
-      if (lane < 16) wtot[lane] = inc - v;
-      if (lane == 15) wtot[16] = inc;
+      for (int o = 1; o < RANK_WAVES; o <<= 1) { const unsigned t = __shfl_up(inc, o); if (lane >= o) inc += t; }
+      if (lane < RANK_WAVES) wtot[lane] = inc - v;
+      if (lane == RANK_WAVES - 1) wtot[16] = inc;
     }
     __syncthreads();
     const unsigned off = base + wtot[wv];
@@ -213,11 +216,11 @@
   }
   if (threadIdx.x == 0) gd[b].n_voxels = (int)base;
   unsigned hbase = 0;
-  for (unsigned q0 = 0; q0 < n_slices; q0 += 1024) {
+  for (unsigned q0 = 0; q0 < n_slices; q0 += RANK_THREADS) {
     const unsigned q = q0 + threadIdx.x;
     const unsigned c = q < n_slices ? head_cnt[(size_t)b * n_slices + q] : 0u;
     unsigned tot;
-    const unsigned ex = block_exscan<1024>(c, &tot, wtot);
+    const unsigned ex = block_exscan<RANK_THREADS>(c, &tot, wtot);
     const unsigned* H = heads + ((size_t)b * n_slices + q) * slice_cap;
     unsigned* S = seg_start + gd[b].rec_off + hbase + ex;
     for (unsigned k = 0; k < c; k++) S[k] = H[k];
diff --git a/lv_slam_amd/csrc/ndt_engine.hpp b/lv_slam_amd/csrc/ndt_engine.hpp
--- a/lv_slam_amd/csrc/ndt_engine.hpp
+++ b/lv_slam_amd/csrc/ndt_engine.hpp
@@ -29,6 +29,9 @@
   DevBuf<int> d_ring;
   DevBuf<CtxStat> d_stat;
   HipStream build_stream; int reserve_wg = 0, launch_slots = 0;
+  bool lean = false;
+  bool reserve_given = false;
+  int last_reserve = 0, last_slots = 0;
   HipEvent ev_built[ASYNC_MAX_CTX], ev_launched[EV], ev_prepared[EV]; bool prep_first = true;
   PinBuf<volatile StreamStatus> h_status; StreamStatus* d_status = nullptr;
   StreamCtx ctx[ASYNC_MAX_CTX];
@@ -170,6 +173,8 @@
   DevBuf<AsyncTab> d_atab;
   unsigned debug_abort_pos = 0xFFFFFFFFu;
   unsigned debug_ring_mask = 0xFFu;
+  int sweep_waves = 0;
+  int last_async_wpe = 0, last_async_grid = 0;
   int arith = 0;
   DevBuf<VoxelRecF> d_recs_fast;
   int pose_model = 0;
@@ -320,4 +325,4 @@
 }
 static bool async_served(const mi355ndt_handle* h) { return h->async_align && !mt_is_live(h->prm) && !is_pca_kd(h->prm) && model_leaves_rounds(h->pose_model, h->ndt_class); }
 static double sweep_alg_bytes(double points, int K) { return points * (12.0 + 4.0 * K); }
-static int launch_slots(const mi355ndt_handle* h, const SweepConst& sc, bool fast) { return h->n_cu * sweep_wpe(sc.K, fast); }
+static int launch_slots(const mi355ndt_handle* h, const SweepConst& sc, bool fast, bool lean = false) { return h->n_cu * sweep_wpe(sc.K, fast, lean); }
diff --git a/lv_slam_amd/csrc/ndt_host_align.hpp b/lv_slam_amd/csrc/ndt_host_align.hpp
--- a/lv_slam_amd/csrc/ndt_host_align.hpp
+++ b/lv_slam_amd/csrc/ndt_host_align.hpp
@@ -69,7 +69,7 @@
   return MI355NDT_OK;
 }
 
-static int align_async(mi355ndt_handle* h, const SweepConst& sc, int B, mi355ndt_result* out) {
+static int align_async(mi355ndt_handle* h, const SweepConst& sc, int B, mi355ndt_result* out, bool lean) {
   const int ring_cap = async_ring_cap(h, B);
   if (ring_cap == 0) return MI355NDT_ERR_UNSUPPORTED;
   if (h->d_ring.reserve((size_t)8 * ring_cap) != hipSuccess) { (void)hipGetLastError(); return MI355NDT_ERR_UNSUPPORTED; }
@@ -85,6 +85,7 @@
   L.active_list = h->d_active_list; L.sweep_ctl = h->d_ctl;
   L.tab_dev = h->d_atab; L.ring = h->d_ring; L.ring_cap = ring_cap; L.ctl = h->d_actl; L.prev = nullptr;
   L.items_per_pair = h->items_per_pair; L.stop_thresh = 0; L.debug_abort_pos = h->debug_abort_pos; L.debug_ring_mask = h->debug_ring_mask;
+  L.lean = lean;
   int rc = launch_async(h, sc, L);
   if (rc) return rc;
   HIPCHK(h, hipMemcpyAsync(h->h_pin_actl, h->d_actl, 8 * sizeof(unsigned), hipMemcpyDeviceToHost, h->stream));
@@ -109,9 +110,11 @@
   memcpy(h->h_pin_guess, guesses, (size_t)B * 16 * sizeof(float));
   HIPCHK(h, hipMemcpyAsync(h->d_guess, h->h_pin_guess, (size_t)B * 16 * sizeof(float), hipMemcpyHostToDevice, s));
   h->ctl_idx = 0;
+  const int tgt_max = *std::max_element(h->h_tgt_cnt.begin(), h->h_tgt_cnt.begin() + B);
+  const bool lean = async_lean(h, sc, sweep_ord(h, sc), tgt_max > 0 ? (size_t)tgt_max : h->tgt_pitch);
   const bool big_batch = (long long)B * h->items_per_pair > (long long)launch_slots(h, sc, sweep_ord(h, sc) == 2) * WAVES;
   if (async_served(h) && (big_batch || h->async_force) && !h->fine_it) {
-    rc = align_async(h, sc, B, out);
+    rc = align_async(h, sc, B, out, lean);
     if (rc != MI355NDT_ERR_UNSUPPORTED) return rc;
   }
   HIPCHK(h, hipMemsetAsync(h->d_ctl, 0, 2 * sizeof(SweepCtl), s));
diff --git a/lv_slam_amd/csrc/ndt_host_build.hpp b/lv_slam_amd/csrc/ndt_host_build.hpp
--- a/lv_slam_amd/csrc/ndt_host_build.hpp
+++ b/lv_slam_amd/csrc/ndt_host_build.hpp
@@ -77,7 +77,7 @@
     HIPCHK(h, h->d_heads.reserve((size_t)B * nsl * scap));
     HIPCHK(h, h->d_head_cnt.reserve((size_t)B * nsl));
     k_mark<unsigned><<<dim3((nsl + 3) / 4, B), 256, 0, s>>>(kb, pitch, h->d_grid, h->d_words, h->d_heads, h->d_head_cnt, nsl, scap, minpts, cb);
-    k_rank<<<B, 1024, 0, s>>>(h->d_grid, h->d_words, h->d_heads, h->d_head_cnt, nsl, scap, h->d_seg_start);
+    k_rank<<<B, RANK_THREADS, 0, s>>>(h->d_grid, h->d_words, h->d_heads, h->d_head_cnt, nsl, scap, h->d_seg_start);
     const int lb = std::max(1, std::min((int)((rpp + LS_WAVES - 1) / LS_WAVES), 64));
     auto leafsum = [&](auto kern, const unsigned* vals) {
       kern<<<xcd_grid(lb, B), 64 * LS_WAVES, 0, s>>>(h->d_tgt, pitch, kb, vals, h->d_grid, h->d_seg_start, h->d_sums, h->d_vox_idx, h->d_vox_n, cb, h->d_cent, lb, B);
diff --git a/lv_slam_amd/csrc/ndt_host_hooks.hpp b/lv_slam_amd/csrc/ndt_host_hooks.hpp
--- a/lv_slam_amd/csrc/ndt_host_hooks.hpp
+++ b/lv_slam_amd/csrc/ndt_host_hooks.hpp
@@ -33,6 +33,21 @@
   HIPCHK(h, hipStreamSynchronize(h->stream));
   if (last) memcpy(last, buf, 16 * sizeof(float));
   if (prev) memcpy(prev, buf + 16, 16 * sizeof(float));
+  return MI355NDT_OK;
+}
+
+int mi355ndt_get_partial_rows(mi355ndt_handle* h, double* out, size_t capacity, int* rows_per_pair) {
+  if (!h) return MI355NDT_ERR_BAD_HANDLE;
+  NOT_IN_STREAM(h);
+  if (!rows_per_pair) return MI355NDT_ERR_BAD_ARG;
+  if (h->n_pairs < 1 || !h->aligned_once || !h->d_partials || h->rows_per_pair < 1) return MI355NDT_ERR_STATE;
+  *rows_per_pair = h->rows_per_pair;
+  if (!out) return MI355NDT_OK;
+  const size_t need = (size_t)h->n_pairs * h->rows_per_pair * NACC;
+  if (capacity < need) return MI355NDT_ERR_BAD_ARG;
+  HIPCHK(h, hipSetDevice(h->device));
+  HIPCHK(h, hipMemcpyAsync(out, h->d_partials, need * sizeof(double), hipMemcpyDeviceToHost, h->stream));
+  HIPCHK(h, hipStreamSynchronize(h->stream));
   return MI355NDT_OK;
 }
 
diff --git a/lv_slam_amd/csrc/ndt_host_life.hpp b/lv_slam_amd/csrc/ndt_host_life.hpp
--- a/lv_slam_amd/csrc/ndt_host_life.hpp
+++ b/lv_slam_amd/csrc/ndt_host_life.hpp
@@ -101,6 +101,7 @@
   if (const char* e = std::getenv("MI355NDT_LEAF_SORTED")) h->leaf_sorted = std::atoi(e) != 0;
   if (const char* e = std::getenv("MI355NDT_FINE_TILES")) { const int v = std::atoi(e); if (v == 1 || v == 2) h->fine_tiles = v; }
   if (const char* e = std::getenv("MI355NDT_ARITH")) h->arith = std::atoi(e) == 1 ? 1 : 0;
+  if (const char* e = std::getenv("MI355NDT_SWEEP_WAVES")) { const int v = std::atoi(e); if (v == 0 || v == 2 || v == 3) h->sweep_waves = v; }
   if (const char* e = std::getenv("MI355NDT_ASYNC")) { h->async_align = std::atoi(e) != 0; h->async_force = std::atoi(e) == 2; }
   if (const char* e = std::getenv("MI355NDT_SCORE_ONLY_LAST_SWEEP")) h->score_only_last = std::atoi(e) != 0;
   if (const char* e = std::getenv("MI355NDT_SWEEP_DYN_SHIFT")) { const int v = std::atoi(e); if (v >= 0 && v <= 30) h->dyn_shift = v; }
@@ -190,7 +191,8 @@
 int mi355ndt_set_option(mi355ndt_handle* h, int option, int value) {
   if (!h) return MI355NDT_ERR_BAD_HANDLE;
   if (h->ss && (option == MI355NDT_OPT_F32_SUM_ORDER || option == MI355NDT_OPT_ARITH || option == MI355NDT_OPT_ASYNC_ALIGN ||
-                       option == MI355NDT_OPT_SCORE_ONLY_LAST_SWEEP || option == MI355NDT_OPT_POSE_MODEL || option == MI355NDT_OPT_NDT_CLASS)) NOT_IN_STREAM(h);
+                       option == MI355NDT_OPT_SCORE_ONLY_LAST_SWEEP || option == MI355NDT_OPT_POSE_MODEL || option == MI355NDT_OPT_NDT_CLASS ||
+                       option == MI355NDT_OPT_SWEEP_WAVES)) NOT_IN_STREAM(h);
   if (option == MI355NDT_OPT_NDT_CLASS) {
     if (value != NDT_CLASS_OMP && value != NDT_CLASS_PCL) return MI355NDT_ERR_BAD_ARG;
     h->ndt_class = value;
@@ -209,6 +211,11 @@
   if (option == MI355NDT_OPT_ARITH) {
     if (value != 0 && value != 1) return MI355NDT_ERR_BAD_ARG;
     h->arith = value;
+    return MI355NDT_OK;
+  }
+  if (option == MI355NDT_OPT_SWEEP_WAVES) {
+    if (const int rc = sweep_waves_option_rc(false, value)) return rc;
+    h->sweep_waves = value;
     return MI355NDT_OK;
   }
   if (option == MI355NDT_OPT_ASYNC_ALIGN) {
@@ -263,6 +270,7 @@
   if (!value) return MI355NDT_ERR_BAD_ARG;
   if (option == MI355NDT_OPT_F32_SUM_ORDER) { *value = h->f32_sum_order; return MI355NDT_OK; }
   if (option == MI355NDT_OPT_ARITH) { *value = h->arith; return MI355NDT_OK; }
+  if (option == MI355NDT_OPT_SWEEP_WAVES) { *value = h->sweep_waves; return MI355NDT_OK; }
   if (option == MI355NDT_OPT_POSE_MODEL) { *value = h->pose_model; return MI355NDT_OK; }
   if (option == MI355NDT_OPT_NDT_CLASS) { *value = h->ndt_class; return MI355NDT_OK; }
   if (option == MI355NDT_OPT_ASYNC_ALIGN) { *value = h->async_force ? 2 : (h->async_align ? 1 : 0); return MI355NDT_OK; }
diff --git a/lv_slam_amd/csrc/ndt_host_profile.hpp b/lv_slam_amd/csrc/ndt_host_profile.hpp
--- a/lv_slam_amd/csrc/ndt_host_profile.hpp
+++ b/lv_slam_amd/csrc/ndt_host_profile.hpp
@@ -82,9 +82,10 @@
   unsigned long long hh[2] = {0, 0};
   HIPCHK(h, hipMemcpy(hh, h->d_hits, sizeof hh, hipMemcpyDeviceToHost));
   *out = h->P;
-  if (h->ss) { out->stream_reserved_slots = h->ss->reserve_wg; out->stream_launch_slots = h->ss->launch_slots; }
+  if (h->ss) { out->stream_reserved_slots = h->ss->last_reserve; out->stream_launch_slots = h->ss->last_slots; }
   out->sweep_hits += (long long)hh[0];
   out->sweep_alg_bytes += 64.0 * (double)hh[0];
   out->score_only_sweeps = (long long)hh[1];
+  out->async_waves_per_simd = h->last_async_wpe; out->async_launch_slots = h->last_async_grid;
   return MI355NDT_OK;
 }
diff --git a/lv_slam_amd/csrc/ndt_host_stream.hpp b/lv_slam_amd/csrc/ndt_host_stream.hpp
--- a/lv_slam_amd/csrc/ndt_host_stream.hpp
+++ b/lv_slam_amd/csrc/ndt_host_stream.hpp
@@ -56,12 +56,13 @@
   {
     const bool small_batch = (unsigned long long)max_pairs * (unsigned long long)max_tgt <= 768ull * 65536ull;
     int r = sc.K == 1 ? (max_tgt <= 98304 ? 128 : 96) : ((sc.K == 7 && small_batch) ? (sc.pca ? 32 : 64) : 0);
-    if (const char* e = std::getenv("MI355NDT_STREAM_RESERVE")) r = std::atoi(e);
-    if (h->s_reserve_opt >= 0) r = h->s_reserve_opt;
+    if (const char* e = std::getenv("MI355NDT_STREAM_RESERVE")) { r = std::atoi(e); ss.reserve_given = true; }
+    if (h->s_reserve_opt >= 0) { r = h->s_reserve_opt; ss.reserve_given = true; }
     r = std::max(0, std::min(r, slots / 2)) & ~7;
     if (n_contexts < 3) r = 0;
     ss.reserve_wg = r;
     ss.launch_slots = std::max(8, slots - r);
+    ss.last_reserve = r; ss.last_slots = ss.launch_slots;
   }
   ss.ring_cap = async_ring_cap(h, (long long)max_pairs + ASYNC_MAX_CARRY);
   if (ss.ring_cap == 0) ss.sync_only = true;
@@ -82,7 +83,7 @@
     }
     rc = mi355ndt_set_stream(e, ss.reserve_wg > 0 ? ss.build_stream : h->stream);
     if (rc) return rc;
-    e->f32_sum_order = h->f32_sum_order; e->arith = h->arith; e->async_align = h->async_align; e->dyn_shift = h->dyn_shift; e->score_only_last = h->score_only_last;
+    e->sweep_waves = h->sweep_waves; e->f32_sum_order = h->f32_sum_order; e->arith = h->arith; e->async_align = h->async_align; e->dyn_shift = h->dyn_shift; e->score_only_last = h->score_only_last;
     e->async_build = true;
     e->ev_pool_target = 128;
     rc = ensure_pair_arrays(e, max_pairs);
@@ -142,7 +143,15 @@
   L.tab_dev = h->d_atab; L.ring = ss.d_ring; L.ring_cap = ss.ring_cap;
   L.ctl = ss.d_ctl + (j & 1); L.prev = ss.drop_carry ? nullptr : ss.d_ctl + ((j + 1) & 1);
   L.items_per_pair = ss.items; L.stop_thresh = flush ? 0 : (ss.thresh_given ? ss.thresh : std::min(ss.thresh, n_new / 4)); L.debug_abort_pos = h->debug_abort_pos; L.debug_ring_mask = h->debug_ring_mask;
+  if (!flush) {
+    const mi355ndt_handle* e = ss.ctx[new_ci].e.get();
+    const int tgt_max = *std::max_element(e->h_tgt_cnt.begin(), e->h_tgt_cnt.begin() + n_new);
+    ss.lean = async_lean(h, sc, sweep_ord(h, sc), tgt_max > 0 ? (size_t)tgt_max : ss.max_tgt);
+  }
+  L.lean = ss.lean;
   L.reserve_wg = flush ? 0 : ss.reserve_wg;
+  if (L.lean && !flush && !ss.reserve_given && ss.reserve_wg > 0) L.reserve_wg = LEAN_RESERVE_WG;
+  if (L.lean) L.reserve_wg = std::min(L.reserve_wg, launch_slots(h, sc, false, true) / 2) & ~7;
   L.ev_prepared = (ss.reserve_wg > 0 && ss.prep_first) ? ss.ev_prepared[j % StreamState::EV] : nullptr;
   L.claim_items = (sc.K == 7 && L.stop_thresh > 0) ? 2 : 1;
   h->ev_last_fresh = false;
@@ -151,6 +160,7 @@
   int rc = launch_async(h, sc, L);
   if (rc) return rc;
   ss.drop_carry = false;
+  if (!flush) { ss.last_reserve = L.reserve_wg; ss.last_slots = h->last_async_grid; }
   const int slot = (int)(j % StreamState::EV);
   k_stream_status<<<1, 64, 0, s>>>(L.ctl, ss.d_stat, reinterpret_cast<volatile unsigned*>(ss.d_status + slot), (unsigned)(j + 1));
   HIPCHK(h, hipGetLastError());
diff --git a/lv_slam_amd/csrc/ndt_host_sweep.hpp b/lv_slam_amd/csrc/ndt_host_sweep.hpp
--- a/lv_slam_amd/csrc/ndt_host_sweep.hpp
+++ b/lv_slam_amd/csrc/ndt_host_sweep.hpp
@@ -21,6 +21,12 @@
   by_K(std::false_type{}); by_K(std::true_type{});
   return rc;
 }
+
+static_assert(sizeof(VoxelRec) == LEAN_REC_BYTES, "the record the estimate counts");
+static bool async_lean(const mi355ndt_handle* h, const SweepConst& sc, int ord, size_t tgt_pts) {
+  return async_served(h) && lean_exists(sc.pca != 0, sc.K, ord) && sweep_waves_choice(h->sweep_waves, h->prm, ord, tgt_pts) == 3;
+}
+constexpr int LEAN_RESERVE_WG = 96;
 
 static int prep_align_ws(mi355ndt_handle* h) {
   const int B = h->n_pairs;
@@ -159,25 +165,27 @@
   unsigned long long* stamp_end = nullptr;
   int claim_items = 1;
   int reserve_wg = 0;
+  bool lean = false;
   hipEvent_t ev_prepared = nullptr;
 };
 #define NDT_CTX_ARGS(i) L.tab.c[i].src, L.tab.c[i].pitch, L.tab.c[i].st, L.tab.c[i].gd, L.tab.c[i].words, L.tab.c[i].recs, L.tab.c[i].partials, L.tab.c[i].src_cnt, \
                         L.tab.c[i].arrived, L.tab.c[i].cent
-template <bool PCA, int K, int ORD>
+template <bool PCA, int K, int ORD, bool LEAN = false>
 static int launch_async_t(mi355ndt_handle* h, const SweepConst& sc, const AsyncLaunch& L) {
-  auto kern = k_align_async<PCA, K, ORD>;
+  auto kern = k_align_async<PCA, K, ORD, LEAN>;
   static std::atomic<int> per_cu_of_device[64];
   int per_cu = per_cu_of_device[h->device & 63].load(std::memory_order_relaxed);
   if (per_cu == 0) {
     if (hipOccupancyMaxActiveBlocksPerMultiprocessor(&per_cu, kern, SWEEP_THREADS, 0) != hipSuccess) { (void)hipGetLastError(); return MI355NDT_ERR_UNSUPPORTED; }
     per_cu_of_device[h->device & 63].store(per_cu, std::memory_order_relaxed);
   }
-  const int slots = launch_slots(h, sc, ORD == 2);
+  const int slots = launch_slots(h, sc, ORD == 2, LEAN);
   if (per_cu * h->n_cu < slots || slots < 8) return MI355NDT_ERR_UNSUPPORTED;
   dim3 grid((unsigned)std::max(8, slots - L.reserve_wg));
   kern<<<grid, SWEEP_THREADS, 0, h->stream>>>(L.tab_dev, L.items_per_pair, L.ring, L.ring_cap, L.ctl, sc, h->prof ? h->d_hits : nullptr,
                                              h->prm.step_size, h->prm.trans_epsilon, h->prm.max_iterations, L.stop_thresh, L.debug_abort_pos, L.debug_ring_mask, L.claim_items,
                                              NDT_CTX_ARGS(0), NDT_CTX_ARGS(1), NDT_CTX_ARGS(2), NDT_CTX_ARGS(3));
+  h->last_async_wpe = SweepTune<PCA, K, ORD, LEAN>::WPE; h->last_async_grid = (int)grid.x;
   return MI355NDT_OK;
 }
 static int launch_async(mi355ndt_handle* h, const SweepConst& sc, const AsyncLaunch& L) {
@@ -190,6 +198,8 @@
   }
   if (h->prof) HIPCHK(h, ev_begin(h, h->ev_sweep));
   const int rc = dispatch_sweep(sc.pca != 0, sc.K, sweep_ord(h, sc), SWEEP_IT_BATCH, [&](auto P, auto KK, auto O, auto) {
+    if constexpr (lean_exists(decltype(P)::value, decltype(KK)::value, decltype(O)::value))
+      if (L.lean) return launch_async_t<false, 7, decltype(O)::value, true>(h, sc, L);
     return launch_async_t<decltype(P)::value, decltype(KK)::value, decltype(O)::value>(h, sc, L);
   });
   if (h->prof) HIPCHK(h, ev_end(h, h->ev_sweep));
diff --git a/lv_slam_amd/csrc/ndt_ord1_list.hpp b/lv_slam_amd/csrc/ndt_ord1_list.hpp
--- a/lv_slam_amd/csrc/ndt_ord1_list.hpp
+++ b/lv_slam_amd/csrc/ndt_ord1_list.hpp
@@ -20,4 +20,5 @@
   X __global__ void k_align_async<false, 1, 1> NDT_ASYNC_ARGS_T;  X __global__ void k_align_async<true, 1, 1> NDT_ASYNC_ARGS_T;           \
   X __global__ void k_align_async<false, 7, 1> NDT_ASYNC_ARGS_T;  X __global__ void k_align_async<true, 7, 1> NDT_ASYNC_ARGS_T;           \
   X __global__ void k_align_async<false, 26, 1> NDT_ASYNC_ARGS_T; X __global__ void k_align_async<true, 26, 1> NDT_ASYNC_ARGS_T;          \
-  X __global__ void k_align_async<false, 27, 1> NDT_ASYNC_ARGS_T;
+  X __global__ void k_align_async<false, 27, 1> NDT_ASYNC_ARGS_T;                                                                          \
+  X __global__ void k_align_async<false, 7, 1, true> NDT_ASYNC_ARGS_T;
diff --git a/lv_slam_amd/csrc/ndt_sweep.hpp b/lv_slam_amd/csrc/ndt_sweep.hpp
--- a/lv_slam_amd/csrc/ndt_sweep.hpp
+++ b/lv_slam_amd/csrc/ndt_sweep.hpp
@@ -381,14 +381,16 @@
 #ifndef FAST_PIPE
 #define FAST_PIPE 1
 #endif
-template <bool PCA, int K, int ORD = 0>
+template <bool PCA, int K, int ORD = 0, bool LEAN = false>
 struct SweepTune {
+  static_assert(!LEAN || (!PCA && K == 7 && (ORD == 0 || ORD == 1)), "the lean body: exact ndt_omp / DIRECT7");
   static constexpr bool FAST = (ORD == 2);
-  static constexpr int  WPE  = FAST ? (K == 1 ? FAST_WPE1 : FAST_WPE7) : SWEEP_WPE;
-  static constexpr bool PIPE = FAST ? (FAST_PIPE != 0) : true;
+  static constexpr int  WPE  = LEAN ? 3 : (FAST ? (K == 1 ? FAST_WPE1 : FAST_WPE7) : SWEEP_WPE);
+  static constexpr bool PIPE = LEAN ? false : (FAST ? (FAST_PIPE != 0) : true);
   static constexpr int  TP   = FAST ? (K == 1 ? FAST_TP1 : FAST_TP7) : (K == 1 ? 8 : (K <= 7 ? 2 : 1));
+  static constexpr int  TPP  = LEAN ? 1 : TP;
 };
-static inline int sweep_wpe(int K, bool fast = false) { return fast ? (K == 1 ? FAST_WPE1 : FAST_WPE7) : SWEEP_WPE; }
+static inline int sweep_wpe(int K, bool fast = false, bool lean = false) { return lean ? 3 : (fast ? (K == 1 ? FAST_WPE1 : FAST_WPE7) : SWEEP_WPE); }
 
 #define POSE_W_LAST 21
 __device__ __forceinline__ unsigned sweep_pose_words(const PairState* S) {
@@ -479,7 +481,7 @@
 struct BatchF { unsigned slot; float mh[3], ml[3], c[6]; int weight; float w; };
 struct BatchD { unsigned slot; double m0, m1, m2; double C[9]; };
 struct NoRows {};
-template <bool PCA, int K, int ORD, bool SO, int Q_CAP, bool W_LATE = false, int PM = 0>
+template <bool PCA, int K, int ORD, bool SO, int Q_CAP, bool W_LATE = false, int PM = 0, bool LEAN = false>
 struct HitQueue {
   static_assert(PM == 0 || ((PM == 1 || PM == 2) && !PCA && ORD != 2 && !SO), "the Euler model: ndt_omp, exact arithmetic, full rows");
   static_assert(PM != 2 || (K == 27 && ORD == 0), "PCL's class: the radius search, one instantiation");
@@ -576,7 +578,7 @@
     eval_batch(B, m, NoHook());
   }
   __device__ __forceinline__ void drain_full() {
-    if (PM == 2 || !SweepTune<PCA, K, ORD>::PIPE) {
+    if (PM == 2 || !SweepTune<PCA, K, ORD, LEAN>::PIPE) {
       while (count >= 64) drain(64);
       return;
     }
@@ -594,7 +596,7 @@
   }
 };
 
-template <bool PCA, int K, int IT, bool FINE, int ORD, bool ASYNC, bool SO = false, int PM = 0>
+template <bool PCA, int K, int IT, bool FINE, int ORD, bool ASYNC, bool SO = false, int PM = 0, bool LEAN = false>
 __device__ __forceinline__ void sweep_item(const int b, const int rem, const float* __restrict__ src, const size_t pitch, const PairState* st,
                                            const GridDesc* __restrict__ gd, const BitWord* __restrict__ words, const VoxelRec* __restrict__ recs,
                                            double* partials, const int rows_per_pair, const SweepConst& sc, const float* __restrict__ cent,
@@ -607,18 +609,22 @@
   static_assert(!FAST || K == 1 || K == 7, "tolerance arithmetic is instantiated for DIRECT1 / DIRECT7");
   static_assert(PM == 0 || (!PCA && !FAST && !ASYNC && !FINE && !SO), "the Euler model takes the lockstep rounds: ndt_omp, exact arithmetic, batch items");
   static_assert(PM != 2 || (K == 27 && ORD == 0 && IT == 8), "PCL's class: the radius search, batch items");
-  typedef SweepTune<PCA, K, ORD> Tune;
+  static_assert(!LEAN || (ASYNC && !FINE && PM == 0 && IT == 8), "the lean body belongs to the one-launch align");
+  typedef SweepTune<PCA, K, ORD, LEAN> Tune;
   const int lane = threadIdx.x & 63, wv = threadIdx.x >> 6;
   constexpr bool PCAQ = PCA && K > 1;
-  constexpr int TP = Tune::TP < IT ? Tune::TP : IT;
+  constexpr int TPS = Tune::TP < IT ? Tune::TP : IT;
+  constexpr int TP = Tune::TPP < TPS ? Tune::TPP : TPS;
+  constexpr int GPS = TPS / TP;
+  static_assert(TPS % TP == 0, "probe groups tile the super-tile");
   constexpr int Q_NEED = (IT / TP > 1 ? 64 : 0) + TP * (K < Q_GROUP ? K : Q_GROUP) * 64;
   constexpr int Q_CAP = FAST ? (Q_NEED <= 128 ? 128 : Q_NEED <= 256 ? 256 : Q_NEED <= 512 ? 512 : 1024) : ((K > 1 && K <= Q_GROUP) ? 1024 : 512);
   static_assert(Q_NEED <= Q_CAP, "hit queue");
-  typedef HitQueue<PCA, K, ORD, SO, Q_CAP, false, PM> Queue;
+  typedef HitQueue<PCA, K, ORD, SO, Q_CAP, false, PM, LEAN> Queue;
   auto& q_ent = item_lds<unsigned[WAVES][Q_CAP], 0>();
   auto& q_w = item_lds<typename Queue::QW[PCAQ ? WAVES : 1][PCAQ ? Q_CAP : 1], 1>();
-  constexpr int NBUF = (IT / TP > 1) ? 2 : 1;
-  auto& stage = item_lds<float[WAVES][NBUF * 64 * TP][6], 2>();
+  constexpr int NBUF = (IT / TPS > 1) ? 2 : 1;
+  auto& stage = item_lds<float[WAVES][NBUF * 64 * TPS][6], 2>();
 
   auto& red = item_lds<double[FINE ? WAVES : 1][FINE ? NACC : 1], 3>();
   const PairState& S = st[b];
@@ -661,8 +667,11 @@
 #pragma unroll 1
       for (int st = 0; st < NST; st++) {
         if (wbase + st * TP * 64 >= n) break;
-        if (Q.old > 0) { __builtin_amdgcn_wave_barrier(); Q.drain(Q.old); }
-        Q.old = Q.count;
+        if (GPS == 1 || st % GPS == 0) {
+          if (Q.old > 0) { __builtin_amdgcn_wave_barrier(); Q.drain(Q.old); }
+          Q.old = Q.count;
+        }
+#define NDT_STAGE_TILE(p) (GPS == 1 ? (st & 1) * TP + (p) : ((st / GPS) & 1) * TPS + (st % GPS) * TP + (p))
         int r0[TP], r1[TP], r2[TP], cc[TP];
         bool valid[TP];
         float kx[TP], ky[TP], kz[TP];
@@ -677,8 +686,8 @@
 #pragma unroll
           for (int a = 0; a < 3; a++) move_axis(T + 4 * a, Rj + 3 * a, px, py, pz, xt[a], r[a]);
           ok = ok && finite3(xt[0], xt[1], xt[2]);
-          if constexpr (PM != 0) { const float xo[3] = {px, py, pz}; stage_point(stage[wv][((st & 1) * TP + p) * 64 + lane], xt, xo); }
-          else stage_point(stage[wv][((st & 1) * TP + p) * 64 + lane], xt, r);
+          if constexpr (PM != 0) { const float xo[3] = {px, py, pz}; stage_point(stage[wv][NDT_STAGE_TILE(p) * 64 + lane], xt, xo); }
+          else stage_point(stage[wv][NDT_STAGE_TILE(p) * 64 + lane], xt, r);
           kx[p] = xt[0]; ky[p] = xt[1]; kz[p] = xt[2];
           rel_cell(xt, sc, leaf, mb0, mb1, mb2, r0[p], r1[p], r2[p]);
           cc[p] = r0[p] + r1[p] * mul1 + r2[p] * mul2;
@@ -724,7 +733,7 @@
           }
 #pragma unroll
           for (int p = 0; p < TP; p++) {
-            const int slot = ((st & 1) * TP + p) * 64 + lane;
+            const int slot = NDT_STAGE_TILE(p) * 64 + lane;
 #pragma unroll
             for (int j = 0; j < Q_GROUP; j++) {
               if (q1 - 1 - j < 0) continue;
@@ -739,6 +748,7 @@
           TL_STAMP(5);
         }
       }
+#undef NDT_STAGE_TILE
       __builtin_amdgcn_wave_barrier();
       if (Q.count > 0) Q.drain(Q.count);
       TL_STAMP(5);
diff --git a/lv_slam_amd/csrc/ndt_sweep_waves.hpp b/lv_slam_amd/csrc/ndt_sweep_waves.hpp
--- /dev/null
+++ b/lv_slam_amd/csrc/ndt_sweep_waves.hpp
@@ -0,0 +1,27 @@
+#pragma once
+#include <algorithm>
+#include <cstddef>
+#include "mi355_ndt.h"
+
+static inline int sweep_waves_option_rc(bool in_stream, int value) {
+  if (in_stream) return MI355NDT_ERR_STATE;
+  return (value == 0 || value == 2 || value == 3) ? MI355NDT_OK : MI355NDT_ERR_BAD_ARG;
+}
+
+constexpr bool lean_exists(bool pca, int K, int ord) { return !pca && K == 7 && (ord == 0 || ord == 1); }
+
+constexpr size_t LEAN_L2_BYTES = (size_t)4 << 20;
+constexpr int LEAN_PAIRS_IN_FLIGHT = 3;
+constexpr size_t LEAN_REC_BYTES_MAX = LEAN_L2_BYTES / 4 / LEAN_PAIRS_IN_FLIGHT;
+constexpr double LEAN_PTS_PER_M2 = 32.0;
+constexpr size_t LEAN_REC_BYTES = 64;
+static inline size_t est_record_bytes(const mi355ndt_params& prm, size_t tgt_pts) {
+  const double by_face = (double)tgt_pts / (LEAN_PTS_PER_M2 * (double)prm.resolution * (double)prm.resolution);
+  const double by_count = (double)tgt_pts / (double)std::max(1, prm.min_points_per_voxel);
+  return (size_t)(std::min(by_face, by_count) * (double)LEAN_REC_BYTES);
+}
+static inline int sweep_waves_choice(int option, const mi355ndt_params& prm, int ord, size_t tgt_pts) {
+  if (!lean_exists(prm.variant == MI355NDT_VARIANT_PCA, prm.neighbor_mode == MI355NDT_DIRECT7 ? 7 : 0, ord) || option == 2) return 2;
+  if (option == 3) return 3;
+  return est_record_bytes(prm, tgt_pts) <= LEAN_REC_BYTES_MAX ? 3 : 2;
+}
diff --git a/lv_slam_amd/ndt.py b/lv_slam_amd/ndt.py
--- a/lv_slam_amd/ndt.py
+++ b/lv_slam_amd/ndt.py
@@ -46,7 +46,8 @@
                 ("update_launches", C.c_longlong), ("async_fallbacks", C.c_longlong), ("stream_launches", C.c_longlong),
                 ("stream_carried", C.c_longlong), ("stream_redone", C.c_longlong), ("cloud_uploads", C.c_longlong), ("cloud_upload_bytes", C.c_longlong),
                 ("cloud_transfers", C.c_longlong), ("cloud_promotions", C.c_longlong),
-                ("stream_reserved_slots", C.c_longlong), ("stream_launch_slots", C.c_longlong), ("score_only_sweeps", C.c_longlong)]
+                ("stream_reserved_slots", C.c_longlong), ("stream_launch_slots", C.c_longlong), ("score_only_sweeps", C.c_longlong),
+                ("async_waves_per_simd", C.c_longlong), ("async_launch_slots", C.c_longlong)]
 
 
 class InfParams(C.Structure):
@@ -111,6 +112,7 @@
     "mi355ndt_version", "mi355ndt_device_count", "mi355ndt_host_numa_node", "mi355ndt_default_params", "mi355ndt_create", "mi355ndt_destroy",
     "mi355ndt_set_params", "mi355ndt_get_params", "mi355ndt_set_stream", "mi355ndt_last_error",
     "mi355ndt_set_target", "mi355ndt_set_source", "mi355ndt_promote_source_to_target", "mi355ndt_align", "mi355ndt_get_aligned", "mi355ndt_get_incremental",
+    "mi355ndt_get_partial_rows",
     "mi355ndt_get_fitness_score", "mi355ndt_fitness_score_T", "mi355ndt_prefilter", "mi355ndt_use_prefiltered", "mi355ndt_derivatives", "mi355ndt_compute_hessian", "mi355ndt_derivatives_T", "mi355ndt_get_grid", "mi355ndt_get_voxels",
     "mi355ndt_batch_reserve", "mi355ndt_batch_set_target", "mi355ndt_batch_set_source", "mi355ndt_batch_set_clouds", "mi355ndt_batch_bind_device",
     "mi355ndt_batch_build_targets", "mi355ndt_batch_align", "mi355ndt_batch_size", "mi355ndt_batch_pose_records", "mi355ndt_batch_fitness_scores",
@@ -146,6 +148,7 @@
 OPT_STREAM_THRESHOLD = 4
 WARN_TOLERANCE_ARITH = 1
 OPT_ARITH = 7
+OPT_SWEEP_WAVES = 14
 OPT_F32_SUM_ORDER = 1
 OPT_SCORE_ONLY_LAST_SWEEP = 8
 OPT_KF_FITNESS_CELL_MM = 9
@@ -190,6 +193,7 @@
     L.mi355ndt_align.argtypes = [vp, vp, C.POINTER(Result)]
     L.mi355ndt_get_aligned.argtypes = [vp, vp, sz]
     L.mi355ndt_get_incremental.argtypes = [vp, i, vp, vp]
+    L.mi355ndt_get_partial_rows.argtypes = [vp, vp, C.c_size_t, C.POINTER(C.c_int)]
     L.mi355ndt_get_fitness_score.argtypes = [vp, C.c_double, vp, vp]
     L.mi355ndt_fitness_score_T.argtypes = [vp, vp, C.c_double, vp, vp]
     L.mi355ndt_prefilter.argtypes = [vp, vp, sz, sz, i, C.c_double, C.c_double, C.c_float, vp, sz, sz, C.POINTER(sz)]
@@ -485,6 +489,14 @@
         self._chk(self.lib.mi355ndt_get_incremental(self.h, pair, a.ctypes.data_as(C.c_void_p), b.ctypes.data_as(C.c_void_p)), "get_incremental")
         return a.reshape(4, 4).T.copy(), b.reshape(4, 4).T.copy()
 
+    def partial_rows(self) -> np.ndarray:
+        rpp = C.c_int()
+        self._chk(self.lib.mi355ndt_get_partial_rows(self.h, None, 0, C.byref(rpp)), "get_partial_rows")
+        B = self.lib.mi355ndt_batch_size(self.h)
+        out = np.zeros((B, rpp.value, 44), np.float64)
+        self._chk(self.lib.mi355ndt_get_partial_rows(self.h, out.ctypes.data_as(C.c_void_p), out.size, C.byref(rpp)), "get_partial_rows")
+        return out
+
     def fitness_score(self, max_range: float = float("inf"), T=None):
         s, n = C.c_double(), C.c_longlong()
         mr = 1.7976931348623157e308 if max_range == float("inf") else float(max_range)
```

After: 68800 (median of 6 runs). 5.4% higher.
